# lucidrains/progen

Measured on NVIDIA B200. Metric: tokens_per_sec, higher is better.
Workload: dtype bf16

## Files before the change

### include/progen_b200.h

```cpp
#ifndef PROGEN_B200_H
#define PROGEN_B200_H
#include <stdint.h>

#ifdef __cplusplus
extern "C" {
#endif

#define PROGEN_F32 0
#define PROGEN_BF16 1

#define PROGEN_BACKEND_SIMT 0
#define PROGEN_BACKEND_TCGEN05 1

#define PROGEN_EPI_STORE 0
#define PROGEN_EPI_ROTARY 1
#define PROGEN_EPI_RESIDUAL 2
#define PROGEN_EPI_GLU 3
#define PROGEN_EPI_GELU 4
#define PROGEN_EPI_GLU_BWD 5
#define PROGEN_EPI_GELU_BWD 6
#define PROGEN_EPI_ACCUM 7

const char* progen_version(void);
const char* progen_last_error(void);
int progen_device_check(void);
long long progen_launch_count(void);

typedef struct progen_gemm_t {
  int32_t M, N, K;
  int32_t a_mn_major, b_mn_major;
  int32_t batch;
  int32_t batch_reduce;
  int32_t causal;
  int32_t split_k;
  int32_t in_dtype, out_dtype, epi_kind, backend;
  int32_t seq_len, dim_head;
  int32_t atomic, tril, tril_rows;
  int64_t lda, ldb;
  int64_t a_batch_rows, b_batch_rows, d_batch_rows;
  int64_t ldo, ldo2, ldaux;
  const void* A;
  const void* B;
  void* out;
  void* out2;
  const float* bias;
  const void* aux;
  const float* rot_sin;
  const float* rot_cos;
} progen_gemm_t;

int progen_gemm(const progen_gemm_t* desc, void* stream);

int progen_embed_fwd(const int* tokens, const float* table, float* x, long long T, int d, int V, void* stream);
int progen_embed_bwd(const int* tokens, const float* dx, float* dtable, long long T, int d, int V, void* stream);

int progen_ln_shift_fwd(const void* x, long long ldx, int x_dtype, const float* scale, void* y, long long ldy, int y_dtype,
                        float* mean, float* rstd, long long T, int d, int seq_len, int shift, void* stream);
int progen_ln_shift_bwd(const void* dy, long long lddy, int act_dtype, const void* x, long long ldx, int x_dtype,
                        const float* scale, const float* mean, const float* rstd, float* dres, void* dout, long long ldo,
                        float* dscale, float* dres_colsum, long long T, int d, int seq_len, int shift, int residual,
                        void* stream);

int progen_colsum(const void* in, long long ld, int dtype, float* out, long long T, int N, void* stream);

int progen_ce_fwd_bwd(const void* logits, int dtype, const int* labels, float* weights, float* loss, void* dlogits,
                      int dlogits_dtype, int B, int n, int V, float inv_batch, void* stream);

int progen_rotary_bwd(void* dqkv, long long ld, int dtype, const float* sin_t, const float* cos_t, long long T, int ncols,
                      int seq_len, int dim_head, void* stream);

int progen_local_attn_fwd_simt(const void* qkv, void* out, float* lse, int dtype, int B, int seq_len, int window, int heads,
                               int dim_head, void* stream);
int progen_local_attn_bwd_simt(const void* qkv, const void* out, const void* dout, const float* lse, void* dqkv,
                               float* delta, int dtype, int B, int seq_len, int window, int heads, int dim_head,
                               void* stream);

int progen_local_attn_fwd(const void* qkv, void* out, float* lse, int B, int seq_len, int window, int heads, int dim_head,
                          void* stream);
int progen_local_attn_bwd(const void* qkv, const void* out, const void* dout, const float* lse, void* dqkv, float* delta,
                          const float* rot_sin, const float* rot_cos, int B, int seq_len, int window, int heads, int dim_head,
                          void* stream);

int progen_local_attn_fwd_tc(const void* qkv, void* out, float* lse, int B, int seq_len, int window, int heads, int dim_head,
                             void* stream);

int progen_local_attn_bwd_tc(const void* qkv, const void* out, const void* dout, const float* lse, void* dqkv, float* delta,
                             const float* rot_sin, const float* rot_cos, int B, int seq_len, int window, int heads, int dim_head,
                             void* stream);
int progen_local_attn_bwd_tc_ex(const void* qkv, const void* out, const void* dout, const float* lse, void* dqkv, float* delta,
                                const float* rot_sin, const float* rot_cos, const float* rot_sin_t, const float* rot_cos_t, int B,
                                int seq_len, int window, int heads, int dim_head, int mode, void* stream);

int progen_sgu_gate_fwd(const void* xs, long long ldx, const void* gp, long long ldg, const float* bias, void* out,
                        long long ldo, int dtype, long long T, int C, int seq_len, void* stream);
int progen_sgu_gate_bwd(const void* ds, long long ldds, const void* xs, long long ldx, const void* gp, long long ldg,
                        const float* bias, void* dxs, long long lddx, void* dgp, long long lddg, float* dbias, int dtype,
                        long long T, int C, int seq_len, void* stream);
int progen_gelu_bwd(void* da, const void* u, int dtype, long long numel, void* stream);
int progen_cast_f32(const float* in, void* out, int out_dtype, long long numel, void* stream);
int progen_tril_cast(const float* w, void* out, int out_dtype, int n, void* stream);

int progen_optim_workspace_floats(void);
int progen_grad_sqnorm(const float* g, long long n, float* workspace, float* out_sqnorm, void* stream);
int progen_adamw_step(float* p, void* p_lp, const float* g, float* m, float* v, float* acc, long long n, long long n_decay,
                      const float* gnorm_sq, float lr, float b1, float b2, float eps, float wd, float max_norm,
                      long long step, int emit, void* stream);
int progen_adamw_step_dev(float* p, void* p_lp, const float* g, float* m, float* v, float* acc, long long n, long long n_decay,
                          const float* gnorm_sq, float lr, float b1, float b2, float eps, float wd, float max_norm,
                          int apply_every, void* state, void* stream);

typedef struct progen_decode_layer_t {
  int32_t kind;
  int32_t _pad;
  const float* ln1_scale;
  const void* wqkv_t;
  const void* wo_t;
  const float* bo;
  const float* ln2_scale;
  const void* win_t;
  const float* bin;
  const void* wout_t;
  const float* bout;
  const float* sgu_ln_scale;
  const float* sgu_w;
  const float* sgu_b;
  const void* sgu_proj_t;
  const float* sgu_proj_b;
  float* kcache;
  float* vcache;
  float* shift1;
  float* shift2;
  float* gn_hist;
} progen_decode_layer_t;

typedef struct progen_decode_t {
  int32_t n, d, heads, dim_head, inner, window, hid, V, depth, wdtype, shift_tokens, top_k;
  const float* embed;
  const float* lnf_scale;
  const void* whead_t;
  const float* bhead;
  const float* rot_sin;
  const float* rot_cos;
  const progen_decode_layer_t* layers;
  int32_t* seq;
  int32_t* pos;
  const float* noise;
  float* logits_all;
  float *x, *y, *q, *att, *u, *gn, *sg, *pj, *logits;
} progen_decode_t;

int progen_decode_step(const progen_decode_t* model, int do_sample, void* stream);

typedef struct progen_decode_run_t {
  int32_t n, d, heads, dim_head, inner, window, hid, V, depth, wdtype, shift_tokens, top_k;
  int32_t B, pos0, nsteps, _pad;
  const float* embed;
  const float* lnf_scale;
  const void* whead_t;
  const float* bhead;
  const float* rot_sin;
  const float* rot_cos;
  const progen_decode_layer_t* layers;
  int32_t* seq;
  const int32_t* start;
  const float* noise;
  float* logits_all;
  float* x;
  float* q;
  float* att;
  float* att_part;
  int32_t* att_count;
  float* u;
  float* sg;
  float* pj;
  float* logits;
  uint32_t* grid_bar;
  long long* prof;
} progen_decode_run_t;

int progen_decode_run(const progen_decode_run_t* run, void* stream);

#ifdef __cplusplus
}
#endif
#endif
```

### progen_b200/csrc/api.cu

```cuda
#include <stdarg.h>
#include "gemm.h"
#include "../../include/progen_b200.h"

static thread_local char g_err[1024] = "";
unsigned long long g_progen_launches = 0;

void progen_set_error(const char* fmt, ...) {
  va_list ap;
  va_start(ap, fmt);
  vsnprintf(g_err, sizeof(g_err), fmt, ap);
  va_end(ap);
}

extern "C" {

const char* progen_version(void) { return "progen_b200 0.1.0 (sm_100a; tcgen05/TMA GEMM, CUDA " CUDA_VERSION_STR ")"; }

const char* progen_last_error(void) { return g_err; }

long long progen_launch_count(void) { return (long long)__atomic_load_n(&g_progen_launches, __ATOMIC_RELAXED); }

int progen_device_check(void) {
  int dev = 0;
  PG_CUDA(cudaGetDevice(&dev));
  cudaDeviceProp prop;
  PG_CUDA(cudaGetDeviceProperties(&prop, dev));
  if (prop.major != 10) {
    progen_set_error("device %d (%s) is sm_%d%d; libprogen_b200 is built for sm_100a only", dev, prop.name, prop.major,
                     prop.minor);
    return PROGEN_ERR_DEVICE;
  }
  return PROGEN_OK;
}

int progen_gemm(const progen_gemm_t* d, void* stream) {
  PG_CHECK_ARG(d != nullptr);
  GemmArgs g;
  g.M = d->M; g.N = d->N; g.K = d->K;
  g.A = d->A; g.lda = d->lda; g.a_mn_major = d->a_mn_major;
  g.B = d->B; g.ldb = d->ldb; g.b_mn_major = d->b_mn_major;
  g.batch = d->batch < 1 ? 1 : d->batch;
  g.a_batch_rows = d->a_batch_rows; g.b_batch_rows = d->b_batch_rows; g.d_batch_rows = d->d_batch_rows;
  g.batch_reduce = d->batch_reduce; g.causal = d->causal; g.split_k = d->split_k < 1 ? 1 : d->split_k;
  g.in_dtype = d->in_dtype; g.out_dtype = d->out_dtype; g.epi_kind = d->epi_kind;
  g.epi.out = d->out; g.epi.ldo = d->ldo; g.epi.out2 = d->out2; g.epi.ldo2 = d->ldo2;
  g.epi.bias = d->bias; g.epi.aux = d->aux; g.epi.ldaux = d->ldaux;
  g.epi.rot_sin = d->rot_sin; g.epi.rot_cos = d->rot_cos;
  g.epi.seq_len = d->seq_len > 0 ? d->seq_len : 1; g.epi.dim_head = d->dim_head > 0 ? d->dim_head : 2;
  g.epi.atomic = d->atomic; g.epi.tril = d->tril; g.epi.tril_rows = d->tril_rows > 0 ? d->tril_rows : 1;
  PG_CHECK_ARG(g.epi_kind >= 0 && g.epi_kind < EPI_NUM_KINDS);
  PG_CHECK_ARG(g.epi.out != nullptr);
  if (g.epi_kind == EPI_GLU || g.epi_kind == EPI_GELU) PG_CHECK_ARG(g.epi.out2 != nullptr && g.epi.bias != nullptr);
  if (g.epi_kind == EPI_GLU_BWD || g.epi_kind == EPI_GELU_BWD) PG_CHECK_ARG(g.epi.aux != nullptr);
  if (g.epi_kind == EPI_ROTARY) PG_CHECK_ARG(g.epi.rot_sin && g.epi.rot_cos && d->seq_len > 0 && d->dim_head > 0 && d->dim_head % 2 == 0);
  if (d->backend == PROGEN_BACKEND_TCGEN05) return gemm_tc_launch(g, (cudaStream_t)stream);
  if (d->backend == PROGEN_BACKEND_SIMT) return gemm_simt_launch(g, (cudaStream_t)stream);
  progen_set_error("progen_gemm: unknown backend %d", d->backend);
  return PROGEN_ERR_ARG;
}

}
```

### progen_b200/csrc/elementwise.cu

```cuda
#include "common.cuh"
#include "../../include/progen_b200.h"

int ln_shift_bwd_stream_launch(const void* dy, long long lddy, int act_dtype, const void* x, long long ldx, int x_dtype,
                               const float* scale, const float* mean, const float* rstd, float* dres, void* dout,
                               long long ldo, float* dscale, float* dres_colsum, long long T, int d, int seq_len, int shift,
                               int residual, cudaStream_t stream);

namespace {

constexpr int ROWS_PER_BLOCK = 8;
constexpr float LN_EPS = 1e-5f;

template <typename T> __device__ __forceinline__ void load4(const T* p, float (&v)[4]);
template <> __device__ __forceinline__ void load4<float>(const float* p, float (&v)[4]) {
  const float4 t = *reinterpret_cast<const float4*>(p);
  v[0] = t.x; v[1] = t.y; v[2] = t.z; v[3] = t.w;
}
template <> __device__ __forceinline__ void load4<bf16>(const bf16* p, float (&v)[4]) {
  const uint2 t = *reinterpret_cast<const uint2*>(p);
  const float2 a = __bfloat1622float2(*reinterpret_cast<const __nv_bfloat162*>(&t.x));
  const float2 b = __bfloat1622float2(*reinterpret_cast<const __nv_bfloat162*>(&t.y));
  v[0] = a.x; v[1] = a.y; v[2] = b.x; v[3] = b.y;
}
__device__ __forceinline__ void store4(float* p, const float (&v)[4]) {
  *reinterpret_cast<float4*>(p) = make_float4(v[0], v[1], v[2], v[3]);
}
__device__ __forceinline__ void store4(bf16* p, const float (&v)[4]) {
  uint2 t;
  t.x = pack_bf16x2(v[0], v[1]); t.y = pack_bf16x2(v[2], v[3]);
  *reinterpret_cast<uint2*>(p) = t;
}

__global__ void embed_fwd_kernel(const int* __restrict__ tok, const float* __restrict__ table, float* __restrict__ x,
                                 long long T, int d, int V) {
  const long long total = T * (d / 4);
  for (long long i = blockIdx.x * (long long)blockDim.x + threadIdx.x; i < total; i += (long long)gridDim.x * blockDim.x) {
    const long long t = i / (d / 4);
    const int c = (int)(i % (d / 4)) * 4;
    int id = tok[t];
    id = id < 0 ? 0 : (id >= V ? V - 1 : id);
    *reinterpret_cast<float4*>(x + t * d + c) = *reinterpret_cast<const float4*>(table + (long long)id * d + c);
  }
}

__global__ void embed_bwd_kernel(const int* __restrict__ tok, const float* __restrict__ dx, float* __restrict__ dtable,
                                 long long T, int d, int V, long long rows_per_block) {
  extern __shared__ float bins[];
  const int c0 = blockIdx.x * 32;
  const int lane = threadIdx.x & 31, warp = threadIdx.x >> 5, nwarp = blockDim.x >> 5;
  for (int i = threadIdx.x; i < V * 32; i += blockDim.x) bins[i] = 0.f;
  __syncthreads();
  const long long r0 = blockIdx.y * rows_per_block;
  const long long r1 = min(T, r0 + rows_per_block);
  if (c0 + lane < d) {
    for (long long t = r0 + warp; t < r1; t += nwarp) {
      int id = tok[t];
      id = id < 0 ? 0 : (id >= V ? V - 1 : id);
      atomicAdd(&bins[id * 32 + lane], dx[t * d + c0 + lane]);
    }
  }
  __syncthreads();
  for (int i = threadIdx.x; i < V * 32; i += blockDim.x) {
    const float v = bins[i];
    const int c = c0 + (i & 31);
    if (v != 0.f && c < d) atomicAdd(dtable + (long long)(i >> 5) * d + c, v);
  }
}

template <typename TI, typename TO>
__global__ void ln_shift_fwd_kernel(const TI* __restrict__ x, long long ldx, const float* __restrict__ scale,
                                    TO* __restrict__ y, long long ldy, float* __restrict__ mean_out,
                                    float* __restrict__ rstd_out, long long T, int d, int seq_len, int shift) {
  const int lane = threadIdx.x & 31, warp = threadIdx.x >> 5;
  const int half = d >> 1;
  for (long long t = blockIdx.x * (long long)ROWS_PER_BLOCK + warp; t < T; t += (long long)gridDim.x * ROWS_PER_BLOCK) {
    const TI* xr = x + t * ldx;
    float s = 0.f;
    for (int c = lane * 4; c < d; c += 128) {
      float v[4];
      load4<TI>(xr + c, v);
      s += v[0] + v[1] + v[2] + v[3];
    }
    const float mean = warp_sum(s) / d;
    float q = 0.f;
    for (int c = lane * 4; c < d; c += 128) {
      float v[4];
      load4<TI>(xr + c, v);
#pragma unroll
      for (int i = 0; i < 4; ++i) { const float u = v[i] - mean; q += u * u; }
    }
    const float rstd = rsqrtf(warp_sum(q) / d + LN_EPS);
    if (lane == 0) { mean_out[t] = mean; rstd_out[t] = rstd; }
    const int pos = (int)(t % seq_len);
    for (int c = lane * 4; c < d; c += 128) {
      float v[4], sc[4], o[4];
      load4<TI>(xr + c, v);
      load4<float>(scale + c, sc);
#pragma unroll
      for (int i = 0; i < 4; ++i) o[i] = (v[i] - mean) * rstd * sc[i];
      if (!shift || c >= half) {
        store4(y + t * ldy + c, o);
      } else {
        if (pos + 1 < seq_len) store4(y + (t + 1) * ldy + c, o);
        if (pos == 0) { const float z[4] = {0.f, 0.f, 0.f, 0.f}; store4(y + t * ldy + c, z); }
      }
    }
  }
}

template <typename TI, typename TO, int NCH, bool RESIDUAL>
__global__ void ln_shift_bwd_kernel(const TO* __restrict__ dy, long long lddy, const TI* __restrict__ x, long long ldx,
                                    const float* __restrict__ scale, const float* __restrict__ mean_in,
                                    const float* __restrict__ rstd_in, float* __restrict__ dres, TO* __restrict__ dout,
                                    long long ldo, float* __restrict__ dscale, float* __restrict__ dres_colsum,
                                    long long T, int d, int seq_len, int shift) {
  const int lane = threadIdx.x & 31, warp = threadIdx.x >> 5;
  const int half = d >> 1;
  float ds_acc[NCH][4];
  float cs_acc[RESIDUAL ? NCH : 1][4];
#pragma unroll
  for (int i = 0; i < NCH; ++i)
#pragma unroll
    for (int j = 0; j < 4; ++j) {
      ds_acc[i][j] = 0.f;
      if (RESIDUAL) cs_acc[RESIDUAL ? i : 0][j] = 0.f;
    }

  for (long long t = blockIdx.x * (long long)ROWS_PER_BLOCK + warp; t < T; t += (long long)gridDim.x * ROWS_PER_BLOCK) {
    const TI* xr = x + t * ldx;
    const float mean = mean_in[t], rstd = rstd_in[t];
    const int pos = (int)(t % seq_len);
    const bool has_next = pos + 1 < seq_len;
    float s1 = 0.f, s2 = 0.f;
    if constexpr (NCH <= 4) {
      float xh[NCH][4], gs[NCH][4], rr[NCH][4];
#pragma unroll
      for (int ch = 0; ch < NCH; ++ch) {
        const int c = ch * 128 + lane * 4;
#pragma unroll
        for (int i = 0; i < 4; ++i) { xh[ch][i] = 0.f; gs[ch][i] = 0.f; rr[ch][i] = 0.f; }
        if (c < d) {
          float sc[4];
          load4<TI>(xr + c, xh[ch]);
          load4<float>(scale + c, sc);
          if (!shift || c >= half) load4<TO>(dy + t * lddy + c, gs[ch]);
          else if (has_next) load4<TO>(dy + (t + 1) * lddy + c, gs[ch]);
          if constexpr (RESIDUAL) load4<float>(dres + t * (long long)d + c, rr[ch]);
#pragma unroll
          for (int i = 0; i < 4; ++i) {
            xh[ch][i] = (xh[ch][i] - mean) * rstd;
            ds_acc[ch][i] += gs[ch][i] * xh[ch][i];
            gs[ch][i] *= sc[i];
            s1 += gs[ch][i]; s2 += gs[ch][i] * xh[ch][i];
          }
        }
      }
      s1 = warp_sum(s1) / d;
      s2 = warp_sum(s2) / d;
#pragma unroll
      for (int ch = 0; ch < NCH; ++ch) {
        const int c = ch * 128 + lane * 4;
        if (c < d) {
          float o[4];
#pragma unroll
          for (int i = 0; i < 4; ++i) o[i] = rstd * (gs[ch][i] - s1 - xh[ch][i] * s2);
          if constexpr (RESIDUAL) {
#pragma unroll
            for (int i = 0; i < 4; ++i) { rr[ch][i] += o[i]; cs_acc[ch][i] += rr[ch][i]; }
            store4(dres + t * (long long)d + c, rr[ch]);
            if (dout) store4(dout + t * ldo + c, rr[ch]);
          } else {
            store4(dout + t * ldo + c, o);
          }
        }
      }
      continue;
    }
#pragma unroll
    for (int ch = 0; ch < NCH; ++ch) {
      const int c = ch * 128 + lane * 4;
      if (c < d) {
        float xv[4], sc[4], g[4] = {0.f, 0.f, 0.f, 0.f};
        load4<TI>(xr + c, xv);
        load4<float>(scale + c, sc);
        if (!shift || c >= half) load4<TO>(dy + t * lddy + c, g);
        else if (has_next) load4<TO>(dy + (t + 1) * lddy + c, g);
#pragma unroll
        for (int i = 0; i < 4; ++i) {
          const float xh = (xv[i] - mean) * rstd;
          ds_acc[ch][i] += g[i] * xh;
          const float gs = g[i] * sc[i];
          s1 += gs; s2 += gs * xh;
        }
      }
    }
    s1 = warp_sum(s1) / d;
    s2 = warp_sum(s2) / d;
#pragma unroll
    for (int ch = 0; ch < NCH; ++ch) {
      const int c = ch * 128 + lane * 4;
      if (c < d) {
        float xv[4], sc[4], g[4] = {0.f, 0.f, 0.f, 0.f}, o[4];
        load4<TI>(xr + c, xv);
        load4<float>(scale + c, sc);
        if (!shift || c >= half) load4<TO>(dy + t * lddy + c, g);
        else if (has_next) load4<TO>(dy + (t + 1) * lddy + c, g);
#pragma unroll
        for (int i = 0; i < 4; ++i) {
          const float xh = (xv[i] - mean) * rstd;
          o[i] = rstd * (g[i] * sc[i] - s1 - xh * s2);
        }
        if constexpr (RESIDUAL) {
          float r[4];
          load4<float>(dres + t * (long long)d + c, r);
#pragma unroll
          for (int i = 0; i < 4; ++i) { r[i] += o[i]; cs_acc[ch][i] += r[i]; }
          store4(dres + t * (long long)d + c, r);
          if (dout) store4(dout + t * ldo + c, r);
        } else {
          store4(dout + t * ldo + c, o);
        }
      }
    }
  }
  __shared__ float red[ROWS_PER_BLOCK][128];
#pragma unroll
  for (int ch = 0; ch < NCH; ++ch) {
    if (ch * 128 >= d) break;
#pragma unroll
    for (int i = 0; i < 4; ++i) red[warp][lane * 4 + i] = ds_acc[ch][i];
    __syncthreads();
    if (threadIdx.x < 128) {
      float s = 0.f;
#pragma unroll
      for (int w = 0; w < ROWS_PER_BLOCK; ++w) s += red[w][threadIdx.x];
      const int c = ch * 128 + threadIdx.x;
      if (c < d) atomicAdd(dscale + c, s);
    }
    __syncthreads();
    if constexpr (RESIDUAL) {
      if (dres_colsum) {
#pragma unroll
        for (int i = 0; i < 4; ++i) red[warp][lane * 4 + i] = cs_acc[ch][i];
        __syncthreads();
        if (threadIdx.x < 128) {
          float s = 0.f;
#pragma unroll
          for (int w = 0; w < ROWS_PER_BLOCK; ++w) s += red[w][threadIdx.x];
          const int c = ch * 128 + threadIdx.x;
          if (c < d) atomicAdd(dres_colsum + c, s);
        }
        __syncthreads();
      }
    }
  }
}

template <typename TI>
__global__ void colsum_kernel(const TI* __restrict__ in, long long ld, float* __restrict__ out, long long T, int N,
                              long long rows_per_block) {
  __shared__ float red[ROWS_PER_BLOCK][128];
  const int lane = threadIdx.x & 31, warp = threadIdx.x >> 5;
  const int c = blockIdx.x * 128 + lane * 4;
  const long long r0 = blockIdx.y * rows_per_block, r1 = min(T, r0 + rows_per_block);
  float acc[4] = {0.f, 0.f, 0.f, 0.f};
  if (c < N) {
    for (long long t = r0 + warp; t < r1; t += ROWS_PER_BLOCK) {
      float v[4];
      load4<TI>(in + t * ld + c, v);
#pragma unroll
      for (int i = 0; i < 4; ++i) acc[i] += v[i];
    }
  }
#pragma unroll
  for (int i = 0; i < 4; ++i) red[warp][lane * 4 + i] = acc[i];
  __syncthreads();
  if (threadIdx.x < 128) {
    float s = 0.f;
#pragma unroll
    for (int w = 0; w < ROWS_PER_BLOCK; ++w) s += red[w][threadIdx.x];
    const int cc = blockIdx.x * 128 + threadIdx.x;
    if (cc < N) atomicAdd(out + cc, s);
  }
}

__global__ void ce_weights_kernel(const int* __restrict__ labels, float* __restrict__ w, int n, float inv_batch) {
  __shared__ int s_first, s_count;
  const int b = blockIdx.x;
  if (threadIdx.x == 0) { s_first = n; s_count = 0; }
  __syncthreads();
  const int* lb = labels + (long long)b * n;
  int first = n, cnt = 0;
  for (int i = threadIdx.x; i < n; i += blockDim.x) {
    if (lb[i] == 0) first = min(first, i); else cnt++;
  }
  atomicMin(&s_first, first);
  atomicAdd(&s_count, cnt);
  __syncthreads();
  const int total = s_count + (s_first < n ? 1 : 0);
  const float wv = inv_batch / (float)total;
  for (int i = threadIdx.x; i < n; i += blockDim.x) w[(long long)b * n + i] = (lb[i] != 0 || i == s_first) ? wv : 0.f;
}

template <typename TL, typename TD>
__global__ void ce_fwd_bwd_kernel(const TL* __restrict__ logits, const int* __restrict__ labels,
                                  const float* __restrict__ w, float* __restrict__ loss, TD* __restrict__ dlogits,
                                  long long T, int V) {
  const int lane = threadIdx.x & 31, warp = threadIdx.x >> 5;
  float block_loss = 0.f;
  for (long long t = blockIdx.x * (long long)ROWS_PER_BLOCK + warp; t < T; t += (long long)gridDim.x * ROWS_PER_BLOCK) {
    const TL* lr = logits + t * V;
    float mx = -INFINITY;
    for (int c = lane * 4; c < V; c += 128) {
      float v[4];
      load4<TL>(lr + c, v);
      mx = fmaxf(mx, fmaxf(fmaxf(v[0], v[1]), fmaxf(v[2], v[3])));
    }
    mx = warp_max(mx);
    float se = 0.f;
    for (int c = lane * 4; c < V; c += 128) {
      float v[4];
      load4<TL>(lr + c, v);
#pragma unroll
      for (int i = 0; i < 4; ++i) se += expf(v[i] - mx);
    }
    se = warp_sum(se);
    const int lab = min(max(labels[t], 0), V - 1);
    const float wt = w[t];
    const float lse = mx + logf(se);
    if (lane == 0) block_loss += wt * (lse - to_f32(lr[lab]));
    if (dlogits) {
      const float inv = 1.f / se;
      for (int c = lane * 4; c < V; c += 128) {
        float v[4], o[4];
        load4<TL>(lr + c, v);
#pragma unroll
        for (int i = 0; i < 4; ++i) o[i] = wt * (expf(v[i] - mx) * inv - ((c + i) == lab ? 1.f : 0.f));
        store4(dlogits + t * V + c, o);
      }
    }
  }
  __shared__ float red[ROWS_PER_BLOCK];
  if (lane == 0) red[warp] = block_loss;
  __syncthreads();
  if (threadIdx.x == 0) {
    float s = 0.f;
    for (int i = 0; i < ROWS_PER_BLOCK; ++i) s += red[i];
    atomicAdd(loss, s);
  }
}

template <typename TO>
__global__ void rotary_bwd_kernel(TO* __restrict__ dqkv, long long ld, const float* __restrict__ sin_t,
                                  const float* __restrict__ cos_t, long long T, int ncols, int seq_len, int dim_head) {
  const long long total = T * (ncols / 4);
  const int half = dim_head >> 1;
  for (long long i = blockIdx.x * (long long)blockDim.x + threadIdx.x; i < total; i += (long long)gridDim.x * blockDim.x) {
    const long long t = i / (ncols / 4);
    const int c = (int)(i % (ncols / 4)) * 4;
    const int pos = (int)(t % seq_len);
    float v[4], o[4];
    load4<TO>(dqkv + t * ld + c, v);
#pragma unroll
    for (int p = 0; p < 4; p += 2) {
      const int j = ((c + p) % dim_head) >> 1;
      const float s = __ldg(sin_t + (long long)pos * half + j), cs = __ldg(cos_t + (long long)pos * half + j);
      o[p] = v[p] * cs + v[p + 1] * s;
      o[p + 1] = v[p + 1] * cs - v[p] * s;
    }
    store4(dqkv + t * ld + c, o);
  }
}

template <typename TO>
__global__ void sgu_gate_fwd_kernel(const TO* __restrict__ xs, long long ldx, const TO* __restrict__ gp, long long ldg,
                                    const float* __restrict__ bias, TO* __restrict__ out, long long ldo, long long T, int C,
                                    int seq_len) {
  const long long total = T * (C / 4);
  for (long long i = blockIdx.x * (long long)blockDim.x + threadIdx.x; i < total; i += (long long)gridDim.x * blockDim.x) {
    const long long t = i / (C / 4);
    const int c = (int)(i % (C / 4)) * 4;
    const float b = __ldg(bias + (t % seq_len));
    float x[4], g[4], o[4];
    load4<TO>(xs + t * ldx + c, x);
    load4<TO>(gp + t * ldg + c, g);
#pragma unroll
    for (int j = 0; j < 4; ++j) o[j] = x[j] * (g[j] + b);
    store4(out + t * ldo + c, o);
  }
}

template <typename TO>
__global__ void sgu_gate_bwd_kernel(const TO* __restrict__ ds, long long ldds, const TO* __restrict__ xs, long long ldx,
                                    const TO* __restrict__ gp, long long ldg, const float* __restrict__ bias,
                                    TO* __restrict__ dxs, long long lddx, TO* __restrict__ dgp, long long lddg,
                                    float* __restrict__ dbias, long long T, int C, int seq_len) {
  const int lane = threadIdx.x & 31, warp = threadIdx.x >> 5;
  for (long long t = blockIdx.x * (long long)ROWS_PER_BLOCK + warp; t < T; t += (long long)gridDim.x * ROWS_PER_BLOCK) {
    const int m = (int)(t % seq_len);
    const float b = __ldg(bias + m);
    float acc = 0.f;
    for (int c = lane * 4; c < C; c += 128) {
      float d[4], x[4], g[4], o1[4], o2[4];
      load4<TO>(ds + t * ldds + c, d);
      load4<TO>(xs + t * ldx + c, x);
      load4<TO>(gp + t * ldg + c, g);
#pragma unroll
      for (int j = 0; j < 4; ++j) {
        o1[j] = d[j] * (g[j] + b);
        o2[j] = d[j] * x[j];
        acc += o2[j];
      }
      store4(dxs + t * lddx + c, o1);
      store4(dgp + t * lddg + c, o2);
    }
    acc = warp_sum(acc);
    if (lane == 0) atomicAdd(dbias + m, acc);
  }
}

template <typename TO>
__global__ void gelu_bwd_kernel(TO* __restrict__ da, const TO* __restrict__ u, long long total4) {
  for (long long i = blockIdx.x * (long long)blockDim.x + threadIdx.x; i < total4; i += (long long)gridDim.x * blockDim.x) {
    float d[4], x[4];
    load4<TO>(da + i * 4, d);
    load4<TO>(u + i * 4, x);
#pragma unroll
    for (int j = 0; j < 4; ++j) d[j] *= gelu_tanh_grad(x[j]);
    store4(da + i * 4, d);
  }
}

template <typename TO>
__global__ void cast_kernel(const float* __restrict__ in, TO* __restrict__ out, long long total4) {
  for (long long i = blockIdx.x * (long long)blockDim.x + threadIdx.x; i < total4; i += (long long)gridDim.x * blockDim.x) {
    float v[4];
    load4<float>(in + i * 4, v);
    store4(out + i * 4, v);
  }
}

template <typename TO>
__global__ void tril_cast_kernel(const float* __restrict__ w, TO* __restrict__ out, int n) {
  const long long total = (long long)n * (n / 4);
  for (long long i = blockIdx.x * (long long)blockDim.x + threadIdx.x; i < total; i += (long long)gridDim.x * blockDim.x) {
    const int r = (int)(i / (n / 4));
    const int c = (int)(i % (n / 4)) * 4;
    float v[4];
    load4<float>(w + (long long)r * n + c, v);
#pragma unroll
    for (int j = 0; j < 4; ++j) v[j] = (c + j <= r) ? v[j] : 0.f;
    store4(out + (long long)r * n + c, v);
  }
}

inline int ew_grid(long long work_items, int threads) {
  long long b = (work_items + threads - 1) / threads;
  const long long cap = (long long)pg_num_sms() * 8;
  return (int)(b < 1 ? 1 : (b > cap ? cap : b));
}
inline int row_grid(long long T) {
  long long b = (T + ROWS_PER_BLOCK - 1) / ROWS_PER_BLOCK;
  const long long cap = (long long)pg_num_sms() * 4;
  return (int)(b < 1 ? 1 : (b > cap ? cap : b));
}

}

extern "C" {

int progen_embed_fwd(const int* tokens, const float* table, float* x, long long T, int d, int V, void* stream) {
  PG_CHECK_ARG(T > 0 && d % 4 == 0 && V > 0);
  embed_fwd_kernel<<<ew_grid(T * (d / 4), 256), 256, 0, (cudaStream_t)stream>>>(tokens, table, x, T, d, V);
  PG_LAUNCH_CHECK();
  return PROGEN_OK;
}

int progen_embed_bwd(const int* tokens, const float* dx, float* dtable, long long T, int d, int V, void* stream) {
  PG_CHECK_ARG(T > 0 && d > 0 && V > 0 && V * 32 * 4 <= 48 * 1024);
  const int row_blocks = (int)((T + 4095) / 4096);
  const long long rpb = (T + row_blocks - 1) / row_blocks;
  dim3 grid((d + 31) / 32, row_blocks);
  embed_bwd_kernel<<<grid, 256, V * 32 * sizeof(float), (cudaStream_t)stream>>>(tokens, dx, dtable, T, d, V, rpb);
  PG_LAUNCH_CHECK();
  return PROGEN_OK;
}

int progen_ln_shift_fwd(const void* x, long long ldx, int x_dtype, const float* scale, void* y, long long ldy, int y_dtype,
                        float* mean, float* rstd, long long T, int d, int seq_len, int shift, void* stream) {
  PG_CHECK_ARG(T > 0 && d % 8 == 0 && seq_len > 0 && T % seq_len == 0);
  PG_CHECK_ARG(ldx % 4 == 0 && ldy % 4 == 0);
  cudaStream_t s = (cudaStream_t)stream;
  const int grid = row_grid(T);
#define LN_FWD(TI, TO) ln_shift_fwd_kernel<TI, TO><<<grid, 256, 0, s>>>((const TI*)x, ldx, scale, (TO*)y, ldy, mean, rstd, T, d, seq_len, shift)
  if (x_dtype == PG_F32 && y_dtype == PG_F32) LN_FWD(float, float);
  else if (x_dtype == PG_F32 && y_dtype == PG_BF16) LN_FWD(float, bf16);
  else if (x_dtype == PG_BF16 && y_dtype == PG_BF16) LN_FWD(bf16, bf16);
  else { progen_set_error("ln_shift_fwd: unsupported dtypes %d -> %d", x_dtype, y_dtype); return PROGEN_ERR_UNSUPPORTED; }
#undef LN_FWD
  PG_LAUNCH_CHECK();
  return PROGEN_OK;
}

int progen_ln_shift_bwd(const void* dy, long long lddy, int act_dtype, const void* x, long long ldx, int x_dtype,
                        const float* scale, const float* mean, const float* rstd, float* dres, void* dout, long long ldo,
                        float* dscale, float* dres_colsum, long long T, int d, int seq_len, int shift, int residual,
                        void* stream) {
  PG_CHECK_ARG(T > 0 && d % 8 == 0 && d <= 4096 && seq_len > 0 && T % seq_len == 0);
  PG_CHECK_ARG(residual ? (dres != nullptr && x_dtype == PG_F32) : (dout != nullptr));
  cudaStream_t s = (cudaStream_t)stream;
  const int rc_stream = ln_shift_bwd_stream_launch(dy, lddy, act_dtype, x, ldx, x_dtype, scale, mean, rstd, dres, dout, ldo,
                                                   dscale, dres_colsum, T, d, seq_len, shift, residual, s);
  if (rc_stream <= 0) return rc_stream;
  long long b = (T + ROWS_PER_BLOCK - 1) / ROWS_PER_BLOCK;
  const int per_sm = d <= 1024 ? 6 : 3;
  const int grid = (int)(b > pg_num_sms() * per_sm ? pg_num_sms() * per_sm : b);
  const int nch = (d + 127) / 128;
#define LN_BWD_N(TI, TO, NCH, RES) ln_shift_bwd_kernel<TI, TO, NCH, RES><<<grid, 256, 0, s>>>((const TO*)dy, lddy, (const TI*)x, ldx, scale, mean, rstd, dres, (TO*)dout, ldo, dscale, dres_colsum, T, d, seq_len, shift)
#define LN_BWD(TI, TO, RES) do { if (nch <= 4) LN_BWD_N(TI, TO, 4, RES); else if (nch <= 8) LN_BWD_N(TI, TO, 8, RES); \
    else if (nch <= 16) LN_BWD_N(TI, TO, 16, RES); else LN_BWD_N(TI, TO, 32, RES); } while (0)
  if (residual) {
    if (act_dtype == PG_F32) LN_BWD(float, float, true);
    else LN_BWD(float, bf16, true);
  } else {
    if (act_dtype == PG_F32 && x_dtype == PG_F32) LN_BWD(float, float, false);
    else if (act_dtype == PG_BF16 && x_dtype == PG_BF16) LN_BWD(bf16, bf16, false);
    else if (act_dtype == PG_BF16 && x_dtype == PG_F32) LN_BWD(float, bf16, false);
    else { progen_set_error("ln_shift_bwd: unsupported dtypes"); return PROGEN_ERR_UNSUPPORTED; }
  }
#undef LN_BWD
#undef LN_BWD_N
  PG_LAUNCH_CHECK();
  return PROGEN_OK;
}

int progen_colsum(const void* in, long long ld, int dtype, float* out, long long T, int N, void* stream) {
  PG_CHECK_ARG(T > 0 && N % 4 == 0 && ld % 4 == 0);
  int row_blocks = (int)((T + 1023) / 1024);
  if (row_blocks > 64) row_blocks = 64;
  const long long rpb = (T + row_blocks - 1) / row_blocks;
  dim3 grid((N + 127) / 128, row_blocks);
  if (dtype == PG_F32) colsum_kernel<float><<<grid, 256, 0, (cudaStream_t)stream>>>((const float*)in, ld, out, T, N, rpb);
  else colsum_kernel<bf16><<<grid, 256, 0, (cudaStream_t)stream>>>((const bf16*)in, ld, out, T, N, rpb);
  PG_LAUNCH_CHECK();
  return PROGEN_OK;
}

int progen_ce_fwd_bwd(const void* logits, int dtype, const int* labels, float* weights, float* loss, void* dlogits,
                      int dlogits_dtype, int B, int n, int V, float inv_batch, void* stream) {
  PG_CHECK_ARG(B > 0 && n > 0 && V % 4 == 0);
  cudaStream_t s = (cudaStream_t)stream;
  const long long T = (long long)B * n;
  ce_weights_kernel<<<B, 256, 0, s>>>(labels, weights, n, inv_batch);
  PG_LAUNCH_CHECK();
  const int grid = row_grid(T);
#define CE_CASE(TL, TD) ce_fwd_bwd_kernel<TL, TD><<<grid, 256, 0, s>>>((const TL*)logits, labels, weights, loss, (TD*)dlogits, T, V)
  if (dtype == PG_F32 && dlogits_dtype == PG_F32) CE_CASE(float, float);
  else if (dtype == PG_F32 && dlogits_dtype == PG_BF16) CE_CASE(float, bf16);
  else if (dtype == PG_BF16 && dlogits_dtype == PG_BF16) CE_CASE(bf16, bf16);
  else { progen_set_error("ce_fwd_bwd: unsupported dtypes %d / %d", dtype, dlogits_dtype); return PROGEN_ERR_UNSUPPORTED; }
#undef CE_CASE
  PG_LAUNCH_CHECK();
  return PROGEN_OK;
}

int progen_rotary_bwd(void* dqkv, long long ld, int dtype, const float* sin_t, const float* cos_t, long long T, int ncols,
                      int seq_len, int dim_head, void* stream) {
  PG_CHECK_ARG(T > 0 && ncols % 4 == 0 && dim_head % 2 == 0 && ld % 4 == 0);
  cudaStream_t s = (cudaStream_t)stream;
  const int grid = ew_grid(T * (ncols / 4), 256);
  if (dtype == PG_F32) rotary_bwd_kernel<float><<<grid, 256, 0, s>>>((float*)dqkv, ld, sin_t, cos_t, T, ncols, seq_len, dim_head);
  else rotary_bwd_kernel<bf16><<<grid, 256, 0, s>>>((bf16*)dqkv, ld, sin_t, cos_t, T, ncols, seq_len, dim_head);
  PG_LAUNCH_CHECK();
  return PROGEN_OK;
}

int progen_sgu_gate_fwd(const void* xs, long long ldx, const void* gp, long long ldg, const float* bias, void* out,
                        long long ldo, int dtype, long long T, int C, int seq_len, void* stream) {
  PG_CHECK_ARG(T > 0 && C % 4 == 0 && ldx % 4 == 0 && ldg % 4 == 0 && ldo % 4 == 0);
  cudaStream_t s = (cudaStream_t)stream;
  const int grid = ew_grid(T * (C / 4), 256);
  if (dtype == PG_F32) sgu_gate_fwd_kernel<float><<<grid, 256, 0, s>>>((const float*)xs, ldx, (const float*)gp, ldg, bias, (float*)out, ldo, T, C, seq_len);
  else sgu_gate_fwd_kernel<bf16><<<grid, 256, 0, s>>>((const bf16*)xs, ldx, (const bf16*)gp, ldg, bias, (bf16*)out, ldo, T, C, seq_len);
  PG_LAUNCH_CHECK();
  return PROGEN_OK;
}

int progen_sgu_gate_bwd(const void* ds, long long ldds, const void* xs, long long ldx, const void* gp, long long ldg,
                        const float* bias, void* dxs, long long lddx, void* dgp, long long lddg, float* dbias, int dtype,
                        long long T, int C, int seq_len, void* stream) {
  PG_CHECK_ARG(T > 0 && C % 4 == 0);
  cudaStream_t s = (cudaStream_t)stream;
  if (dtype == PG_F32) sgu_gate_bwd_kernel<float><<<row_grid(T), 256, 0, s>>>((const float*)ds, ldds, (const float*)xs, ldx, (const float*)gp, ldg, bias, (float*)dxs, lddx, (float*)dgp, lddg, dbias, T, C, seq_len);
  else sgu_gate_bwd_kernel<bf16><<<row_grid(T), 256, 0, s>>>((const bf16*)ds, ldds, (const bf16*)xs, ldx, (const bf16*)gp, ldg, bias, (bf16*)dxs, lddx, (bf16*)dgp, lddg, dbias, T, C, seq_len);
  PG_LAUNCH_CHECK();
  return PROGEN_OK;
}

int progen_gelu_bwd(void* da, const void* u, int dtype, long long numel, void* stream) {
  PG_CHECK_ARG(numel > 0 && numel % 4 == 0);
  cudaStream_t s = (cudaStream_t)stream;
  const int grid = ew_grid(numel / 4, 256);
  if (dtype == PG_F32) gelu_bwd_kernel<float><<<grid, 256, 0, s>>>((float*)da, (const float*)u, numel / 4);
  else gelu_bwd_kernel<bf16><<<grid, 256, 0, s>>>((bf16*)da, (const bf16*)u, numel / 4);
  PG_LAUNCH_CHECK();
  return PROGEN_OK;
}

int progen_cast_f32(const float* in, void* out, int out_dtype, long long numel, void* stream) {
  PG_CHECK_ARG(numel > 0 && numel % 4 == 0);
  cudaStream_t s = (cudaStream_t)stream;
  const int grid = ew_grid(numel / 4, 256);
  if (out_dtype == PG_F32) cast_kernel<float><<<grid, 256, 0, s>>>(in, (float*)out, numel / 4);
  else cast_kernel<bf16><<<grid, 256, 0, s>>>(in, (bf16*)out, numel / 4);
  PG_LAUNCH_CHECK();
  return PROGEN_OK;
}

int progen_tril_cast(const float* w, void* out, int out_dtype, int n, void* stream) {
  PG_CHECK_ARG(n > 0 && n % 4 == 0);
  cudaStream_t s = (cudaStream_t)stream;
  const int grid = ew_grid((long long)n * (n / 4), 256);
  if (out_dtype == PG_F32) tril_cast_kernel<float><<<grid, 256, 0, s>>>(w, (float*)out, n);
  else tril_cast_kernel<bf16><<<grid, 256, 0, s>>>(w, (bf16*)out, n);
  PG_LAUNCH_CHECK();
  return PROGEN_OK;
}

}
```

### progen_b200/csrc/epilogues.cuh

```cuda
#pragma once
#include "common.cuh"

enum EpiKind : int {
  EPI_STORE = 0,
  EPI_ROTARY = 1,
  EPI_RESIDUAL = 2,
  EPI_GLU = 3,
  EPI_GELU = 4,
  EPI_GLU_BWD = 5,
  EPI_GELU_BWD = 6,
  EPI_ACCUM = 7,
  EPI_NUM_KINDS = 8
};

struct EpiArgs {
  void* out; long long ldo;
  void* out2; long long ldo2;
  const float* bias;
  const void* aux; long long ldaux;
  const float* rot_sin;
  const float* rot_cos;
  int seq_len; int dim_head;
  int atomic;
  int tril;
  int tril_rows;
};

struct DirectIO {
  template <int N, typename T> __device__ __forceinline__ void store(T* p, long long, const float (&v)[N], bool valid) const {
    if (valid) store_vec<N>(p, v);
  }
  template <int N, typename T> __device__ __forceinline__ void load(const T* p, long long, float (&v)[N], bool valid) const {
    if (valid) load_vec<N>(p, v);
    else {
#pragma unroll
      for (int i = 0; i < N; ++i) v[i] = 0.f;
    }
  }
};

constexpr int STAGE_WARP_BYTES = 32 * 64;

template <int PPR> __device__ __forceinline__ int stage_off(int r, int q) {
  return r * (PPR * 16) + ((q ^ ((r * PPR / 8) & (PPR - 1))) << 4);
}

struct WarpStagedIO {
  uint8_t* buf;
  int lane;
  unsigned valid_mask;

  template <typename T> static __device__ __forceinline__ uint4 pack16(const float* v) {
    uint4 t;
    if constexpr (sizeof(T) == 2) {
      t.x = pack_bf16x2(v[0], v[1]); t.y = pack_bf16x2(v[2], v[3]); t.z = pack_bf16x2(v[4], v[5]); t.w = pack_bf16x2(v[6], v[7]);
    } else {
      t.x = __float_as_uint(v[0]); t.y = __float_as_uint(v[1]); t.z = __float_as_uint(v[2]); t.w = __float_as_uint(v[3]);
    }
    return t;
  }
  template <typename T> static __device__ __forceinline__ void unpack16(const uint4 t, float* v) {
    if constexpr (sizeof(T) == 2) {
      const __nv_bfloat162* h = reinterpret_cast<const __nv_bfloat162*>(&t);
#pragma unroll
      for (int j = 0; j < 4; ++j) { const float2 f = __bfloat1622float2(h[j]); v[2 * j] = f.x; v[2 * j + 1] = f.y; }
    } else {
      v[0] = __uint_as_float(t.x); v[1] = __uint_as_float(t.y); v[2] = __uint_as_float(t.z); v[3] = __uint_as_float(t.w);
    }
  }

  template <int N, typename T> __device__ __forceinline__ void store(T* p, long long ld, const float (&v)[N], bool) const {
    constexpr int BYTES = N * (int)sizeof(T);
    constexpr int SW = BYTES < 64 ? BYTES : 64;
    constexpr int PPR = SW / 16;
    constexpr int EPP = 16 / (int)sizeof(T);
    uint8_t* base = reinterpret_cast<uint8_t*>(p - (long long)lane * ld);
#pragma unroll
    for (int s = 0; s < BYTES / SW; ++s) {
#pragma unroll
      for (int q = 0; q < PPR; ++q)
        *reinterpret_cast<uint4*>(buf + stage_off<PPR>(lane, q)) = pack16<T>(&v[s * (SW / (int)sizeof(T)) + q * EPP]);
      __syncwarp();
#pragma unroll
      for (int it = 0; it < PPR; ++it) {
        const int idx = it * 32 + lane;
        const int r = idx / PPR, q = idx % PPR;
        if ((valid_mask >> r) & 1u) {
          const uint4 t = *reinterpret_cast<const uint4*>(buf + stage_off<PPR>(r, q));
          *reinterpret_cast<uint4*>(base + (long long)r * ld * (int)sizeof(T) + s * SW + q * 16) = t;
        }
      }
      __syncwarp();
    }
  }
  template <int N, typename T>
  __device__ __forceinline__ void load_issue(const T* p, long long ld, uint4 (&t)[N * (int)sizeof(T) / 16], unsigned mask) const {
    constexpr int BYTES = N * (int)sizeof(T);
    constexpr int SW = BYTES < 64 ? BYTES : 64;
    constexpr int PPR = SW / 16;
    constexpr int PASSES = BYTES / SW;
    const uint8_t* base = reinterpret_cast<const uint8_t*>(p - (long long)lane * ld);
#pragma unroll
    for (int s = 0; s < PASSES; ++s) {
#pragma unroll
      for (int it = 0; it < PPR; ++it) {
        const int idx = it * 32 + lane;
        const int r = idx / PPR, q = idx % PPR;
        t[s * PPR + it] = make_uint4(0u, 0u, 0u, 0u);
        if ((mask >> r) & 1u)
          t[s * PPR + it] = *reinterpret_cast<const uint4*>(base + (long long)r * ld * (int)sizeof(T) + s * SW + q * 16);
      }
    }
  }
  template <int N, typename T> __device__ __forceinline__ void load(const T* p, long long ld, float (&v)[N], bool) const {
    uint4 t[N * (int)sizeof(T) / 16];
    load_issue<N, T>(p, ld, t, valid_mask);
    load_finish<N, T>(t, v);
  }
  template <int N, typename T>
  __device__ __forceinline__ void load_finish(const uint4 (&t)[N * (int)sizeof(T) / 16], float (&v)[N]) const {
    constexpr int BYTES = N * (int)sizeof(T);
    constexpr int SW = BYTES < 64 ? BYTES : 64;
    constexpr int PPR = SW / 16;
    constexpr int EPP = 16 / (int)sizeof(T);
    constexpr int PASSES = BYTES / SW;
#pragma unroll
    for (int s = 0; s < PASSES; ++s) {
#pragma unroll
      for (int it = 0; it < PPR; ++it) {
        const int idx = it * 32 + lane;
        const int r = idx / PPR, q = idx % PPR;
        *reinterpret_cast<uint4*>(buf + stage_off<PPR>(r, q)) = t[s * PPR + it];
      }
      __syncwarp();
#pragma unroll
      for (int q = 0; q < PPR; ++q)
        unpack16<T>(*reinterpret_cast<const uint4*>(buf + stage_off<PPR>(lane, q)), &v[s * (SW / (int)sizeof(T)) + q * EPP]);
      __syncwarp();
    }
  }
};

template <int NV> __device__ __forceinline__ void add_bias(const float* __restrict__ bias, int col, float (&v)[NV]) {
#pragma unroll
  for (int i = 0; i < NV; i += 4) {
    const float4 b = __ldg(reinterpret_cast<const float4*>(bias + col + i));
    v[i] += b.x; v[i + 1] += b.y; v[i + 2] += b.z; v[i + 3] += b.w;
  }
}

template <int KIND, typename TO, int NV, typename IO>
__device__ __forceinline__ void epi_apply(const EpiArgs& e, const IO& io, long long row, int col, float (&v)[NV], bool valid) {
  constexpr bool FAST = sizeof(TO) == 2;
  if constexpr (KIND == EPI_STORE) {
    if (e.bias) add_bias<NV>(e.bias, col, v);
    io.template store<NV>(reinterpret_cast<TO*>(e.out) + row * e.ldo + col, e.ldo, v, valid);
  } else if constexpr (KIND == EPI_ROTARY) {
    const int pos = (int)(row % e.seq_len);
    const int half = e.dim_head >> 1;
    const float* sp = e.rot_sin + (long long)pos * half;
    const float* cp = e.rot_cos + (long long)pos * half;
    float o[NV];
    if (e.dim_head % NV == 0) {
      const int j0 = (col % e.dim_head) >> 1;
      float s[NV / 2], c[NV / 2];
      if constexpr (NV >= 32) {
        io.template load<NV / 2>(sp + j0, half, s, true);
        io.template load<NV / 2>(cp + j0, half, c, true);
      } else {
        load_vec<NV / 2>(sp + j0, s);
        load_vec<NV / 2>(cp + j0, c);
      }
#pragma unroll
      for (int i = 0; i < NV; i += 2) {
        o[i] = v[i] * c[i >> 1] - v[i + 1] * s[i >> 1];
        o[i + 1] = v[i + 1] * c[i >> 1] + v[i] * s[i >> 1];
      }
    } else {
#pragma unroll
      for (int i = 0; i < NV; i += 2) {
        const int j = ((col + i) % e.dim_head) >> 1;
        const float s = __ldg(sp + j), c = __ldg(cp + j);
        o[i] = v[i] * c - v[i + 1] * s;
        o[i + 1] = v[i + 1] * c + v[i] * s;
      }
    }
    io.template store<NV>(reinterpret_cast<TO*>(e.out) + row * e.ldo + col, e.ldo, o, valid);
  } else if constexpr (KIND == EPI_RESIDUAL) {
    float* p = reinterpret_cast<float*>(e.out) + row * e.ldo + col;
    float r[NV];
    if (e.aux) io.template load<NV>(reinterpret_cast<const float*>(e.aux) + row * e.ldaux + col, e.ldaux, r, valid);
    else io.template load<NV>(const_cast<const float*>(p), e.ldo, r, valid);
    if (e.bias) add_bias<NV>(e.bias, col, v);
#pragma unroll
    for (int i = 0; i < NV; ++i) r[i] += v[i];
    io.template store<NV>(p, e.ldo, r, valid);
  } else if constexpr (KIND == EPI_GLU) {
    add_bias<NV>(e.bias, col, v);
    io.template store<NV>(reinterpret_cast<TO*>(e.out2) + row * e.ldo2 + col, e.ldo2, v, valid);
    TO* po = reinterpret_cast<TO*>(e.out) + row * e.ldo + (col >> 1);
    if constexpr (NV >= 16) {
      float o[NV / 2];
#pragma unroll
      for (int i = 0; i < NV / 2; ++i) o[i] = v[2 * i] * gelu_fwd<FAST>(v[2 * i + 1]);
      io.template store<NV / 2>(po, e.ldo, o, valid);
    } else {
      if (valid) {
#pragma unroll
        for (int i = 0; i < NV / 2; ++i) po[i] = from_f32<TO>(v[2 * i] * gelu_fwd<FAST>(v[2 * i + 1]));
      }
    }
  } else if constexpr (KIND == EPI_GELU) {
    add_bias<NV>(e.bias, col, v);
    io.template store<NV>(reinterpret_cast<TO*>(e.out2) + row * e.ldo2 + col, e.ldo2, v, valid);
    float o[NV];
#pragma unroll
    for (int i = 0; i < NV; ++i) o[i] = gelu_fwd<FAST>(v[i]);
    io.template store<NV>(reinterpret_cast<TO*>(e.out) + row * e.ldo + col, e.ldo, o, valid);
  } else if constexpr (KIND == EPI_GLU_BWD) {
    float u[2 * NV];
    io.template load<2 * NV>(reinterpret_cast<const TO*>(e.aux) + row * e.ldaux + 2 * col, e.ldaux, u, valid);
#pragma unroll
    for (int i = 0; i < NV; ++i) {
      const float dh = v[i], val = u[2 * i], gate = u[2 * i + 1];
      float gf, gd;
      gelu_fwd_bwd<FAST>(gate, gf, gd);
      u[2 * i] = dh * gf;
      u[2 * i + 1] = dh * val * gd;
    }
    io.template store<2 * NV>(reinterpret_cast<TO*>(e.out) + row * e.ldo + 2 * col, e.ldo, u, valid);
  } else if constexpr (KIND == EPI_GELU_BWD) {
    float u[NV];
    io.template load<NV>(reinterpret_cast<const TO*>(e.aux) + row * e.ldaux + col, e.ldaux, u, valid);
#pragma unroll
    for (int i = 0; i < NV; ++i) v[i] *= gelu_bwd<FAST>(u[i]);
    io.template store<NV>(reinterpret_cast<TO*>(e.out) + row * e.ldo + col, e.ldo, v, valid);
  } else if constexpr (KIND == EPI_ACCUM) {
    if (!valid) return;
    float* p = reinterpret_cast<float*>(e.out) + row * e.ldo + col;
    const int lim = e.tril ? (int)(row % e.tril_rows) : 0x7fffffff;
    if (e.atomic) {
#pragma unroll
      for (int i = 0; i < NV; i += 4) {
        if (col + i + 3 <= lim) {
          asm volatile("red.global.add.v4.f32 [%0], {%1, %2, %3, %4};" ::"l"(p + i), "f"(v[i]), "f"(v[i + 1]),
                       "f"(v[i + 2]), "f"(v[i + 3]) : "memory");
        } else {
#pragma unroll
          for (int j = 0; j < 4; ++j)
            if (col + i + j <= lim) atomicAdd(p + i + j, v[i + j]);
        }
      }
    } else {
      float r[NV];
      load_vec<NV>(p, r);
#pragma unroll
      for (int i = 0; i < NV; ++i) r[i] += (col + i <= lim) ? v[i] : 0.f;
      store_vec<NV>(p, r);
    }
  }
}

template <int KIND> constexpr bool epi_has_aux = KIND == EPI_RESIDUAL || KIND == EPI_GLU_BWD || KIND == EPI_GELU_BWD;
```

### progen_b200/csrc/gemm_tc2.cu

```cuda
#include "tc_ptx.cuh"
#include "gemm.h"

namespace {

using namespace tc;
using namespace tc2;

constexpr int BM = 128;
constexpr int BN = 256;
constexpr int BK = 64;
constexpr int EW = 8;
constexpr int NGROUP = 2;
constexpr int CPG = BN / NGROUP / 32;
constexpr int THREADS = 128 + 32 * EW;
constexpr int A_BYTES = BM * BK * 2;
constexpr int B_BYTES = (BN / 2) * BK * 2;
constexpr int STAGE_BYTES = A_BYTES + B_BYTES;
constexpr int BAR_BYTES = 256;
constexpr int TMEM_COLS = 2 * BN;
constexpr int SMEM_LIMIT = 227 * 1024;

template <int KIND, typename TO> struct Epi2 {
  static constexpr bool AUX = epi_has_aux<KIND>;
  static constexpr int ROWB0 = (KIND == EPI_RESIDUAL || KIND == EPI_ACCUM) ? 32 * 4 : KIND == EPI_GLU_BWD ? 64 * (int)sizeof(TO) : 32 * (int)sizeof(TO);
  static constexpr int ROWB1 = KIND == EPI_GLU ? 16 * (int)sizeof(TO) : KIND == EPI_GELU ? 32 * (int)sizeof(TO) : 0;
  static constexpr int NB = AUX ? 3 : 2;
  static constexpr int SLOT_BYTES = BM * (ROWB0 + ROWB1);
  static constexpr int SLOTS_TOTAL = NGROUP * NB * SLOT_BYTES;
  static constexpr int ROT_BYTES = KIND == EPI_ROTARY ? EW * STAGE_WARP_BYTES : 0;
  static constexpr int FIXED = 1024 + SLOTS_TOTAL + BAR_BYTES + ROT_BYTES;
  static constexpr int STAGES_FIT = (SMEM_LIMIT - FIXED) / STAGE_BYTES;
  static constexpr int STAGES = STAGES_FIT > 6 ? 6 : STAGES_FIT;
  static constexpr int SMEM_TOTAL = STAGES * STAGE_BYTES + FIXED;
  static_assert(ROWB0 <= 128 && ROWB0 >= 32 && STAGES >= 3, "epilogue slot shape");
};

struct Gemm2Dev {
  int M, N, K;
  int split_k;
  EpiArgs epi;
};

template <int CL>
__device__ __forceinline__ bool decode_tile2(const Gemm2Dev& g, int t, int& m0, int& n0, int& kb0, int& kb1) {
  const int m_tiles = (g.M + 2 * BM - 1) / (2 * BM);
  const int n_tiles = g.N / (BN * CL);
  const int tiles = m_tiles * n_tiles;
  if (t >= tiles * g.split_k) return false;
  const int tile = t % tiles, sp = t / tiles;
  m0 = (tile / n_tiles) * (2 * BM);
  n0 = (tile % n_tiles) * (BN * CL);
  const long long kb_total = g.K / BK;
  kb0 = (int)(kb_total * sp / g.split_k);
  kb1 = (int)(kb_total * (sp + 1) / g.split_k);
  return true;
}

template <int ROWB> __device__ __forceinline__ uint32_t box_off(int r, int q) { return (uint32_t)stage_off<ROWB / 16>(r, q); }

template <int ROWB, typename T, int N> __device__ __forceinline__ void box_read(const uint8_t* box, int r, float (&v)[N]) {
  constexpr int EPP = 16 / (int)sizeof(T);
  static_assert(N * (int)sizeof(T) == ROWB, "row width");
#pragma unroll
  for (int q = 0; q < ROWB / 16; ++q)
    WarpStagedIO::unpack16<T>(*reinterpret_cast<const uint4*>(box + box_off<ROWB>(r, q)), &v[q * EPP]);
}
template <int ROWB, typename T, int N> __device__ __forceinline__ void box_write(uint8_t* box, int r, const float (&v)[N]) {
  constexpr int EPP = 16 / (int)sizeof(T);
  static_assert(N * (int)sizeof(T) == ROWB, "row width");
#pragma unroll
  for (int q = 0; q < ROWB / 16; ++q)
    *reinterpret_cast<uint4*>(box + box_off<ROWB>(r, q)) = WarpStagedIO::pack16<T>(&v[q * EPP]);
}

template <bool A_MN, bool B_MN, int KIND, typename TO, int CL>
__global__ void __launch_bounds__(THREADS, 1)
gemm_tc2_kernel(const __grid_constant__ CUtensorMap tma_a, const __grid_constant__ CUtensorMap tma_b,
                const __grid_constant__ CUtensorMap tma_aux, const __grid_constant__ CUtensorMap tma_out,
                const __grid_constant__ CUtensorMap tma_out2, const Gemm2Dev g) {
  using E = Epi2<KIND, TO>;
  constexpr int STAGES = E::STAGES;
  extern __shared__ uint8_t smem_raw[];
  const uint32_t smem_base = (smem_u32(smem_raw) + 1023u) & ~1023u;
  const uint32_t slots_base = smem_base + STAGES * STAGE_BYTES;
  const uint32_t bar_base = slots_base + E::SLOTS_TOTAL;
  auto full_bar = [&](int s) { return bar_base + 8u * s; };
  auto empty_bar = [&](int s) { return bar_base + 8u * (6 + s); };
  auto tfull_bar = [&](int s) { return bar_base + 8u * (12 + s); };
  auto tempty_bar = [&](int s) { return bar_base + 8u * (14 + s); };
  auto sready_bar = [&](int grp, int b) { return bar_base + 8u * (16 + grp * 3 + b); };
  const uint32_t tmem_slot = bar_base + 8u * 22;
  uint8_t* gen = smem_raw + (smem_base - smem_u32(smem_raw));

  const int warp = threadIdx.x >> 5, lane = threadIdx.x & 31;
  const uint32_t crank = cluster_ctarank();
  const uint32_t rank = crank & 1u, pidx = crank >> 1, lead_crank = crank & ~1u;
  const bool leader = rank == 0;
  const int pair = blockIdx.x / (2 * CL), npairs = gridDim.x / (2 * CL);
  const int ncol = (int)pidx * BN;
  constexpr uint16_t ALL_CTAS = (uint16_t)((1u << (2 * CL)) - 1u);

  if (warp == 0 && lane == 0) {
    prefetch_tensormap(&tma_a); prefetch_tensormap(&tma_b); prefetch_tensormap(&tma_out);
    if constexpr (E::AUX) prefetch_tensormap(&tma_aux);
    if constexpr (E::ROWB1 > 0) prefetch_tensormap(&tma_out2);
  }
  if (warp == 1 && lane == 0) {
    for (int s = 0; s < STAGES; ++s) { mbar_init(full_bar(s), 1); mbar_init(empty_bar(s), CL); }
    for (int s = 0; s < 2; ++s) { mbar_init(tfull_bar(s), 1); mbar_init(tempty_bar(s), 2 * EW); }
    for (int grp = 0; grp < NGROUP; ++grp)
      for (int b = 0; b < E::NB; ++b) mbar_init(sready_bar(grp, b), 1);
    fence_barrier_init();
  }
  if (warp == 2) tmem_alloc_pair<TMEM_COLS>(tmem_slot);
  tcgen05_fence_before();
  cluster_sync();
  tcgen05_fence_after();
  const uint32_t tmem_base = *reinterpret_cast<volatile uint32_t*>(gen + (tmem_slot - smem_base));

  if (warp == 0) {
    {
      int stage = 0;
      uint32_t phase = 0;
      int m0, n0, kb0, kb1;
      for (int t = pair; decode_tile2<CL>(g, t, m0, n0, kb0, kb1); t += npairs) {
        n0 += ncol;
        for (int kb = kb0; kb < kb1; ++kb) {
          mbar_wait(empty_bar(stage), phase ^ 1);
          const uint32_t sa = smem_base + stage * STAGE_BYTES, sb = sa + A_BYTES;
          const uint32_t lead_full = mapa(full_bar(stage), lead_crank);
          const int k0 = kb * BK;
          if (elect_one()) {
          if (leader) mbar_expect_tx(full_bar(stage), 2 * STAGE_BYTES);
          if constexpr (CL == 1) {
            if constexpr (!A_MN) {
              tma_load_2d_pair(sa, &tma_a, lead_full, k0, m0 + (int)rank * BM);
            } else {
#pragma unroll
              for (int i = 0; i < BM / 64; ++i)
                tma_load_2d_pair(sa + i * 8192, &tma_a, lead_full, m0 + (int)rank * BM + 64 * i, k0);
            }
          } else if (pidx == 0) {
            const uint16_t mask = (uint16_t)((1u << rank) | (1u << (rank + 2)));
            if constexpr (!A_MN) {
              tma_load_2d_pair_mc(sa, &tma_a, full_bar(stage), mask, k0, m0 + (int)rank * BM);
            } else {
#pragma unroll
              for (int i = 0; i < BM / 64; ++i)
                tma_load_2d_pair_mc(sa + i * 8192, &tma_a, full_bar(stage), mask, m0 + (int)rank * BM + 64 * i, k0);
            }
          }
          if constexpr (!B_MN) {
            tma_load_2d_pair(sb, &tma_b, lead_full, k0, n0 + (int)rank * (BN / 2));
          } else {
#pragma unroll
            for (int i = 0; i < BN / 2 / 64; ++i)
              tma_load_2d_pair(sb + i * 8192, &tma_b, lead_full, n0 + (int)rank * (BN / 2) + 64 * i, k0);
          }
          }
          __syncwarp();
          if (++stage == STAGES) { stage = 0; phase ^= 1; }
        }
      }
    }
  } else if (warp == 1) {
    if (leader) {
      constexpr uint32_t idesc = make_idesc(2 * BM, BN, A_MN, B_MN);
      int stage = 0, acc = 0;
      uint32_t phase = 0, acc_phase = 0;
      int m0, n0, kb0, kb1;
      for (int t = pair; decode_tile2<CL>(g, t, m0, n0, kb0, kb1); t += npairs) {
        mbar_wait(tempty_bar(acc), acc_phase ^ 1);
        tcgen05_fence_after();
        const uint32_t d_tmem = tmem_base + acc * BN;
        for (int kb = kb0; kb < kb1; ++kb) {
          mbar_wait(full_bar(stage), phase);
          tcgen05_fence_after();
          const uint32_t sa = smem_base + stage * STAGE_BYTES;
          const uint64_t adesc = make_smem_desc<A_MN>(sa);
          const uint64_t bdesc = make_smem_desc<B_MN>(sa + A_BYTES);
          if (elect_one()) {
#pragma unroll
            for (int k = 0; k < BK / 16; ++k)
              umma_bf16_pair(d_tmem, adesc + (uint64_t)(k * (A_MN ? (2048 >> 4) : 2)),
                             bdesc + (uint64_t)(k * (B_MN ? (2048 >> 4) : 2)), idesc, (kb > kb0 || k > 0) ? 1u : 0u);
            tcgen05_commit_pair(empty_bar(stage), ALL_CTAS);
          }
          __syncwarp();
          if (++stage == STAGES) { stage = 0; phase ^= 1; }
        }
        if (elect_one()) tcgen05_commit_pair(tfull_bar(acc), (uint16_t)(3u << (2 * pidx)));
        __syncwarp();
        if (++acc == 2) { acc = 0; acc_phase ^= 1; }
      }
    }
  } else if (warp >= 4) {
    const int q = warp & 3;
    const int grp = (warp - 4) >> 2;
    const int r_in_tile = q * 32 + lane;
    const bool elected = q == 0 && lane == 0;
    const int m_tiles = (g.M + 2 * BM - 1) / (2 * BM), n_tiles = g.N / (BN * CL);
    const int total_tiles = m_tiles * n_tiles * g.split_k;
    const int my_tiles = total_tiles > pair ? (total_tiles - pair + npairs - 1) / npairs : 0;
    const int nchunks = my_tiles * CPG;
    auto chunk_coords = [&](int i, int& row0, int& col) {
      int m0, n0, kb0, kb1;
      decode_tile2<CL>(g, pair + (i / CPG) * npairs, m0, n0, kb0, kb1);
      row0 = m0 + (int)rank * BM;
      col = n0 + ncol + (grp * CPG + (i % CPG)) * 32;
    };
    auto slot_addr = [&](int b) { return slots_base + (uint32_t)((grp * E::NB + b) * E::SLOT_BYTES); };
    auto prepare = [&](int i) {
      const int b = i % E::NB;
      if constexpr (E::AUX) {
        int row0, col;
        chunk_coords(i, row0, col);
        mbar_expect_tx(sready_bar(grp, b), BM * E::ROWB0);
        tma_load_2d(slot_addr(b), &tma_aux, sready_bar(grp, b), KIND == EPI_GLU_BWD ? 2 * col : col, row0);
      } else {
        mbar_arrive(sready_bar(grp, b));
      }
    };
    if (elected)
      for (int i = 0; i < E::NB - 1 && i < nchunks; ++i) prepare(i);

    WarpStagedIO rio;
    rio.buf = gen + (bar_base - smem_base) + BAR_BYTES + (warp - 4) * STAGE_WARP_BYTES;
    rio.lane = lane;
    rio.valid_mask = 0xffffffffu;
    float rs[KIND == EPI_ROTARY ? 32 : 1], rc[KIND == EPI_ROTARY ? 32 : 1];

    int acc = 0;
    uint32_t acc_phase = 0;
    uint32_t taddr = 0;
    uint32_t vr[32];
    constexpr bool PF = KIND != EPI_ROTARY;
    long long row = 0;
#pragma unroll 1
    for (int i = 0; i < nchunks; ++i) {
      int row0, col;
      chunk_coords(i, row0, col);
      const int ci = i % CPG;
      if (ci == 0) {
        row = row0 + r_in_tile;
        if constexpr (KIND == EPI_ROTARY) {
          const long long pos = row % g.epi.seq_len;
          rio.template load<32>(g.epi.rot_sin + pos * 32, 32, rs, true);
          rio.template load<32>(g.epi.rot_cos + pos * 32, 32, rc, true);
        }
        mbar_wait(tfull_bar(acc), acc_phase);
        tcgen05_fence_after();
        taddr = tmem_base + acc * BN + ((uint32_t)(q * 32) << 16) + grp * (CPG * 32);
        tmem_ld32_issue(taddr, vr);
      }
      else if (!PF) tmem_ld32_issue(taddr + ci * 32, vr);
      const int b = i % E::NB;
      tmem_ld32_wait(vr);
      float v[32];
#pragma unroll
      for (int j = 0; j < 32; ++j) v[j] = __uint_as_float(vr[j]);
      if (ci == CPG - 1) {
        tcgen05_fence_before();
        __syncwarp();
        if (lane == 0) mbar_arrive_cluster(mapa(tempty_bar(acc), lead_crank));
        if (++acc == 2) { acc = 0; acc_phase ^= 1; }
      }
      mbar_wait(sready_bar(grp, b), (uint32_t)(i / E::NB) & 1u);
      uint8_t* box0 = gen + (slot_addr(b) - smem_base);
      uint8_t* box1 = box0 + BM * E::ROWB0;
      constexpr bool FAST = sizeof(TO) == 2;
      if constexpr (KIND == EPI_STORE) {
        if (g.epi.bias) add_bias<32>(g.epi.bias, col, v);
        box_write<E::ROWB0, TO, 32>(box0, r_in_tile, v);
      } else if constexpr (KIND == EPI_ROTARY) {
        float o[32];
        if ((col & 32) == 0) {
#pragma unroll
          for (int j = 0; j < 32; j += 2) {
            o[j] = v[j] * rc[j >> 1] - v[j + 1] * rs[j >> 1];
            o[j + 1] = v[j + 1] * rc[j >> 1] + v[j] * rs[j >> 1];
          }
        } else {
#pragma unroll
          for (int j = 0; j < 32; j += 2) {
            o[j] = v[j] * rc[16 + (j >> 1)] - v[j + 1] * rs[16 + (j >> 1)];
            o[j + 1] = v[j + 1] * rc[16 + (j >> 1)] + v[j] * rs[16 + (j >> 1)];
          }
        }
        box_write<E::ROWB0, TO, 32>(box0, r_in_tile, o);
      } else if constexpr (KIND == EPI_RESIDUAL) {
        float r[32];
        box_read<E::ROWB0, float, 32>(box0, r_in_tile, r);
        if (g.epi.bias) add_bias<32>(g.epi.bias, col, v);
#pragma unroll
        for (int j = 0; j < 32; ++j) r[j] += v[j];
        box_write<E::ROWB0, float, 32>(box0, r_in_tile, r);
      } else if constexpr (KIND == EPI_GLU) {
        add_bias<32>(g.epi.bias, col, v);
        box_write<E::ROWB0, TO, 32>(box0, r_in_tile, v);
        float o[16];
#pragma unroll
        for (int j = 0; j < 16; ++j) o[j] = v[2 * j] * gelu_fwd<FAST>(v[2 * j + 1]);
        box_write<E::ROWB1, TO, 16>(box1, r_in_tile, o);
      } else if constexpr (KIND == EPI_GELU) {
        add_bias<32>(g.epi.bias, col, v);
        box_write<E::ROWB0, TO, 32>(box0, r_in_tile, v);
        float o[32];
#pragma unroll
        for (int j = 0; j < 32; ++j) o[j] = gelu_fwd<FAST>(v[j]);
        box_write<E::ROWB1, TO, 32>(box1, r_in_tile, o);
      } else if constexpr (KIND == EPI_GLU_BWD) {
        float u[64];
        box_read<E::ROWB0, TO, 64>(box0, r_in_tile, u);
#pragma unroll
        for (int j = 0; j < 32; ++j) {
          const float dh = v[j], val = u[2 * j], gate = u[2 * j + 1];
          float gf, gd;
          gelu_fwd_bwd<FAST>(gate, gf, gd);
          u[2 * j] = dh * gf;
          u[2 * j + 1] = dh * val * gd;
        }
        box_write<E::ROWB0, TO, 64>(box0, r_in_tile, u);
      } else if constexpr (KIND == EPI_ACCUM) {
        box_write<E::ROWB0, float, 32>(box0, r_in_tile, v);
      } else if constexpr (KIND == EPI_GELU_BWD) {
        float u[32];
        box_read<E::ROWB0, TO, 32>(box0, r_in_tile, u);
#pragma unroll
        for (int j = 0; j < 32; ++j) v[j] *= gelu_bwd<FAST>(u[j]);
        box_write<E::ROWB0, TO, 32>(box0, r_in_tile, v);
      }
      if (PF && ci + 1 < CPG) tmem_ld32_issue(taddr + (ci + 1) * 32, vr);
      fence_proxy_async();
      if (grp == 0) asm volatile("bar.sync 1, 128;" ::: "memory");
      else asm volatile("bar.sync 2, 128;" ::: "memory");
      if (elected) {
        if constexpr (KIND == EPI_GLU) {
          tma_store_2d(&tma_out2, slot_addr(b), col, row0);
          tma_store_2d(&tma_out, slot_addr(b) + BM * E::ROWB0, col >> 1, row0);
        } else if constexpr (KIND == EPI_GELU) {
          tma_store_2d(&tma_out2, slot_addr(b), col, row0);
          tma_store_2d(&tma_out, slot_addr(b) + BM * E::ROWB0, col, row0);
        } else if constexpr (KIND == EPI_ACCUM) {
          tma_reduce_add_2d(&tma_out, slot_addr(b), col, row0);
        } else {
          tma_store_2d(&tma_out, slot_addr(b), KIND == EPI_GLU_BWD ? 2 * col : col, row0);
        }
        bulk_commit_group();
        if (i + E::NB - 1 < nchunks) {
          bulk_wait_group_read<1>();
          prepare(i + E::NB - 1);
        }
      }
    }
    if (elected) bulk_wait_group<0>();
  }

  tcgen05_fence_before();
  cluster_sync();
  if (warp == 2) { tcgen05_fence_after(); tmem_dealloc_pair<TMEM_COLS>(tmem_base); }
}

template <bool A_MN, bool B_MN, int KIND, typename TO, int CL>
int max_clusters() {
  using E = Epi2<KIND, TO>;
  static int cached = -1;
  if (cached >= 0) return cached;
  auto kern = gemm_tc2_kernel<A_MN, B_MN, KIND, TO, CL>;
  if (cudaFuncSetAttribute(kern, cudaFuncAttributeMaxDynamicSharedMemorySize, E::SMEM_TOTAL) != cudaSuccess) return cached = 0;
  cudaLaunchConfig_t cfg{};
  cfg.gridDim = dim3(2 * CL * (pg_num_sms() / (2 * CL)));
  cfg.blockDim = dim3(THREADS);
  cfg.dynamicSmemBytes = E::SMEM_TOTAL;
  cudaLaunchAttribute attr[1];
  attr[0].id = cudaLaunchAttributeClusterDimension;
  attr[0].val.clusterDim.x = 2 * CL; attr[0].val.clusterDim.y = 1; attr[0].val.clusterDim.z = 1;
  cfg.attrs = attr;
  cfg.numAttrs = 1;
  int n = 0;
  if (cudaOccupancyMaxActiveClusters(&n, kern, &cfg) != cudaSuccess) { cudaGetLastError(); n = 0; }
  const int cap = pg_num_sms() / (2 * CL);
  if (getenv("PROGEN_DEBUG")) fprintf(stderr, "[progen] gemm_tc2 kind %d: %d resident clusters of %d CTAs (cap %d)\n", KIND, n, 2 * CL, cap);
  return cached = (n < cap ? n : cap);
}

template <bool A_MN, bool B_MN, int KIND, typename TO, int CL>
int launch2(const CUtensorMap& ta, const CUtensorMap& tb, const CUtensorMap& taux, const CUtensorMap& tout,
            const CUtensorMap& tout2, const Gemm2Dev& gd, int items, cudaStream_t stream) {
  using E = Epi2<KIND, TO>;
  auto kern = gemm_tc2_kernel<A_MN, B_MN, KIND, TO, CL>;
  int clusters = max_clusters<A_MN, B_MN, KIND, TO, CL>();
  if (clusters <= 0) { progen_set_error("gemm_tc2: no resident cluster of %d CTAs", 2 * CL); return PROGEN_ERR_CUDA; }
  if (items < clusters) clusters = items;
  cudaLaunchConfig_t cfg{};
  cfg.gridDim = dim3(2 * CL * clusters);
  cfg.blockDim = dim3(THREADS);
  cfg.dynamicSmemBytes = E::SMEM_TOTAL;
  cfg.stream = stream;
  cudaLaunchAttribute attr[1];
  attr[0].id = cudaLaunchAttributeClusterDimension;
  attr[0].val.clusterDim.x = 2 * CL; attr[0].val.clusterDim.y = 1; attr[0].val.clusterDim.z = 1;
  cfg.attrs = attr;
  cfg.numAttrs = 1;
  PG_CUDA(cudaLaunchKernelEx(&cfg, kern, ta, tb, taux, tout, tout2, gd));
  PG_LAUNCH_CHECK();
  return PROGEN_OK;
}

template <bool A_MN, bool B_MN, int KIND, typename TO>
int launch2_auto(const CUtensorMap& ta, const CUtensorMap& tb, const CUtensorMap& taux, const CUtensorMap& tout,
                 const CUtensorMap& tout2, Gemm2Dev gd, const GemmArgs& a, cudaStream_t stream) {
  static int quad = [] { const char* e = getenv("PROGEN_GEMM_4CTA"); return e ? atoi(e) : 0; }();
  const int m_tiles = (a.M + 2 * BM - 1) / (2 * BM);
  const bool use4 = quad && a.N % (2 * BN) == 0 && max_clusters<A_MN, B_MN, KIND, TO, 2>() > 0;
  const int cl = use4 ? 2 : 1;
  const int tiles = m_tiles * (a.N / (BN * cl));
  const int streams = use4 ? max_clusters<A_MN, B_MN, KIND, TO, 2>() : max_clusters<A_MN, B_MN, KIND, TO, 1>();
  int split = 1;
  if (a.epi_kind == EPI_ACCUM && a.epi.atomic && streams > 0) {
    const int kb_total = a.K / BK;
    double best = 0.0;
    for (int s = 1; s <= 48 && kb_total / s >= 16; ++s) {
      const int items = tiles * s, waves = (items + streams - 1) / streams;
      const double eff = (double)items / (waves * streams);
      if (eff > best + 0.02) { best = eff; split = s; }
    }
  }
  gd.split_k = split;
  if (use4) return launch2<A_MN, B_MN, KIND, TO, 2>(ta, tb, taux, tout, tout2, gd, tiles * split, stream);
  return launch2<A_MN, B_MN, KIND, TO, 1>(ta, tb, taux, tout, tout2, gd, tiles * split, stream);
}

}

bool gemm_tc2_eligible(const GemmArgs& a) {
  static int enabled = [] { const char* e = getenv("PROGEN_GEMM_2CTA"); return e ? atoi(e) : 1; }();
  if (!enabled) return false;
  if (a.in_dtype != PG_BF16 || a.batch != 1 || a.causal || a.batch_reduce) return false;
  if (a.N % BN != 0 || a.K % BK != 0 || a.M < 2 * BM) return false;
  const bool am = a.a_mn_major != 0, bm = a.b_mn_major != 0, obf = a.out_dtype == PG_BF16;
  if (a.epi_kind == EPI_ACCUM) {
    if (!am || !bm || a.epi.tril || a.M % 8 != 0) return false;
    if (a.split_k > 1 && !a.epi.atomic) return false;
    return a.epi.out && ((uintptr_t)a.epi.out & 15) == 0 && (a.epi.ldo * 4) % 16 == 0;
  }
  if (am || a.split_k != 1) return false;
  const int osz = obf ? 2 : 4;
  auto tma_ok = [](const void* p, long long ld, int esz) { return p && ((uintptr_t)p & 15) == 0 && (ld * esz) % 16 == 0; };
  switch (a.epi_kind) {
    case EPI_STORE: return tma_ok(a.epi.out, a.epi.ldo, osz);
    case EPI_ROTARY: return bm && obf && a.epi.dim_head == 64 && a.epi.seq_len % 128 == 0 && tma_ok(a.epi.out, a.epi.ldo, 2);
    case EPI_GLU: case EPI_GELU:
      return bm && obf && a.epi.bias && tma_ok(a.epi.out, a.epi.ldo, 2) && tma_ok(a.epi.out2, a.epi.ldo2, 2);
    case EPI_RESIDUAL:
      return bm && tma_ok(a.epi.out, a.epi.ldo, 4) && (!a.epi.aux || tma_ok(a.epi.aux, a.epi.ldaux, 4));
    case EPI_GLU_BWD: case EPI_GELU_BWD:
      return !bm && obf && tma_ok(a.epi.out, a.epi.ldo, 2) && tma_ok(a.epi.aux, a.epi.ldaux, 2);
    default: return false;
  }
}

int gemm_tc2_launch(const GemmArgs& a, cudaStream_t stream) {
  PG_CHECK_ARG(gemm_tc2_eligible(a));
  PG_CHECK_ARG(a.lda % 8 == 0 && a.ldb % 8 == 0);
  CUtensorMap ta, tb, taux, tout, tout2;
  int rc;
  if (!a.a_mn_major) rc = pg_tensor_map_2d_bf16(a.A, a.K, a.M, a.lda, BK, BM, &ta);
  else               rc = pg_tensor_map_2d_bf16(a.A, a.M, a.K, a.lda, 64, BK, &ta);
  if (rc) return rc;
  if (!a.b_mn_major) rc = pg_tensor_map_2d_bf16(a.B, a.K, a.N, a.ldb, BK, BN / 2, &tb);
  else               rc = pg_tensor_map_2d_bf16(a.B, a.N, a.K, a.ldb, 64, BK, &tb);
  if (rc) return rc;
  const bool bm = a.b_mn_major != 0, obf = a.out_dtype == PG_BF16;
  const uint32_t osz = obf ? 2 : 4;
  const EpiArgs& e = a.epi;
  auto emap = [&](const void* p, uint32_t esz, uint64_t width, long long ld, uint32_t box_cols, CUtensorMap* m) {
    return pg_tensor_map_2d(p, esz, width, (uint64_t)a.M, (uint64_t)ld, box_cols, BM, box_cols * esz, m);
  };
  taux = ta; tout2 = ta;
  switch (a.epi_kind) {
    case EPI_STORE: case EPI_ROTARY: rc = emap(e.out, osz, a.N, e.ldo, 32, &tout); break;
    case EPI_ACCUM: rc = emap(e.out, 4, a.N, e.ldo, 32, &tout); break;
    case EPI_RESIDUAL:
      rc = emap(e.out, 4, a.N, e.ldo, 32, &tout);
      if (!rc) rc = e.aux ? emap(e.aux, 4, a.N, e.ldaux, 32, &taux) : emap(e.out, 4, a.N, e.ldo, 32, &taux);
      break;
    case EPI_GLU:
      rc = emap(e.out2, 2, a.N, e.ldo2, 32, &tout2);
      if (!rc) rc = emap(e.out, 2, a.N / 2, e.ldo, 16, &tout);
      break;
    case EPI_GELU:
      rc = emap(e.out2, 2, a.N, e.ldo2, 32, &tout2);
      if (!rc) rc = emap(e.out, 2, a.N, e.ldo, 32, &tout);
      break;
    case EPI_GLU_BWD:
      rc = emap(e.out, 2, 2ull * a.N, e.ldo, 64, &tout);
      if (!rc) rc = emap(e.aux, 2, 2ull * a.N, e.ldaux, 64, &taux);
      break;
    case EPI_GELU_BWD:
      rc = emap(e.out, 2, a.N, e.ldo, 32, &tout);
      if (!rc) rc = emap(e.aux, 2, a.N, e.ldaux, 32, &taux);
      break;
    default: break;
  }
  if (rc) return rc;
  Gemm2Dev gd{a.M, a.N, a.K, 1, a.epi};
#define TC2_CASE(BMJ, KIND, TO) return launch2_auto<false, BMJ, KIND, TO>(ta, tb, taux, tout, tout2, gd, a, stream)
  switch (a.epi_kind) {
    case EPI_ACCUM: return launch2_auto<true, true, EPI_ACCUM, float>(ta, tb, taux, tout, tout2, gd, a, stream);
    case EPI_STORE:
      if (bm) { if (obf) TC2_CASE(true, EPI_STORE, bf16); else TC2_CASE(true, EPI_STORE, float); }
      else { if (obf) TC2_CASE(false, EPI_STORE, bf16); else TC2_CASE(false, EPI_STORE, float); }
    case EPI_ROTARY: if (bm && obf) TC2_CASE(true, EPI_ROTARY, bf16); break;
    case EPI_RESIDUAL: if (bm) TC2_CASE(true, EPI_RESIDUAL, float); break;
    case EPI_GLU: if (bm && obf) TC2_CASE(true, EPI_GLU, bf16); break;
    case EPI_GELU: if (bm && obf) TC2_CASE(true, EPI_GELU, bf16); break;
    case EPI_GLU_BWD: if (!bm && obf) TC2_CASE(false, EPI_GLU_BWD, bf16); break;
    case EPI_GELU_BWD: if (!bm && obf) TC2_CASE(false, EPI_GELU_BWD, bf16); break;
    default: break;
  }
#undef TC2_CASE
  progen_set_error("gemm_tc2: unsupported combination epi=%d b_mn=%d out=%d", a.epi_kind, (int)bm, a.out_dtype);
  return PROGEN_ERR_UNSUPPORTED;
}
```

### progen_b200/csrc/ln_stream.cu

```cuda
#include "tc_ptx.cuh"
#include "../../include/progen_b200.h"

namespace {

using namespace tc;

constexpr int RB = 8;
constexpr int CG = 2;
constexpr int CW = RB * CG;
constexpr int THREADS = 32 * (CW + 1);
constexpr int MAX_STAGES = 6;
constexpr int SMEM_BUDGET = 212 * 1024;

struct LnStreamArgs {
  const void* dy; long long lddy;
  const void* x; long long ldx;
  const float* scale; const float* mean; const float* rstd;
  float* dres;
  void* dout; long long ldo;
  float* dscale; float* dres_colsum;
  long long T; int d, seq_len, shift;
  int stages;
  int off_dy, off_r, off_out, off_stat, stage_bytes;
};

__device__ __forceinline__ void bulk_load(uint32_t dst, const void* src, uint32_t bytes, uint32_t bar) {
  asm volatile("cp.async.bulk.shared::cluster.global.mbarrier::complete_tx::bytes [%0], [%1], %2, [%3];"
               ::"r"(dst), "l"(src), "r"(bytes), "r"(bar) : "memory");
}
__device__ __forceinline__ void bulk_store(void* dst, uint32_t src, uint32_t bytes) {
  asm volatile("cp.async.bulk.global.shared::cta.bulk_group [%0], [%1], %2;" ::"l"(dst), "r"(src), "r"(bytes) : "memory");
}
__device__ __forceinline__ void bulk_commit() { asm volatile("cp.async.bulk.commit_group;" ::: "memory"); }
__device__ __forceinline__ void bulk_wait_read() { asm volatile("cp.async.bulk.wait_group.read 0;" ::: "memory"); }
__device__ __forceinline__ void bulk_wait_all() { asm volatile("cp.async.bulk.wait_group 0;" ::: "memory"); }
__device__ __forceinline__ void named_bar_sync(int id, int count) {
  asm volatile("bar.sync %0, %1;" ::"r"(id), "r"(count) : "memory");
}

template <typename T> __device__ __forceinline__ void ld4(const uint8_t* p, float (&v)[4]) {
  if constexpr (sizeof(T) == 4) {
    const float4 t = *reinterpret_cast<const float4*>(p);
    v[0] = t.x; v[1] = t.y; v[2] = t.z; v[3] = t.w;
  } else {
    const uint2 t = *reinterpret_cast<const uint2*>(p);
    const float2 a = __bfloat1622float2(*reinterpret_cast<const __nv_bfloat162*>(&t.x));
    const float2 b = __bfloat1622float2(*reinterpret_cast<const __nv_bfloat162*>(&t.y));
    v[0] = a.x; v[1] = a.y; v[2] = b.x; v[3] = b.y;
  }
}
template <typename T> __device__ __forceinline__ void st4(uint8_t* p, const float (&v)[4]) {
  if constexpr (sizeof(T) == 4) {
    *reinterpret_cast<float4*>(p) = make_float4(v[0], v[1], v[2], v[3]);
  } else {
    uint2 t;
    t.x = pack_bf16x2(v[0], v[1]); t.y = pack_bf16x2(v[2], v[3]);
    *reinterpret_cast<uint2*>(p) = t;
  }
}

template <typename TI, typename TO, int NCH, bool RESIDUAL, int RBT>
__global__ void __launch_bounds__(32 * (RBT * CG + 1), 1) ln_shift_bwd_stream_kernel(const LnStreamArgs a) {
  constexpr int CWT = RBT * CG;
  extern __shared__ __align__(128) uint8_t smem[];
  __shared__ __align__(8) uint64_t bars[2 * MAX_STAGES];
  __shared__ float red[CWT][128];
  const int warp = threadIdx.x >> 5, lane = threadIdx.x & 31;
  const int d = a.d, half = d >> 1;
  const uint32_t smem0 = smem_u32(smem);
  auto full_bar = [&](int s) { return smem_u32(&bars[s]); };
  auto done_bar = [&](int s) { return smem_u32(&bars[MAX_STAGES + s]); };
  const long long nchunks = a.T / RBT;
  const long long n_my = nchunks > blockIdx.x ? (nchunks - blockIdx.x + gridDim.x - 1) / gridDim.x : 0;
  const bool has_out = a.dout != nullptr;

  if (threadIdx.x == 0) {
    for (int s = 0; s < a.stages; ++s) { mbar_init(full_bar(s), 1); mbar_init(done_bar(s), RBT); }
    fence_barrier_init();
  }
  __syncthreads();

  if (warp == CWT) {
    const uint32_t xrow = d * (uint32_t)sizeof(TI), yrow = d * (uint32_t)sizeof(TO), rrow = d * 4u;
    const int dy_rows = a.shift ? RBT + 1 : RBT;
    const bool x_contig = a.ldx == d, dy_contig = a.lddy == d;
    uint32_t tx = RBT * xrow + 2 * RBT * 4u + (RESIDUAL ? RBT * rrow : 0u);
    for (long long it = 0; it < n_my + a.stages; ++it) {
      const int stage = (int)(it % a.stages);
      const uint32_t sbase = smem0 + stage * a.stage_bytes;
      if (it >= a.stages) {
        const long long t0 = (blockIdx.x + (it - a.stages) * gridDim.x) * RBT;
        mbar_wait(done_bar(stage), (uint32_t)((it / a.stages) - 1) & 1u);
        if (lane <= RBT) {
          bool issued = false;
          if (lane == RBT) {
            if constexpr (RESIDUAL) { bulk_store(a.dres + t0 * (long long)d, sbase + a.off_r, RBT * rrow); issued = true; }
          }
          if (issued) { bulk_commit(); bulk_wait_read(); }
        }
        __syncwarp();
      }
      if (it < n_my) {
        const long long t0 = (blockIdx.x + it * gridDim.x) * RBT;
        const int ny = (t0 + dy_rows <= a.T) ? dy_rows : RBT;
        if (lane == 0) mbar_expect_tx(full_bar(stage), tx + ny * yrow);
        __syncwarp();
        const uint32_t fb = full_bar(stage);
        if (lane < RBT) {
          const TI* xs = reinterpret_cast<const TI*>(a.x) + (t0 + lane) * a.ldx;
          if (!x_contig) bulk_load(sbase + lane * xrow, xs, xrow, fb);
          else if (lane == 0) bulk_load(sbase, xs, RBT * xrow, fb);
        } else if (lane < RBT + 9) {
          const int r = lane - RBT;
          const TO* ys = reinterpret_cast<const TO*>(a.dy) + (t0 + r) * a.lddy;
          if (!dy_contig) { if (r < ny) bulk_load(sbase + a.off_dy + r * yrow, ys, yrow, fb); }
          else if (r == 0) bulk_load(sbase + a.off_dy, ys, ny * yrow, fb);
        } else if (lane == RBT + 9) {
          bulk_load(sbase + a.off_stat, a.mean + t0, RBT * 4u, fb);
        } else if (lane == RBT + 10) {
          bulk_load(sbase + a.off_stat + RBT * 4u, a.rstd + t0, RBT * 4u, fb);
        } else if (lane == RBT + 11) {
          if constexpr (RESIDUAL) bulk_load(sbase + a.off_r, a.dres + t0 * (long long)d, RBT * rrow, fb);
        }
      }
    }
    if (lane <= RBT) bulk_wait_all();
    return;
  }

  constexpr bool SCREG = NCH <= 4;
  float ds_acc[NCH][4], cs_acc[RESIDUAL ? NCH : 1][4], sc[SCREG ? NCH : 1][4];
#pragma unroll
  for (int ch = 0; ch < NCH; ++ch) {
    const int c = ch * 128 + lane * 4;
#pragma unroll
    for (int i = 0; i < 4; ++i) {
      ds_acc[ch][i] = 0.f;
      if (RESIDUAL) cs_acc[RESIDUAL ? ch : 0][i] = 0.f;
      if constexpr (SCREG) sc[ch][i] = c < d ? a.scale[c + i] : 0.f;
    }
  }
  auto scale4 = [&](int ch, int c, float (&s4)[4]) {
    if constexpr (SCREG) {
#pragma unroll
      for (int i = 0; i < 4; ++i) s4[i] = sc[ch][i];
    } else {
      const float4 t = __ldg(reinterpret_cast<const float4*>(a.scale + c));
      s4[0] = t.x; s4[1] = t.y; s4[2] = t.z; s4[3] = t.w;
    }
  };
  const int group = warp / RBT, row = warp % RBT;
  constexpr bool KEEP = NCH <= 4;
  for (long long it = group; it < n_my; it += CG) {
    const int stage = (int)(it % a.stages);
    uint8_t* sb = smem + stage * a.stage_bytes;
    const long long t = (blockIdx.x + it * gridDim.x) * RBT + row;
    const bool has_next = (int)(t % a.seq_len) + 1 < a.seq_len;
    mbar_wait(full_bar(stage), (uint32_t)(it / a.stages) & 1u);
    const float mean = reinterpret_cast<const float*>(sb + a.off_stat)[row];
    const float rstd = reinterpret_cast<const float*>(sb + a.off_stat)[RBT + row];
    const uint8_t* xr = sb + (size_t)row * d * sizeof(TI);
    const uint8_t* yr = sb + a.off_dy + (size_t)row * d * sizeof(TO);
    const uint8_t* yn = yr + (size_t)d * sizeof(TO);
    float s1 = 0.f, s2 = 0.f;
    float kx[KEEP ? NCH : 1][4], kg[KEEP ? NCH : 1][4];
#pragma unroll
    for (int ch = 0; ch < NCH; ++ch) {
      const int c = ch * 128 + lane * 4;
      if (c < d) {
        float xv[4], g[4] = {0.f, 0.f, 0.f, 0.f};
        ld4<TI>(xr + c * sizeof(TI), xv);
        if (!a.shift || c >= half) ld4<TO>(yr + c * sizeof(TO), g);
        else if (has_next) ld4<TO>(yn + c * sizeof(TO), g);
        float s4[4];
        scale4(ch, c, s4);
#pragma unroll
        for (int i = 0; i < 4; ++i) {
          const float xh = (xv[i] - mean) * rstd;
          ds_acc[ch][i] += g[i] * xh;
          const float gs = g[i] * s4[i];
          s1 += gs; s2 += gs * xh;
          if constexpr (KEEP) { kx[ch][i] = xh; kg[ch][i] = gs; }
        }
      }
    }
    s1 = warp_sum(s1) / d;
    s2 = warp_sum(s2) / d;
    uint8_t* rr = sb + a.off_r + (size_t)row * d * 4;
    TO* orow = reinterpret_cast<TO*>(a.dout) + t * a.ldo;
#pragma unroll
    for (int ch = 0; ch < NCH; ++ch) {
      const int c = ch * 128 + lane * 4;
      if (c < d) {
        float o[4];
        if constexpr (KEEP) {
#pragma unroll
          for (int i = 0; i < 4; ++i) o[i] = rstd * (kg[ch][i] - s1 - kx[ch][i] * s2);
        } else {
          float xv[4], g[4] = {0.f, 0.f, 0.f, 0.f};
          ld4<TI>(xr + c * sizeof(TI), xv);
          if (!a.shift || c >= half) ld4<TO>(yr + c * sizeof(TO), g);
          else if (has_next) ld4<TO>(yn + c * sizeof(TO), g);
          float s4[4];
          scale4(ch, c, s4);
#pragma unroll
          for (int i = 0; i < 4; ++i) {
            const float xh = (xv[i] - mean) * rstd;
            o[i] = rstd * (g[i] * s4[i] - s1 - xh * s2);
          }
        }
        if constexpr (RESIDUAL) {
          float r[4];
          ld4<float>(rr + c * 4, r);
#pragma unroll
          for (int i = 0; i < 4; ++i) { r[i] += o[i]; cs_acc[ch][i] += r[i]; }
          st4<float>(rr + c * 4, r);
          if (has_out) st4<TO>(reinterpret_cast<uint8_t*>(orow + c), r);
        } else {
          st4<TO>(reinterpret_cast<uint8_t*>(orow + c), o);
        }
      }
    }
    fence_proxy_async();
    __syncwarp();
    if (lane == 0) mbar_arrive(done_bar(stage));
  }

#pragma unroll
  for (int ch = 0; ch < NCH; ++ch) {
    if (ch * 128 >= d) break;
#pragma unroll
    for (int pass = 0; pass < (RESIDUAL ? 2 : 1); ++pass) {
      float* dst = pass == 0 ? a.dscale : a.dres_colsum;
      if (dst == nullptr) continue;
#pragma unroll
      for (int i = 0; i < 4; ++i) red[warp][lane * 4 + i] = pass == 0 ? ds_acc[ch][i] : cs_acc[RESIDUAL ? ch : 0][i];
      named_bar_sync(1, 32 * CWT);
      if (threadIdx.x < 128) {
        float s = 0.f;
#pragma unroll
        for (int w = 0; w < CWT; ++w) s += red[w][threadIdx.x];
        const int c = ch * 128 + threadIdx.x;
        if (c < d) atomicAdd(dst + c, s);
      }
      named_bar_sync(1, 32 * CWT);
    }
  }
}

template <typename TI, typename TO, bool RESIDUAL>
int launch_stream(const LnStreamArgs& a, int smem_bytes, int rbt, cudaStream_t s) {
  const long long nchunks = a.T / rbt;
  const int grid = (int)(nchunks < pg_num_sms() ? nchunks : pg_num_sms());
  static bool attr_set = false;
  if (!attr_set) {
    PG_CUDA(cudaFuncSetAttribute(ln_shift_bwd_stream_kernel<TI, TO, 4, RESIDUAL, 8>, cudaFuncAttributeMaxDynamicSharedMemorySize, SMEM_BUDGET));
    PG_CUDA(cudaFuncSetAttribute(ln_shift_bwd_stream_kernel<TI, TO, 8, RESIDUAL, 8>, cudaFuncAttributeMaxDynamicSharedMemorySize, SMEM_BUDGET));
    PG_CUDA(cudaFuncSetAttribute(ln_shift_bwd_stream_kernel<TI, TO, 12, RESIDUAL, 4>, cudaFuncAttributeMaxDynamicSharedMemorySize, SMEM_BUDGET));
    PG_CUDA(cudaFuncSetAttribute(ln_shift_bwd_stream_kernel<TI, TO, 16, RESIDUAL, 4>, cudaFuncAttributeMaxDynamicSharedMemorySize, SMEM_BUDGET));
    attr_set = true;
  }
  if (a.d <= 512) ln_shift_bwd_stream_kernel<TI, TO, 4, RESIDUAL, 8><<<grid, 32 * (8 * CG + 1), smem_bytes, s>>>(a);
  else if (a.d <= 1024) ln_shift_bwd_stream_kernel<TI, TO, 8, RESIDUAL, 8><<<grid, 32 * (8 * CG + 1), smem_bytes, s>>>(a);
  else if (a.d <= 1536) ln_shift_bwd_stream_kernel<TI, TO, 12, RESIDUAL, 4><<<grid, 32 * (4 * CG + 1), smem_bytes, s>>>(a);
  else ln_shift_bwd_stream_kernel<TI, TO, 16, RESIDUAL, 4><<<grid, 32 * (4 * CG + 1), smem_bytes, s>>>(a);
  PG_LAUNCH_CHECK();
  return PROGEN_OK;
}

}

int ln_shift_bwd_stream_launch(const void* dy, long long lddy, int act_dtype, const void* x, long long ldx, int x_dtype,
                               const float* scale, const float* mean, const float* rstd, float* dres, void* dout,
                               long long ldo, float* dscale, float* dres_colsum, long long T, int d, int seq_len, int shift,
                               int residual, cudaStream_t stream) {
  static int enabled = [] { const char* e = getenv("PROGEN_LN_STREAM"); return e ? atoi(e) : 1; }();
  if (!enabled) return 1;
  const int so = act_dtype == PG_BF16 ? 2 : 4, si = x_dtype == PG_BF16 ? 2 : 4;
  const int rbt = d > 1024 ? 4 : RB;
  if (T % RB != 0 || T % seq_len != 0 || d % 128 != 0 || d > 2048 || T < 8 * RB) return 1;
  if ((lddy * so) % 16 || (ldx * si) % 16 || (ldo * so) % 16) return 1;
  if (((uintptr_t)dy | (uintptr_t)x | (uintptr_t)dout | (uintptr_t)dres | (uintptr_t)mean | (uintptr_t)rstd) % 16) return 1;
  LnStreamArgs a{};
  a.dy = dy; a.lddy = lddy; a.x = x; a.ldx = ldx; a.scale = scale; a.mean = mean; a.rstd = rstd; a.dres = dres;
  a.dout = dout; a.ldo = ldo; a.dscale = dscale; a.dres_colsum = residual ? dres_colsum : nullptr;
  a.T = T; a.d = d; a.seq_len = seq_len; a.shift = shift;
  auto up = [](int v) { return (v + 127) & ~127; };
  int off = up(rbt * d * si);
  a.off_dy = off; off += up((rbt + 1) * d * so);
  a.off_r = off; if (residual) off += up(rbt * d * 4);
  a.off_out = off;
  a.off_stat = off; off += 128;
  a.stage_bytes = off;
  a.stages = SMEM_BUDGET / a.stage_bytes;
  if (a.stages > MAX_STAGES) a.stages = MAX_STAGES;
  if (a.stages < 2) return 1;
  const int smem_bytes = a.stages * a.stage_bytes;
#define LNS(TI, TO, RES) return launch_stream<TI, TO, RES>(a, smem_bytes, rbt, stream)
  if (residual) {
    if (x_dtype != PG_F32) return 1;
    if (act_dtype == PG_F32) LNS(float, float, true);
    LNS(float, bf16, true);
  }
  if (act_dtype == PG_F32 && x_dtype == PG_F32) LNS(float, float, false);
  if (act_dtype == PG_BF16 && x_dtype == PG_BF16) LNS(bf16, bf16, false);
  if (act_dtype == PG_BF16 && x_dtype == PG_F32) LNS(float, bf16, false);
#undef LNS
  return 1;
}
```

### progen_b200/csrc/tc_ptx.cuh

```cuda
#pragma once
#include <cuda.h>
#include "common.cuh"

namespace tc {

__device__ __forceinline__ uint32_t smem_u32(const void* p) { return (uint32_t)__cvta_generic_to_shared(p); }

__device__ __forceinline__ void mbar_init(uint32_t bar, uint32_t count) {
  asm volatile("mbarrier.init.shared::cta.b64 [%0], %1;" ::"r"(bar), "r"(count) : "memory");
}
__device__ __forceinline__ void mbar_expect_tx(uint32_t bar, uint32_t bytes) {
  asm volatile("mbarrier.arrive.expect_tx.shared::cta.b64 _, [%0], %1;" ::"r"(bar), "r"(bytes) : "memory");
}
__device__ __forceinline__ void mbar_arrive(uint32_t bar) {
  asm volatile("mbarrier.arrive.shared::cta.b64 _, [%0];" ::"r"(bar) : "memory");
}
__device__ __forceinline__ void mbar_wait(uint32_t bar, uint32_t parity) {
  uint32_t ok = 0, spins = 0;
  do {
    asm volatile(
        "{\n\t.reg .pred p;\n\t"
        "mbarrier.try_wait.parity.shared::cta.b64 p, [%1], %2;\n\t"
        "selp.u32 %0, 1, 0, p;\n\t}"
        : "=r"(ok) : "r"(bar), "r"(parity) : "memory");
    if (!ok && ++spins > (1u << 26)) __trap();
  } while (!ok);
}
__device__ __forceinline__ void fence_barrier_init() { asm volatile("fence.mbarrier_init.release.cluster;" ::: "memory"); }
__device__ __forceinline__ void fence_proxy_async() { asm volatile("fence.proxy.async.shared::cta;" ::: "memory"); }

__device__ __forceinline__ void tma_load_2d(uint32_t dst, const CUtensorMap* map, uint32_t bar, int c0, int c1) {
  asm volatile(
      "cp.async.bulk.tensor.2d.shared::cluster.global.mbarrier::complete_tx::bytes [%0], [%1, {%3, %4}], [%2];"
      ::"r"(dst), "l"(map), "r"(bar), "r"(c0), "r"(c1) : "memory");
}
__device__ __forceinline__ void prefetch_tensormap(const CUtensorMap* map) {
  asm volatile("prefetch.tensormap [%0];" ::"l"(map) : "memory");
}

template <int COLS> __device__ __forceinline__ void tmem_alloc(uint32_t slot_smem_addr) {
  asm volatile("tcgen05.alloc.cta_group::1.sync.aligned.shared::cta.b32 [%0], %1;" ::"r"(slot_smem_addr), "n"(COLS) : "memory");
  asm volatile("tcgen05.relinquish_alloc_permit.cta_group::1.sync.aligned;" ::: "memory");
}
template <int COLS> __device__ __forceinline__ void tmem_dealloc(uint32_t taddr) {
  asm volatile("tcgen05.dealloc.cta_group::1.sync.aligned.b32 %0, %1;" ::"r"(taddr), "n"(COLS) : "memory");
}
__device__ __forceinline__ void tcgen05_commit(uint32_t bar) {
  asm volatile("tcgen05.commit.cta_group::1.mbarrier::arrive::one.shared::cluster.b64 [%0];" ::"r"(bar) : "memory");
}
__device__ __forceinline__ void tcgen05_fence_before() { asm volatile("tcgen05.fence::before_thread_sync;" ::: "memory"); }
__device__ __forceinline__ void tcgen05_fence_after() { asm volatile("tcgen05.fence::after_thread_sync;" ::: "memory"); }

__device__ __forceinline__ void umma_bf16(uint32_t d_tmem, uint64_t adesc, uint64_t bdesc, uint32_t idesc, uint32_t accum) {
  asm volatile(
      "{\n\t.reg .pred p;\n\t"
      "setp.ne.b32 p, %4, 0;\n\t"
      "tcgen05.mma.cta_group::1.kind::f16 [%0], %1, %2, %3, p;\n\t}"
      ::"r"(d_tmem), "l"(adesc), "l"(bdesc), "r"(idesc), "r"(accum) : "memory");
}

__device__ __forceinline__ void tmem_ld32(uint32_t taddr, float (&v)[32]) {
  uint32_t r[32];
  asm volatile(
      "tcgen05.ld.sync.aligned.32x32b.x32.b32 "
      "{%0, %1, %2, %3, %4, %5, %6, %7, %8, %9, %10, %11, %12, %13, %14, %15, "
      "%16, %17, %18, %19, %20, %21, %22, %23, %24, %25, %26, %27, %28, %29, %30, %31}, [%32];"
      : "=r"(r[0]), "=r"(r[1]), "=r"(r[2]), "=r"(r[3]), "=r"(r[4]), "=r"(r[5]), "=r"(r[6]), "=r"(r[7]),
        "=r"(r[8]), "=r"(r[9]), "=r"(r[10]), "=r"(r[11]), "=r"(r[12]), "=r"(r[13]), "=r"(r[14]), "=r"(r[15]),
        "=r"(r[16]), "=r"(r[17]), "=r"(r[18]), "=r"(r[19]), "=r"(r[20]), "=r"(r[21]), "=r"(r[22]), "=r"(r[23]),
        "=r"(r[24]), "=r"(r[25]), "=r"(r[26]), "=r"(r[27]), "=r"(r[28]), "=r"(r[29]), "=r"(r[30]), "=r"(r[31])
      : "r"(taddr));
  asm volatile("tcgen05.wait::ld.sync.aligned;" ::: "memory");
#pragma unroll
  for (int i = 0; i < 32; ++i) v[i] = __uint_as_float(r[i]);
}

__device__ __forceinline__ void tmem_ld32_issue(uint32_t taddr, uint32_t (&r)[32]) {
  asm volatile(
      "tcgen05.ld.sync.aligned.32x32b.x32.b32 {%0, %1, %2, %3, %4, %5, %6, %7, %8, %9, %10, %11, %12, %13, %14, %15, %16, %17, %18, %19, %20, %21, %22, %23, %24, %25, %26, %27, %28, %29, %30, %31}, [%32];"
      : "=r"(r[0]), "=r"(r[1]), "=r"(r[2]), "=r"(r[3]), "=r"(r[4]), "=r"(r[5]), "=r"(r[6]), "=r"(r[7]), "=r"(r[8]), "=r"(r[9]), "=r"(r[10]), "=r"(r[11]), "=r"(r[12]), "=r"(r[13]), "=r"(r[14]), "=r"(r[15]), "=r"(r[16]), "=r"(r[17]), "=r"(r[18]), "=r"(r[19]), "=r"(r[20]), "=r"(r[21]), "=r"(r[22]), "=r"(r[23]), "=r"(r[24]), "=r"(r[25]), "=r"(r[26]), "=r"(r[27]), "=r"(r[28]), "=r"(r[29]), "=r"(r[30]), "=r"(r[31])
      : "r"(taddr));
}
__device__ __forceinline__ void tmem_ld32_wait(uint32_t (&r)[32]) {
  asm volatile("tcgen05.wait::ld.sync.aligned;" : "+r"(r[0]), "+r"(r[1]), "+r"(r[2]), "+r"(r[3]), "+r"(r[4]), "+r"(r[5]), "+r"(r[6]), "+r"(r[7]), "+r"(r[8]), "+r"(r[9]), "+r"(r[10]), "+r"(r[11]), "+r"(r[12]), "+r"(r[13]), "+r"(r[14]), "+r"(r[15]), "+r"(r[16]), "+r"(r[17]), "+r"(r[18]), "+r"(r[19]), "+r"(r[20]), "+r"(r[21]), "+r"(r[22]), "+r"(r[23]), "+r"(r[24]), "+r"(r[25]), "+r"(r[26]), "+r"(r[27]), "+r"(r[28]), "+r"(r[29]), "+r"(r[30]), "+r"(r[31]) :: "memory");
}

__device__ __forceinline__ void tmem_ld64(uint32_t taddr, float (&v)[64]) {
  uint32_t r[64];
  asm volatile(
      "tcgen05.ld.sync.aligned.32x32b.x64.b32 {%0, %1, %2, %3, %4, %5, %6, %7, %8, %9, %10, %11, %12, %13, %14, %15, %16, %17, %18, %19, %20, %21, %22, %23, %24, %25, %26, %27, %28, %29, %30, %31, %32, %33, %34, %35, %36, %37, %38, %39, %40, %41, %42, %43, %44, %45, %46, %47, %48, %49, %50, %51, %52, %53, %54, %55, %56, %57, %58, %59, %60, %61, %62, %63}, [%64];"
      : "=r"(r[0]), "=r"(r[1]), "=r"(r[2]), "=r"(r[3]), "=r"(r[4]), "=r"(r[5]), "=r"(r[6]), "=r"(r[7]), "=r"(r[8]), "=r"(r[9]), "=r"(r[10]), "=r"(r[11]), "=r"(r[12]), "=r"(r[13]), "=r"(r[14]), "=r"(r[15]), "=r"(r[16]), "=r"(r[17]), "=r"(r[18]), "=r"(r[19]), "=r"(r[20]), "=r"(r[21]), "=r"(r[22]), "=r"(r[23]), "=r"(r[24]), "=r"(r[25]), "=r"(r[26]), "=r"(r[27]), "=r"(r[28]), "=r"(r[29]), "=r"(r[30]), "=r"(r[31]), "=r"(r[32]), "=r"(r[33]), "=r"(r[34]), "=r"(r[35]), "=r"(r[36]), "=r"(r[37]), "=r"(r[38]), "=r"(r[39]), "=r"(r[40]), "=r"(r[41]), "=r"(r[42]), "=r"(r[43]), "=r"(r[44]), "=r"(r[45]), "=r"(r[46]), "=r"(r[47]), "=r"(r[48]), "=r"(r[49]), "=r"(r[50]), "=r"(r[51]), "=r"(r[52]), "=r"(r[53]), "=r"(r[54]), "=r"(r[55]), "=r"(r[56]), "=r"(r[57]), "=r"(r[58]), "=r"(r[59]), "=r"(r[60]), "=r"(r[61]), "=r"(r[62]), "=r"(r[63])
      : "r"(taddr));
  asm volatile("tcgen05.wait::ld.sync.aligned;" ::: "memory");
#pragma unroll
  for (int i = 0; i < 64; ++i) v[i] = __uint_as_float(r[i]);
}

__device__ __forceinline__ void tmem_ld32x2(uint32_t taddr_a, uint32_t taddr_b, float (&a)[32], float (&b)[32]) {
  uint32_t ra[32], rb[32];
  asm volatile(
      "tcgen05.ld.sync.aligned.32x32b.x32.b32 {%0, %1, %2, %3, %4, %5, %6, %7, %8, %9, %10, %11, %12, %13, %14, %15, %16, %17, %18, %19, %20, %21, %22, %23, %24, %25, %26, %27, %28, %29, %30, %31}, [%64];\n\t"
      "tcgen05.ld.sync.aligned.32x32b.x32.b32 {%32, %33, %34, %35, %36, %37, %38, %39, %40, %41, %42, %43, %44, %45, %46, %47, %48, %49, %50, %51, %52, %53, %54, %55, %56, %57, %58, %59, %60, %61, %62, %63}, [%65];\n\t"
      "tcgen05.wait::ld.sync.aligned;"
      : "=r"(ra[0]), "=r"(ra[1]), "=r"(ra[2]), "=r"(ra[3]), "=r"(ra[4]), "=r"(ra[5]), "=r"(ra[6]), "=r"(ra[7]), "=r"(ra[8]), "=r"(ra[9]), "=r"(ra[10]), "=r"(ra[11]), "=r"(ra[12]), "=r"(ra[13]), "=r"(ra[14]), "=r"(ra[15]), "=r"(ra[16]), "=r"(ra[17]), "=r"(ra[18]), "=r"(ra[19]), "=r"(ra[20]), "=r"(ra[21]), "=r"(ra[22]), "=r"(ra[23]), "=r"(ra[24]), "=r"(ra[25]), "=r"(ra[26]), "=r"(ra[27]), "=r"(ra[28]), "=r"(ra[29]), "=r"(ra[30]), "=r"(ra[31]), "=r"(rb[0]), "=r"(rb[1]), "=r"(rb[2]), "=r"(rb[3]), "=r"(rb[4]), "=r"(rb[5]), "=r"(rb[6]), "=r"(rb[7]), "=r"(rb[8]), "=r"(rb[9]), "=r"(rb[10]), "=r"(rb[11]), "=r"(rb[12]), "=r"(rb[13]), "=r"(rb[14]), "=r"(rb[15]), "=r"(rb[16]), "=r"(rb[17]), "=r"(rb[18]), "=r"(rb[19]), "=r"(rb[20]), "=r"(rb[21]), "=r"(rb[22]), "=r"(rb[23]), "=r"(rb[24]), "=r"(rb[25]), "=r"(rb[26]), "=r"(rb[27]), "=r"(rb[28]), "=r"(rb[29]), "=r"(rb[30]), "=r"(rb[31])
      : "r"(taddr_a), "r"(taddr_b) : "memory");
#pragma unroll
  for (int i = 0; i < 32; ++i) { a[i] = __uint_as_float(ra[i]); b[i] = __uint_as_float(rb[i]); }
}

template <bool MN_MAJOR>
__device__ __forceinline__ uint64_t make_smem_desc(uint32_t smem_addr, uint32_t lbo_bytes = 8192) {
  uint64_t d = 0;
  d |= (uint64_t)((smem_addr & 0x3FFFF) >> 4);
  d |= (uint64_t)(MN_MAJOR ? (lbo_bytes >> 4) : 1) << 16;
  d |= (uint64_t)(1024 >> 4) << 32;
  d |= (uint64_t)1 << 46;
  d |= (uint64_t)2 << 61;
  return d;
}
__device__ __forceinline__ constexpr uint32_t make_idesc(int M, int N, bool a_mn, bool b_mn) {
  return (1u << 4) | (1u << 7) | (1u << 10) | ((a_mn ? 1u : 0u) << 15) | ((b_mn ? 1u : 0u) << 16) |
         ((uint32_t)(N >> 3) << 17) | ((uint32_t)(M >> 4) << 24);
}

__device__ __forceinline__ void tma_store_2d(const CUtensorMap* map, uint32_t src, int c0, int c1) {
  asm volatile("cp.async.bulk.tensor.2d.global.shared::cta.bulk_group [%0, {%2, %3}], [%1];"
               ::"l"(map), "r"(src), "r"(c0), "r"(c1) : "memory");
}
__device__ __forceinline__ void tma_reduce_add_2d(const CUtensorMap* map, uint32_t src, int c0, int c1) {
  asm volatile("cp.reduce.async.bulk.tensor.2d.global.shared::cta.add.tile.bulk_group [%0, {%2, %3}], [%1];"
               ::"l"(map), "r"(src), "r"(c0), "r"(c1) : "memory");
}
__device__ __forceinline__ void bulk_commit_group() { asm volatile("cp.async.bulk.commit_group;" ::: "memory"); }
template <int N> __device__ __forceinline__ void bulk_wait_group_read() {
  asm volatile("cp.async.bulk.wait_group.read %0;" ::"n"(N) : "memory");
}
template <int N> __device__ __forceinline__ void bulk_wait_group() {
  asm volatile("cp.async.bulk.wait_group %0;" ::"n"(N) : "memory");
}

__device__ __forceinline__ void umma_bf16_ts(uint32_t d_tmem, uint32_t a_tmem, uint64_t bdesc, uint32_t idesc, uint32_t accum) {
  asm volatile(
      "{\n\t.reg .pred p;\n\t"
      "setp.ne.b32 p, %4, 0;\n\t"
      "tcgen05.mma.cta_group::1.kind::f16 [%0], [%1], %2, %3, p;\n\t}"
      ::"r"(d_tmem), "r"(a_tmem), "l"(bdesc), "r"(idesc), "r"(accum) : "memory");
}
__device__ __forceinline__ void tmem_cp_128x256b(uint32_t taddr, uint64_t sdesc) {
  asm volatile("tcgen05.cp.cta_group::1.128x256b [%0], %1;" ::"r"(taddr), "l"(sdesc) : "memory");
}
template <int N> __device__ __forceinline__ void tmem_st(uint32_t taddr, const uint32_t (&r)[N]);
template <> __device__ __forceinline__ void tmem_st<8>(uint32_t taddr, const uint32_t (&r)[8]) {
  asm volatile("tcgen05.st.sync.aligned.32x32b.x8.b32 [%0], {%1, %2, %3, %4, %5, %6, %7, %8};"
               ::"r"(taddr), "r"(r[0]), "r"(r[1]), "r"(r[2]), "r"(r[3]), "r"(r[4]), "r"(r[5]), "r"(r[6]), "r"(r[7]) : "memory");
}
template <> __device__ __forceinline__ void tmem_st<16>(uint32_t taddr, const uint32_t (&r)[16]) {
  asm volatile("tcgen05.st.sync.aligned.32x32b.x16.b32 [%0], {%1, %2, %3, %4, %5, %6, %7, %8, %9, %10, %11, %12, %13, %14, %15, %16};"
               ::"r"(taddr), "r"(r[0]), "r"(r[1]), "r"(r[2]), "r"(r[3]), "r"(r[4]), "r"(r[5]), "r"(r[6]), "r"(r[7]), "r"(r[8]), "r"(r[9]), "r"(r[10]), "r"(r[11]), "r"(r[12]), "r"(r[13]), "r"(r[14]), "r"(r[15]) : "memory");
}
template <> __device__ __forceinline__ void tmem_st<32>(uint32_t taddr, const uint32_t (&r)[32]) {
  asm volatile("tcgen05.st.sync.aligned.32x32b.x32.b32 [%0], {%1, %2, %3, %4, %5, %6, %7, %8, %9, %10, %11, %12, %13, %14, %15, %16, %17, %18, %19, %20, %21, %22, %23, %24, %25, %26, %27, %28, %29, %30, %31, %32};"
               ::"r"(taddr), "r"(r[0]), "r"(r[1]), "r"(r[2]), "r"(r[3]), "r"(r[4]), "r"(r[5]), "r"(r[6]), "r"(r[7]), "r"(r[8]), "r"(r[9]), "r"(r[10]), "r"(r[11]), "r"(r[12]), "r"(r[13]), "r"(r[14]), "r"(r[15]), "r"(r[16]), "r"(r[17]), "r"(r[18]), "r"(r[19]), "r"(r[20]), "r"(r[21]), "r"(r[22]), "r"(r[23]), "r"(r[24]), "r"(r[25]), "r"(r[26]), "r"(r[27]), "r"(r[28]), "r"(r[29]), "r"(r[30]), "r"(r[31]) : "memory");
}
__device__ __forceinline__ void tmem_st_wait() { asm volatile("tcgen05.wait::st.sync.aligned;" ::: "memory"); }
__device__ __forceinline__ void tmem_ld_wait() { asm volatile("tcgen05.wait::ld.sync.aligned;" ::: "memory"); }

__device__ __forceinline__ float2 ffma2(float2 a, float2 b, float2 c) {
  float2 d;
  asm("fma.rn.f32x2 %0, %1, %2, %3;" : "=l"(reinterpret_cast<uint64_t&>(d))
      : "l"(reinterpret_cast<uint64_t&>(a)), "l"(reinterpret_cast<uint64_t&>(b)), "l"(reinterpret_cast<uint64_t&>(c)));
  return d;
}
__device__ __forceinline__ float2 fadd2(float2 a, float2 b) {
  float2 d;
  asm("add.rn.f32x2 %0, %1, %2;" : "=l"(reinterpret_cast<uint64_t&>(d))
      : "l"(reinterpret_cast<uint64_t&>(a)), "l"(reinterpret_cast<uint64_t&>(b)));
  return d;
}
__device__ __forceinline__ float2 fmul2(float2 a, float2 b) {
  float2 d;
  asm("mul.rn.f32x2 %0, %1, %2;" : "=l"(reinterpret_cast<uint64_t&>(d))
      : "l"(reinterpret_cast<uint64_t&>(a)), "l"(reinterpret_cast<uint64_t&>(b)));
  return d;
}
__device__ __forceinline__ float fmax3(float a, float b, float c) {
  float d;
  asm("max.f32 %0, %1, %2, %3;" : "=f"(d) : "f"(a), "f"(b), "f"(c));
  return d;
}
__device__ __forceinline__ float ex2f(float x) {
  float y;
  asm("ex2.approx.ftz.f32 %0, %1;" : "=f"(y) : "f"(x));
  return y;
}
__device__ __forceinline__ float ex2_poly(float x) {
  x = fmaxf(x, -126.f);
  float r;
  asm("add.rm.ftz.f32 %0, %1, %2;" : "=f"(r) : "f"(x), "f"(12582912.f));
  const float f = x - (r - 12582912.f);
  float p = fmaf(0.07711908966302872f, f, 0.22756439447402954f);
  p = fmaf(p, f, 0.6951461434364319f);
  p = fmaf(p, f, 1.0f);
  return __uint_as_float(__float_as_uint(p) + (__float_as_uint(r) << 23));
}
__device__ __forceinline__ bool elect_one() {
  uint32_t pred = 0;
  asm volatile("{\n\t.reg .pred P1;\n\telect.sync _|P1, 0xffffffff;\n\tselp.u32 %0, 1, 0, P1;\n\t}" : "=r"(pred));
  return pred != 0;
}
template <int REGS> __device__ __forceinline__ void setmaxnreg_inc() { asm volatile("setmaxnreg.inc.sync.aligned.u32 %0;" ::"n"(REGS)); }
template <int REGS> __device__ __forceinline__ void setmaxnreg_dec() { asm volatile("setmaxnreg.dec.sync.aligned.u32 %0;" ::"n"(REGS)); }

}

int pg_tensor_map_2d_bf16(const void* ptr, uint64_t inner, uint64_t outer, uint64_t row_stride_elems, uint32_t box_inner,
                          uint32_t box_outer, CUtensorMap* out);
int pg_tensor_map_2d(const void* ptr, uint32_t elem_bytes, uint64_t inner, uint64_t outer, uint64_t row_stride_elems,
                     uint32_t box_inner, uint32_t box_outer, uint32_t swizzle_bytes, CUtensorMap* out);

namespace tc2 {

__device__ __forceinline__ uint32_t cluster_ctarank() {
  uint32_t r;
  asm volatile("mov.u32 %0, %%cluster_ctarank;" : "=r"(r));
  return r;
}
__device__ __forceinline__ void cluster_sync() {
  asm volatile("barrier.cluster.arrive.release.aligned;" ::: "memory");
  asm volatile("barrier.cluster.wait.acquire.aligned;" ::: "memory");
}
__device__ __forceinline__ uint32_t mapa(uint32_t smem_addr, uint32_t rank) {
  uint32_t r;
  asm volatile("mapa.shared::cluster.u32 %0, %1, %2;" : "=r"(r) : "r"(smem_addr), "r"(rank));
  return r;
}
__device__ __forceinline__ void mbar_arrive_cluster(uint32_t cluster_addr) {
  asm volatile("mbarrier.arrive.relaxed.cluster.shared::cluster.b64 _, [%0];" ::"r"(cluster_addr) : "memory");
}
__device__ __forceinline__ void tma_load_2d_pair(uint32_t dst, const CUtensorMap* map, uint32_t bar_cluster_addr, int c0, int c1) {
  asm volatile(
      "cp.async.bulk.tensor.2d.cta_group::2.shared::cluster.global.mbarrier::complete_tx::bytes [%0], [%1, {%3, %4}], [%2];"
      ::"r"(dst), "l"(map), "r"(bar_cluster_addr), "r"(c0), "r"(c1) : "memory");
}
__device__ __forceinline__ void tma_load_2d_pair_mc(uint32_t dst, const CUtensorMap* map, uint32_t bar_own_addr, uint16_t cta_mask,
                                                    int c0, int c1) {
  asm volatile(
      "cp.async.bulk.tensor.2d.cta_group::2.shared::cluster.global.mbarrier::complete_tx::bytes.multicast::cluster"
      " [%0], [%1, {%4, %5}], [%2], %3;"
      ::"r"(dst), "l"(map), "r"(bar_own_addr & 0xFEFFFFFFu), "h"(cta_mask), "r"(c0), "r"(c1) : "memory");
}
template <int COLS> __device__ __forceinline__ void tmem_alloc_pair(uint32_t slot_smem_addr) {
  asm volatile("tcgen05.alloc.cta_group::2.sync.aligned.shared::cta.b32 [%0], %1;" ::"r"(slot_smem_addr), "n"(COLS) : "memory");
  asm volatile("tcgen05.relinquish_alloc_permit.cta_group::2.sync.aligned;" ::: "memory");
}
template <int COLS> __device__ __forceinline__ void tmem_dealloc_pair(uint32_t taddr) {
  asm volatile("tcgen05.dealloc.cta_group::2.sync.aligned.b32 %0, %1;" ::"r"(taddr), "n"(COLS) : "memory");
}
__device__ __forceinline__ void tcgen05_commit_pair(uint32_t bar, uint16_t cta_mask = 3) {
  asm volatile("tcgen05.commit.cta_group::2.mbarrier::arrive::one.shared::cluster.multicast::cluster.b64 [%0], %1;"
               ::"r"(bar), "h"(cta_mask) : "memory");
}
__device__ __forceinline__ void umma_bf16_pair(uint32_t d_tmem, uint64_t adesc, uint64_t bdesc, uint32_t idesc, uint32_t accum) {
  asm volatile(
      "{\n\t.reg .pred p;\n\t"
      "setp.ne.b32 p, %4, 0;\n\t"
      "tcgen05.mma.cta_group::2.kind::f16 [%0], %1, %2, %3, p;\n\t}"
      ::"r"(d_tmem), "l"(adesc), "l"(bdesc), "r"(idesc), "r"(accum) : "memory");
}

}
```

### progen_b200/engine.py

```python
import math
import numpy as np
import torch

from . import lib as L

P = 'pro_gen_base/~/'
ALIGN = 64


def layer_kinds(depth, global_mlp_depth, ff_glu):
    out = []
    for i in range(depth):
        use_gmlp = (depth - i) <= global_mlp_depth
        out.append('sgu' if use_gmlp else ('glu' if ff_glu else 'gelu'))
    return out


class ParamSpec:
    __slots__ = ('module', 'name', 'shape', 'decay', 'interleave', 'offset', 'size')

    def __init__(self, module, name, shape, interleave=False):
        self.module, self.name, self.shape = module, name, tuple(shape)
        self.decay = len(shape) > 1
        self.interleave = interleave
        self.size = int(np.prod(shape))
        self.offset = -1


def build_param_specs(cfg):
    d, V, n = cfg['dim'], cfg['num_tokens'], cfg['seq_len']
    inner = cfg['heads'] * cfg['dim_head']
    hid = d * cfg['ff_mult']
    specs = [ParamSpec(P + 'embed', 'embeddings', (V, d))]
    for i, kind in enumerate(layer_kinds(cfg['depth'], cfg['global_mlp_depth'], cfg['ff_glu'])):
        a = P + f'attn{i}/~/'
        specs += [ParamSpec(a + 'layer_norm', 'scale', (d,)),
                  ParamSpec(a + 'linear', 'w', (d, 3 * inner)),
                  ParamSpec(a + 'linear_1', 'w', (inner, d)), ParamSpec(a + 'linear_1', 'b', (d,))]
        f = P + f'ff{i}/~/'
        h_in = hid * 2 if kind == 'glu' else hid
        h_out = hid // 2 if kind == 'sgu' else hid
        glu = kind == 'glu'
        specs += [ParamSpec(f + 'layer_norm', 'scale', (d,)),
                  ParamSpec(f + 'linear', 'w', (d, h_in), interleave=glu), ParamSpec(f + 'linear', 'b', (h_in,), interleave=glu)]
        if kind == 'sgu':
            half = hid // 2
            specs += [ParamSpec(f + 'sgu/~/layer_norm', 'scale', (half,)),
                      ParamSpec(f + 'sgu', 'spatial_weights', (n, n)), ParamSpec(f + 'sgu', 'spatial_biases', (n, 1)),
                      ParamSpec(f + 'sgu/~/linear', 'w', (half, half)), ParamSpec(f + 'sgu/~/linear', 'b', (half,))]
        specs += [ParamSpec(f + 'linear_1', 'w', (h_out, d)), ParamSpec(f + 'linear_1', 'b', (d,))]
    specs += [ParamSpec(P + 'layer_norm', 'scale', (d,)),
              ParamSpec(P + 'linear', 'w', (d, V)), ParamSpec(P + 'linear', 'b', (V,))]
    off = 0
    for s in [s for s in specs if s.decay] + [s for s in specs if not s.decay]:
        s.offset = off
        off += (s.size + ALIGN - 1) // ALIGN * ALIGN
    n_decay = sum((s.size + ALIGN - 1) // ALIGN * ALIGN for s in specs if s.decay)
    return specs, off, n_decay


def _interleave(a):
    H = a.shape[-1] // 2
    return np.stack((a[..., :H], a[..., H:]), axis=-1).reshape(a.shape)


def _deinterleave(a):
    return np.concatenate((a[..., 0::2], a[..., 1::2]), axis=-1)


class Engine:
    def __init__(self, cfg, mixed_precision=False, device=None):
        L.require_device()
        self.cfg = cfg
        self.dev = torch.device('cuda', torch.cuda.current_device()) if device is None else torch.device(device)
        self.mp = bool(mixed_precision)
        self.act = torch.bfloat16 if self.mp else torch.float32
        self.act_dt = L.BF16 if self.mp else L.F32
        self.backend = L.BACKEND_TC if self.mp else L.BACKEND_SIMT
        self.kinds = layer_kinds(cfg['depth'], cfg['global_mlp_depth'], cfg['ff_glu'])
        self.attn_tc = self.mp
        import os
        self.attn_fwd_kind = os.environ.get('PROGEN_ATTN_FWD', 'tcgen05')
        self.attn_bwd_kind = os.environ.get('PROGEN_ATTN_BWD', 'tcgen05')
        if cfg['window_size'] % 128 != 0:
            self.attn_fwd_kind = self.attn_bwd_kind = 'mma'
        d, n, w = cfg['dim'], cfg['seq_len'], cfg['window_size']
        self.d, self.n, self.w, self.V = d, n, w, cfg['num_tokens']
        self.h, self.dh = cfg['heads'], cfg['dim_head']
        self.I = self.h * self.dh
        self.hid = d * cfg['ff_mult']
        if n % w != 0:
            raise L.ProgenError('sequence length must be divisible by the window size')
        if self.dh not in (16, 32, 64, 128):
            raise L.ProgenError('dim_head must be one of 16/32/64/128')
        if d % 8 or self.I % 8 or self.V % 8:
            raise L.ProgenError('dim, heads*dim_head and num_tokens must be multiples of 8')
        if self.V > 384:
            raise L.ProgenError('num_tokens > 384 is not supported (embed_bwd keeps num_tokens x 32 fp32 bins in 48 KB of shared memory)')
        if self.mp and self.dh != 64:
            raise L.ProgenError(f'mixed_precision needs dim_head == 64 (got {self.dh}); use mixed_precision=False for other head sizes')
        if self.mp and w % 64:
            raise L.ProgenError(f'mixed_precision needs window_size % 64 == 0 (got {w}); use mixed_precision=False')
        if self.mp:
            bad = [k for k, v in dict(dim=d, inner=self.I, seq_len=n, num_tokens=self.V).items() if v % 64]
            if bad:
                raise L.ProgenError(f'mixed_precision (tcgen05 path) needs {bad} to be multiples of 64')
        self.specs, self.n_params_padded, self.n_decay = build_param_specs(cfg)
        self.by_key = {(s.module, s.name): s for s in self.specs}
        self.num_params = sum(s.size for s in self.specs)
        f32 = dict(device=self.dev, dtype=torch.float32)
        self.params = torch.zeros(self.n_params_padded, **f32)
        self.grads = torch.zeros(self.n_params_padded, **f32)
        self.params_lp = torch.zeros(self.n_params_padded, device=self.dev, dtype=torch.bfloat16) if self.mp else None
        self.wm = {}
        for i, kind in enumerate(self.kinds):
            if kind == 'sgu':
                self.wm[i] = torch.zeros(n, n, device=self.dev, dtype=self.act)
        inv_freq = 1.0 / (10000 ** (np.arange(0, self.dh, 2, dtype=np.float64) / self.dh))
        ang = np.arange(n, dtype=np.float64)[:, None] * inv_freq[None, :]
        self.rot_sin = torch.tensor(np.sin(ang), **f32).contiguous()
        self.rot_cos = torch.tensor(np.cos(ang), **f32).contiguous()
        self.rot_sin_t = self.rot_sin.t().contiguous()
        self.rot_cos_t = self.rot_cos.t().contiguous()
        self.B = 0
        self.loss = torch.zeros(1, device=self.dev)
        self.loaded_token = None
        self.on_layer_grads = None
        self.lib = L.load()

    def layer_grad_range(self, i):
        pre = (P + f'attn{i}/~/', P + f'ff{i}/~/')
        segs = [s for s in self.specs if s.decay and s.module.startswith(pre)]
        return min(s.offset for s in segs), max(s.offset + (s.size + ALIGN - 1) // ALIGN * ALIGN for s in segs)

    def seg(self, buf, module, name):
        s = self.by_key[(module, name)]
        return buf[s.offset:s.offset + s.size]

    def load_params(self, params):
        host = np.zeros(self.n_params_padded, np.float32)
        for s in self.specs:
            a = params[s.module][s.name]
            a = a.detach().cpu().numpy() if isinstance(a, torch.Tensor) else np.asarray(a)
            a = a.astype(np.float32)
            if a.shape != s.shape:
                raise L.ProgenError(f'{s.module}/{s.name}: expected shape {s.shape}, got {a.shape}')
            if s.interleave:
                a = _interleave(a)
            host[s.offset:s.offset + s.size] = a.ravel()
        self.params.copy_(torch.from_numpy(host))
        self.refresh_compute_copies()

    def export_tree(self, buf):
        host = buf.detach().float().cpu().numpy()
        out = {}
        for s in self.specs:
            a = host[s.offset:s.offset + s.size].reshape(s.shape).copy()
            if s.interleave:
                a = _deinterleave(a)
            out.setdefault(s.module, {})[s.name] = a
        return out

    def export_params(self):
        return self.export_tree(self.params)

    def export_grads(self):
        return self.export_tree(self.grads)

    def refresh_compute_copies(self):
        st = L.stream()
        if self.mp:
            L.check(self.lib.progen_cast_f32(self.params.data_ptr(), self.params_lp.data_ptr(), L.BF16, self.n_params_padded, st),
                    'cast params')
        self.refresh_masked_copies()

    def refresh_masked_copies(self):
        st = L.stream()
        for i, wm in self.wm.items():
            src = self.seg(self.params, P + f'ff{i}/~/sgu', 'spatial_weights')
            L.check(self.lib.progen_tril_cast(src.data_ptr(), wm.data_ptr(), self.act_dt, self.n, st), 'tril_cast')

    def W(self, module, name):
        return self.seg(self.params_lp if self.mp else self.params, module, name)

    def Pf(self, module, name):
        return self.seg(self.params, module, name)

    def G(self, module, name):
        return self.seg(self.grads, module, name)

    def ensure_batch(self, B):
        if B == self.B:
            return
        self.B = B
        self.alloc_epoch = getattr(self, 'alloc_epoch', 0) + 1
        T = B * self.n
        self.T = T
        d, I, hid = self.d, self.I, self.hid
        dev, act = self.dev, self.act
        A = lambda *shape: torch.empty(*shape, device=dev, dtype=act)
        F = lambda *shape: torch.empty(*shape, device=dev, dtype=torch.float32)
        nl = len(self.kinds)
        self.tok = torch.empty(T, device=dev, dtype=torch.int32)
        self.labels = torch.empty(T, device=dev, dtype=torch.int32)
        self.X = [F(T, d) for _ in range(2 * nl + 1)]
        self.lay = []
        for kind in self.kinds:
            s = dict(mean1=F(T), rstd1=F(T), y1=A(T, d), qkv=A(T, 3 * I), att=A(T, I), lse=F(T, self.h),
                     mean2=F(T), rstd2=F(T), y2=A(T, d))
            if kind == 'glu':
                s.update(u=A(T, 2 * hid), hact=A(T, hid))
            else:
                s.update(u=A(T, hid), hact=A(T, hid))
            if kind == 'sgu':
                half = hid // 2
                s.update(mean3=F(T), rstd3=F(T), gn=A(T, half), gp=A(T, half), sg=A(T, half), pj=A(T, half))
            self.lay.append(s)
        self.meanf, self.rstdf, self.yf = F(T), F(T), A(T, d)
        self.logits = F(T, self.V)
        self.dlogits = A(T, self.V)
        self.ce_w = F(T)
        self.dres = F(T, d)
        self.dres_lp = A(T, d) if self.mp else self.dres
        self.dy = A(T, d)
        self.dqkv = A(T, 3 * I)
        self.datt = A(T, I)
        self.delta = F(T, self.h)
        self.du = A(T, 2 * hid)
        self.dh_ = A(T, hid)
        half = hid // 2
        if 'sgu' in self.kinds:
            self.dpj, self.dsg, self.dgp, self.dgn = A(T, half), A(T, half), A(T, half), A(T, half)

    def _mm(self, **kw):
        L.gemm(backend=self.backend, in_dtype=self.act_dt, **kw)

    def fwd_gemm(self, x, K, w, N, out, epi=L.EPI_STORE, out_dtype=None, **kw):
        self._mm(M=self.T, N=N, K=K, A=x, lda=K, B=w, ldb=N, b_mn=True, out=out, ldo=kw.pop('ldo', N), epi=epi,
                 out_dtype=self.act_dt if out_dtype is None else out_dtype, **kw)

    def dgrad_gemm(self, dy, N_out, w, K_in, out, epi=L.EPI_STORE, **kw):
        self._mm(M=self.T, N=K_in, K=N_out, A=dy, lda=N_out, B=w, ldb=N_out, out=out, ldo=kw.pop('ldo', K_in), epi=epi,
                 out_dtype=self.act_dt, **kw)

    def wgrad_gemm(self, x, K_in, dy, N_out, dw):
        split = 1
        if self.backend == L.BACKEND_TC:
            bn = 256 if (N_out % 256 == 0) else 128
            tiles = ((K_in + 127) // 128) * ((N_out + bn - 1) // bn)
            split = max(1, min(self.T // 64, 148 // tiles))
        self._mm(M=K_in, N=N_out, K=self.T, A=x, lda=K_in, a_mn=True, B=dy, ldb=N_out, b_mn=True, out=dw, ldo=N_out,
                 epi=L.EPI_ACCUM, out_dtype=L.F32, split_k=split, atomic=split > 1)

    def colsum(self, t, N, out, ld=None):
        L.check(self.lib.progen_colsum(t.data_ptr(), N if ld is None else ld, L.dt(t), out.data_ptr(), self.T, N, L.stream()), 'colsum')

    def ln_fwd(self, x, ldx, scale, y, ldy, mean, rstd, dcols, shift):
        L.check(self.lib.progen_ln_shift_fwd(x.data_ptr(), ldx, L.dt(x), scale.data_ptr(), y.data_ptr(), ldy, L.dt(y),
                                             mean.data_ptr(), rstd.data_ptr(), self.T, dcols, self.n, int(shift), L.stream()), 'ln_fwd')

    def forward(self, ids):
        B = ids.shape[0]
        self.ensure_batch(B)
        self.tok.copy_(torch.as_tensor(ids).reshape(-1).to(device=self.dev, dtype=torch.int32), non_blocking=True)
        self._forward_device()
        return self.logits

    def _forward_device(self):
        lib, st = self.lib, L.stream()
        cfg, d, I, hid, T, n = self.cfg, self.d, self.I, self.hid, self.T, self.n
        shift = cfg['shift_tokens']
        L.check(lib.progen_embed_fwd(self.tok.data_ptr(), self.Pf(P + 'embed', 'embeddings').data_ptr(), self.X[0].data_ptr(),
                                     T, d, self.V, st), 'embed_fwd')
        for i, kind in enumerate(self.kinds):
            s = self.lay[i]
            a, f = P + f'attn{i}/~/', P + f'ff{i}/~/'
            x0, x1, x2 = self.X[2 * i], self.X[2 * i + 1], self.X[2 * i + 2]
            self.ln_fwd(x0, d, self.Pf(a + 'layer_norm', 'scale'), s['y1'], d, s['mean1'], s['rstd1'], d, shift)
            self.fwd_gemm(s['y1'], d, self.W(a + 'linear', 'w'), 3 * I, s['qkv'], epi=L.EPI_ROTARY, rot_sin=self.rot_sin,
                          rot_cos=self.rot_cos, seq_len=n, dim_head=self.dh)
            self.attn_fwd(s['qkv'], s['att'], s['lse'])
            self.fwd_gemm(s['att'], I, self.W(a + 'linear_1', 'w'), d, x1, epi=L.EPI_RESIDUAL, bias=self.Pf(a + 'linear_1', 'b'),
                          aux=x0, ldaux=d)
            self.ln_fwd(x1, d, self.Pf(f + 'layer_norm', 'scale'), s['y2'], d, s['mean2'], s['rstd2'], d, shift)
            if kind == 'glu':
                self.fwd_gemm(s['y2'], d, self.W(f + 'linear', 'w'), 2 * hid, s['hact'], epi=L.EPI_GLU, ldo=hid, out2=s['u'],
                              ldo2=2 * hid, bias=self.Pf(f + 'linear', 'b'))
                last, last_k = s['hact'], hid
            else:
                self.fwd_gemm(s['y2'], d, self.W(f + 'linear', 'w'), hid, s['hact'], epi=L.EPI_GELU, out2=s['u'], ldo2=hid,
                              bias=self.Pf(f + 'linear', 'b'))
                last, last_k = s['hact'], hid
            if kind == 'sgu':
                half = hid // 2
                g = f + 'sgu'
                gate = s['hact'][:, half:]
                self.ln_fwd(gate, hid, self.Pf(g + '/~/layer_norm', 'scale'), s['gn'], half, s['mean3'], s['rstd3'], half, False)
                self._mm(M=n, N=half, K=n, A=self.wm[i], lda=n, B=s['gn'], ldb=half, b_mn=True, out=s['gp'], ldo=half,
                         out_dtype=self.act_dt, batch=self.B, b_batch_rows=n, d_batch_rows=n, causal=1)
                L.check(lib.progen_sgu_gate_fwd(s['hact'].data_ptr(), hid, s['gp'].data_ptr(), half,
                                                self.Pf(g, 'spatial_biases').data_ptr(), s['sg'].data_ptr(), half, self.act_dt,
                                                T, half, n, st), 'sgu_gate_fwd')
                self.fwd_gemm(s['sg'], half, self.W(g + '/~/linear', 'w'), half, s['pj'], bias=self.Pf(g + '/~/linear', 'b'))
                last, last_k = s['pj'], half
            self.fwd_gemm(last, last_k, self.W(f + 'linear_1', 'w'), d, x2, epi=L.EPI_RESIDUAL, bias=self.Pf(f + 'linear_1', 'b'),
                          aux=x1, ldaux=d)
        xl = self.X[-1]
        self.ln_fwd(xl, d, self.Pf(P + 'layer_norm', 'scale'), self.yf, d, self.meanf, self.rstdf, d, False)
        self.fwd_gemm(self.yf, d, self.W(P + 'linear', 'w'), self.V, self.logits, bias=self.Pf(P + 'linear', 'b'), out_dtype=L.F32)

    def attn_fwd(self, qkv, out, lse):
        if self.attn_tc:
            if self.attn_fwd_kind == 'tcgen05':
                L.check(self.lib.progen_local_attn_fwd_tc(qkv.data_ptr(), out.data_ptr(), lse.data_ptr(), self.B, self.n, self.w,
                                                          self.h, self.dh, L.stream()), 'local_attn_fwd_tc')
                return
            L.check(self.lib.progen_local_attn_fwd(qkv.data_ptr(), out.data_ptr(), lse.data_ptr(), self.B, self.n, self.w, self.h,
                                                   self.dh, L.stream()), 'local_attn_fwd')
            return
        L.check(self.lib.progen_local_attn_fwd_simt(qkv.data_ptr(), out.data_ptr(), lse.data_ptr(), self.act_dt, self.B, self.n,
                                                    self.w, self.h, self.dh, L.stream()), 'local_attn_fwd')

    def attn_bwd(self, qkv, out, dout, lse, dqkv):
        if self.attn_tc:
            if self.attn_bwd_kind == 'tcgen05':
                L.check(self.lib.progen_local_attn_bwd_tc_ex(qkv.data_ptr(), out.data_ptr(), dout.data_ptr(), lse.data_ptr(),
                                                             dqkv.data_ptr(), self.delta.data_ptr(), self.rot_sin.data_ptr(),
                                                             self.rot_cos.data_ptr(), self.rot_sin_t.data_ptr(),
                                                             self.rot_cos_t.data_ptr(), self.B, self.n, self.w, self.h, self.dh, -1,
                                                             L.stream()), 'local_attn_bwd')
                return
            L.check(self.lib.progen_local_attn_bwd(qkv.data_ptr(), out.data_ptr(), dout.data_ptr(), lse.data_ptr(), dqkv.data_ptr(),
                                                   self.delta.data_ptr(), self.rot_sin.data_ptr(), self.rot_cos.data_ptr(), self.B,
                                                   self.n, self.w, self.h, self.dh, L.stream()), 'local_attn_bwd')
            return
        L.check(self.lib.progen_local_attn_bwd_simt(qkv.data_ptr(), out.data_ptr(), dout.data_ptr(), lse.data_ptr(), dqkv.data_ptr(),
                                                    self.delta.data_ptr(), self.act_dt, self.B, self.n, self.w, self.h, self.dh,
                                                    L.stream()), 'local_attn_bwd')

    def loss_and_grad(self, data, global_batch=None, zero_grads=True):
        B = self.load_batch(data)
        self.step_device(global_batch or B, zero_grads)
        return self.loss

    def load_batch(self, data):
        data = torch.as_tensor(np.asarray(data).astype(np.int32) if not isinstance(data, torch.Tensor) else data)
        B = data.shape[0]
        self.ensure_batch(B)
        dd = data.to(device=self.dev, dtype=torch.int32, non_blocking=True)
        self.tok.copy_(dd[:, :-1].reshape(-1))
        self.labels.copy_(dd[:, 1:].reshape(-1))
        return B

    def step_device(self, global_batch, zero_grads=True):
        self._forward_device()
        lib, st = self.lib, L.stream()
        self.loss.zero_()
        if zero_grads:
            self.grads.zero_()
        L.check(lib.progen_ce_fwd_bwd(self.logits.data_ptr(), L.F32, self.labels.data_ptr(), self.ce_w.data_ptr(),
                                      self.loss.data_ptr(), self.dlogits.data_ptr(), self.act_dt, self.B, self.n, self.V,
                                      1.0 / global_batch, st), 'ce_fwd_bwd')
        self._backward_device()

    def ln_bwd_res(self, dy, x, scale, mean, rstd, dscale, shift, next_bias_grad=None):
        L.check(self.lib.progen_ln_shift_bwd(dy.data_ptr(), self.d, self.act_dt, x.data_ptr(), self.d, L.F32, scale.data_ptr(),
                                             mean.data_ptr(), rstd.data_ptr(), self.dres.data_ptr(),
                                             self.dres_lp.data_ptr() if self.mp else 0, self.d, dscale.data_ptr(),
                                             L.ptr(next_bias_grad), self.T, self.d, self.n, int(shift), 1, L.stream()), 'ln_bwd')

    def _backward_device(self):
        lib, st = self.lib, L.stream()
        cfg, d, I, hid, T, n = self.cfg, self.d, self.I, self.hid, self.T, self.n
        shift = cfg['shift_tokens']
        hw, hl = P + 'linear', P + 'layer_norm'
        self.colsum(self.dlogits, self.V, self.G(hw, 'b'))
        self.wgrad_gemm(self.yf, d, self.dlogits, self.V, self.G(hw, 'w'))
        self.dgrad_gemm(self.dlogits, self.V, self.W(hw, 'w'), d, self.dy)
        self.dres.zero_()
        nl = len(self.kinds)
        self.ln_bwd_res(self.dy, self.X[-1], self.Pf(hl, 'scale'), self.meanf, self.rstdf, self.G(hl, 'scale'), False,
                        next_bias_grad=self.G(P + f'ff{nl - 1}/~/linear_1', 'b'))
        for i in reversed(range(len(self.kinds))):
            kind, s = self.kinds[i], self.lay[i]
            a, f = P + f'attn{i}/~/', P + f'ff{i}/~/'
            x0, x1 = self.X[2 * i], self.X[2 * i + 1]
            dres_lp = self.dres_lp
            if kind == 'sgu':
                half = hid // 2
                g = f + 'sgu'
                self.wgrad_gemm(s['pj'], half, dres_lp, d, self.G(f + 'linear_1', 'w'))
                self.dgrad_gemm(dres_lp, d, self.W(f + 'linear_1', 'w'), half, self.dpj)
                self.colsum(self.dpj, half, self.G(g + '/~/linear', 'b'))
                self.wgrad_gemm(s['sg'], half, self.dpj, half, self.G(g + '/~/linear', 'w'))
                self.dgrad_gemm(self.dpj, half, self.W(g + '/~/linear', 'w'), half, self.dsg)
                da = self.dh_
                L.check(lib.progen_sgu_gate_bwd(self.dsg.data_ptr(), half, s['hact'].data_ptr(), hid, s['gp'].data_ptr(), half,
                                                self.Pf(g, 'spatial_biases').data_ptr(), da.data_ptr(), hid, self.dgp.data_ptr(),
                                                half, self.G(g, 'spatial_biases').data_ptr(), self.act_dt, T, half, n, st),
                        'sgu_gate_bwd')
                self._mm(M=n, N=n, K=half, A=self.dgp, lda=half, B=s['gn'], ldb=half, out=self.G(g, 'spatial_weights'), ldo=n,
                         epi=L.EPI_ACCUM, out_dtype=L.F32, batch=self.B, a_batch_rows=n, b_batch_rows=n, batch_reduce=True,
                         atomic=True, tril=True, tril_rows=n)
                self._mm(M=n, N=half, K=n, A=self.wm[i], lda=n, a_mn=True, B=self.dgp, ldb=half, b_mn=True, out=self.dgn,
                         ldo=half, out_dtype=self.act_dt, batch=self.B, b_batch_rows=n, d_batch_rows=n, causal=2)
                gate = s['hact'][:, half:]
                L.check(lib.progen_ln_shift_bwd(self.dgn.data_ptr(), half, self.act_dt, gate.data_ptr(), hid, self.act_dt,
                                                self.Pf(g + '/~/layer_norm', 'scale').data_ptr(), s['mean3'].data_ptr(),
                                                s['rstd3'].data_ptr(), 0, da[:, half:].data_ptr(), hid,
                                                self.G(g + '/~/layer_norm', 'scale').data_ptr(), 0, T, half, n, 0, 0, st), 'ln_bwd_sgu')
                L.check(lib.progen_gelu_bwd(da.data_ptr(), s['u'].data_ptr(), self.act_dt, T * hid, st), 'gelu_bwd')
                du, n_in = da, hid
            elif kind == 'glu':
                self.wgrad_gemm(s['hact'], hid, dres_lp, d, self.G(f + 'linear_1', 'w'))
                self.dgrad_gemm(dres_lp, d, self.W(f + 'linear_1', 'w'), hid, self.du, epi=L.EPI_GLU_BWD, ldo=2 * hid,
                                aux=s['u'], ldaux=2 * hid)
                du, n_in = self.du, 2 * hid
            else:
                self.wgrad_gemm(s['hact'], hid, dres_lp, d, self.G(f + 'linear_1', 'w'))
                self.dgrad_gemm(dres_lp, d, self.W(f + 'linear_1', 'w'), hid, self.dh_, epi=L.EPI_GELU_BWD, aux=s['u'], ldaux=hid)
                du, n_in = self.dh_, hid
            self.colsum(du, n_in, self.G(f + 'linear', 'b'))
            self.wgrad_gemm(s['y2'], d, du, n_in, self.G(f + 'linear', 'w'))
            self.dgrad_gemm(du, n_in, self.W(f + 'linear', 'w'), d, self.dy)
            self.ln_bwd_res(self.dy, x1, self.Pf(f + 'layer_norm', 'scale'), s['mean2'], s['rstd2'], self.G(f + 'layer_norm', 'scale'), shift,
                            next_bias_grad=self.G(a + 'linear_1', 'b'))
            self.wgrad_gemm(s['att'], I, dres_lp, d, self.G(a + 'linear_1', 'w'))
            self.dgrad_gemm(dres_lp, d, self.W(a + 'linear_1', 'w'), I, self.datt)
            self.attn_bwd(s['qkv'], s['att'], self.datt, s['lse'], self.dqkv)
            if not self.attn_tc:
                L.check(lib.progen_rotary_bwd(self.dqkv.data_ptr(), 3 * I, self.act_dt, self.rot_sin.data_ptr(),
                                              self.rot_cos.data_ptr(), T, 3 * I, n, self.dh, st), 'rotary_bwd')
            self.wgrad_gemm(s['y1'], d, self.dqkv, 3 * I, self.G(a + 'linear', 'w'))
            self.dgrad_gemm(self.dqkv, 3 * I, self.W(a + 'linear', 'w'), d, self.dy)
            self.ln_bwd_res(self.dy, x0, self.Pf(a + 'layer_norm', 'scale'), s['mean1'], s['rstd1'], self.G(a + 'layer_norm', 'scale'), shift,
                            next_bias_grad=self.G(P + f'ff{i - 1}/~/linear_1', 'b') if i > 0 else None)
            if self.on_layer_grads is not None:
                self.on_layer_grads(i)
        L.check(lib.progen_embed_bwd(self.tok.data_ptr(), self.dres.data_ptr(), self.G(P + 'embed', 'embeddings').data_ptr(),
                                     T, d, self.V, st), 'embed_bwd')
```

### progen_b200/lib.py

```python
import ctypes as C
import os
import torch

F32, BF16 = 0, 1
BACKEND_SIMT, BACKEND_TC = 0, 1
EPI_STORE, EPI_ROTARY, EPI_RESIDUAL, EPI_GLU, EPI_GELU, EPI_GLU_BWD, EPI_GELU_BWD, EPI_ACCUM = range(8)

_HERE = os.path.dirname(os.path.abspath(__file__))
LIB_PATH = os.path.join(_HERE, 'libprogen_b200.so')


class ProgenError(RuntimeError):
    pass


class GemmDesc(C.Structure):
    _fields_ = [
        ('M', C.c_int32), ('N', C.c_int32), ('K', C.c_int32),
        ('a_mn_major', C.c_int32), ('b_mn_major', C.c_int32),
        ('batch', C.c_int32), ('batch_reduce', C.c_int32), ('causal', C.c_int32), ('split_k', C.c_int32),
        ('in_dtype', C.c_int32), ('out_dtype', C.c_int32), ('epi_kind', C.c_int32), ('backend', C.c_int32),
        ('seq_len', C.c_int32), ('dim_head', C.c_int32),
        ('atomic', C.c_int32), ('tril', C.c_int32), ('tril_rows', C.c_int32),
        ('lda', C.c_int64), ('ldb', C.c_int64),
        ('a_batch_rows', C.c_int64), ('b_batch_rows', C.c_int64), ('d_batch_rows', C.c_int64),
        ('ldo', C.c_int64), ('ldo2', C.c_int64), ('ldaux', C.c_int64),
        ('A', C.c_void_p), ('B', C.c_void_p), ('out', C.c_void_p), ('out2', C.c_void_p),
        ('bias', C.c_void_p), ('aux', C.c_void_p), ('rot_sin', C.c_void_p), ('rot_cos', C.c_void_p),
    ]


_lib = None

_LL, _I, _P, _F = C.c_longlong, C.c_int, C.c_void_p, C.c_float

PROTOTYPES = {
    'progen_version': [],
    'progen_last_error': [],
    'progen_device_check': [],
    'progen_launch_count': [],
    'progen_gemm': [C.POINTER(GemmDesc), _P],
    'progen_embed_fwd': [_P, _P, _P, _LL, _I, _I, _P],
    'progen_embed_bwd': [_P, _P, _P, _LL, _I, _I, _P],
    'progen_ln_shift_fwd': [_P, _LL, _I, _P, _P, _LL, _I, _P, _P, _LL, _I, _I, _I, _P],
    'progen_ln_shift_bwd': [_P, _LL, _I, _P, _LL, _I, _P, _P, _P, _P, _P, _LL, _P, _P, _LL, _I, _I, _I, _I, _P],
    'progen_colsum': [_P, _LL, _I, _P, _LL, _I, _P],
    'progen_ce_fwd_bwd': [_P, _I, _P, _P, _P, _P, _I, _I, _I, _I, _F, _P],
    'progen_rotary_bwd': [_P, _LL, _I, _P, _P, _LL, _I, _I, _I, _P],
    'progen_local_attn_fwd_simt': [_P, _P, _P, _I, _I, _I, _I, _I, _I, _P],
    'progen_local_attn_bwd_simt': [_P, _P, _P, _P, _P, _P, _I, _I, _I, _I, _I, _I, _P],
    'progen_local_attn_fwd': [_P, _P, _P, _I, _I, _I, _I, _I, _P],
    'progen_local_attn_fwd_tc': [_P, _P, _P, _I, _I, _I, _I, _I, _P],
    'progen_local_attn_bwd': [_P, _P, _P, _P, _P, _P, _P, _P, _I, _I, _I, _I, _I, _P],
    'progen_local_attn_bwd_tc': [_P, _P, _P, _P, _P, _P, _P, _P, _I, _I, _I, _I, _I, _P],
    'progen_local_attn_bwd_tc_ex': [_P, _P, _P, _P, _P, _P, _P, _P, _P, _P, _I, _I, _I, _I, _I, _I, _P],
    'progen_sgu_gate_fwd': [_P, _LL, _P, _LL, _P, _P, _LL, _I, _LL, _I, _I, _P],
    'progen_sgu_gate_bwd': [_P, _LL, _P, _LL, _P, _LL, _P, _P, _LL, _P, _LL, _P, _I, _LL, _I, _I, _P],
    'progen_gelu_bwd': [_P, _P, _I, _LL, _P],
    'progen_cast_f32': [_P, _P, _I, _LL, _P],
    'progen_tril_cast': [_P, _P, _I, _I, _P],
    'progen_decode_step': [_P, _I, _P],
    'progen_decode_run': [_P, _P],
    'progen_optim_workspace_floats': [],
    'progen_grad_sqnorm': [_P, _LL, _P, _P, _P],
    'progen_adamw_step': [_P, _P, _P, _P, _P, _P, _LL, _LL, _P, _F, _F, _F, _F, _F, _F, _LL, _I, _P],
    'progen_adamw_step_dev': [_P, _P, _P, _P, _P, _P, _LL, _LL, _P, _F, _F, _F, _F, _F, _F, _I, _P, _P],
}
_RESTYPES = {'progen_version': C.c_char_p, 'progen_last_error': C.c_char_p, 'progen_launch_count': C.c_longlong}


def load():
    global _lib
    if _lib is not None:
        return _lib
    if not os.path.exists(LIB_PATH):
        raise ProgenError(f'{LIB_PATH} not found: run `python -c "import __graft_entry__ as g; g.build()"` '
                          f'(or progen_b200/csrc/build.sh). There is no CPU fallback.')
    lib = C.CDLL(LIB_PATH)
    for name, argtypes in PROTOTYPES.items():
        fn = getattr(lib, name)
        fn.argtypes = argtypes
        fn.restype = _RESTYPES.get(name, C.c_int)
    _lib = lib
    return lib


def version():
    return load().progen_version().decode()


def check(rc, what=''):
    if rc != 0:
        raise ProgenError(f'{what} failed (code {rc}): {load().progen_last_error().decode()}')


def require_device():
    if not torch.cuda.is_available():
        raise ProgenError('no CUDA device: progen_b200 has no CPU fallback (sm_100a only)')
    check(load().progen_device_check(), 'progen_device_check')


def dt(t):
    if t.dtype == torch.float32:
        return F32
    if t.dtype == torch.bfloat16:
        return BF16
    raise ProgenError(f'unsupported dtype {t.dtype}')


def ptr(t):
    return 0 if t is None else t.data_ptr()


def stream():
    return torch.cuda.current_stream().cuda_stream


def gemm(*, M, N, K, A, lda, B, ldb, out, ldo, epi=EPI_STORE, backend, a_mn=False, b_mn=False, in_dtype, out_dtype=F32,
         batch=1, a_batch_rows=0, b_batch_rows=0, d_batch_rows=0, batch_reduce=False, causal=0, split_k=1,
         out2=None, ldo2=0, bias=None, aux=None, ldaux=0, rot_sin=None, rot_cos=None, seq_len=0, dim_head=0,
         atomic=False, tril=False, tril_rows=0):
    d = GemmDesc()
    d.M, d.N, d.K = M, N, K
    d.a_mn_major, d.b_mn_major = int(a_mn), int(b_mn)
    d.batch, d.batch_reduce, d.causal, d.split_k = batch, int(batch_reduce), causal, split_k
    d.in_dtype, d.out_dtype, d.epi_kind, d.backend = in_dtype, out_dtype, epi, backend
    d.seq_len, d.dim_head = seq_len, dim_head
    d.atomic, d.tril, d.tril_rows = int(atomic), int(tril), tril_rows
    d.lda, d.ldb = lda, ldb
    d.a_batch_rows, d.b_batch_rows, d.d_batch_rows = a_batch_rows, b_batch_rows, d_batch_rows
    d.ldo, d.ldo2, d.ldaux = ldo, ldo2, ldaux
    as_ptr = lambda x: x if isinstance(x, int) else ptr(x)
    d.A, d.B, d.out, d.out2 = as_ptr(A), as_ptr(B), as_ptr(out), as_ptr(out2)
    d.bias, d.aux, d.rot_sin, d.rot_cos = as_ptr(bias), as_ptr(aux), as_ptr(rot_sin), as_ptr(rot_cos)
    check(load().progen_gemm(C.byref(d), stream()), 'progen_gemm')
```

Before: 1.862 million.

## Fuse bias-gradient colsum into wgrad GEMM and GELU backward into SGU/LN kernels

Adds an optional colsum output to the tcgen05 wgrad GEMM. Two otherwise idle warps read the B tiles already staged in shared memory and atomically accumulate per-column sums, so the separate colsum pass over dy goes away. Also folds the GELU backward multiply into the SGU gate backward and LN-shift backward kernels, removing a separate elementwise pass over the hidden activations. The cost is extra empty-barrier arrivals and cross-cluster sync in the GEMM pipeline, which could stall the producer, plus more atomics.

```diff
diff --git a/include/progen_b200.h b/include/progen_b200.h
--- a/include/progen_b200.h
+++ b/include/progen_b200.h
@@ -47,6 +47,7 @@
   const void* aux;
   const float* rot_sin;
   const float* rot_cos;
+  float* colsum;
 } progen_gemm_t;
 
 int progen_gemm(const progen_gemm_t* desc, void* stream);
@@ -60,6 +61,10 @@
                         const float* scale, const float* mean, const float* rstd, float* dres, void* dout, long long ldo,
                         float* dscale, float* dres_colsum, long long T, int d, int seq_len, int shift, int residual,
                         void* stream);
+int progen_ln_shift_bwd_ex(const void* dy, long long lddy, int act_dtype, const void* x, long long ldx, int x_dtype,
+                           const float* scale, const float* mean, const float* rstd, float* dres, void* dout, long long ldo,
+                           float* dscale, float* dres_colsum, const void* gelu_u, long long ldu, long long T, int d, int seq_len,
+                           int shift, int residual, void* stream);
 
 int progen_colsum(const void* in, long long ld, int dtype, float* out, long long T, int N, void* stream);
 
@@ -96,6 +101,9 @@
 int progen_sgu_gate_bwd(const void* ds, long long ldds, const void* xs, long long ldx, const void* gp, long long ldg,
                         const float* bias, void* dxs, long long lddx, void* dgp, long long lddg, float* dbias, int dtype,
                         long long T, int C, int seq_len, void* stream);
+int progen_sgu_gate_bwd_ex(const void* ds, long long ldds, const void* xs, long long ldx, const void* gp, long long ldg,
+                           const float* bias, void* dxs, long long lddx, void* dgp, long long lddg, float* dbias,
+                           const void* gelu_u, long long ldu, int dtype, long long T, int C, int seq_len, void* stream);
 int progen_gelu_bwd(void* da, const void* u, int dtype, long long numel, void* stream);
 int progen_cast_f32(const float* in, void* out, int out_dtype, long long numel, void* stream);
 int progen_tril_cast(const float* w, void* out, int out_dtype, int n, void* stream);
diff --git a/progen_b200/csrc/api.cu b/progen_b200/csrc/api.cu
--- a/progen_b200/csrc/api.cu
+++ b/progen_b200/csrc/api.cu
@@ -53,6 +53,15 @@
   if (g.epi_kind == EPI_GLU || g.epi_kind == EPI_GELU) PG_CHECK_ARG(g.epi.out2 != nullptr && g.epi.bias != nullptr);
   if (g.epi_kind == EPI_GLU_BWD || g.epi_kind == EPI_GELU_BWD) PG_CHECK_ARG(g.epi.aux != nullptr);
   if (g.epi_kind == EPI_ROTARY) PG_CHECK_ARG(g.epi.rot_sin && g.epi.rot_cos && d->seq_len > 0 && d->dim_head > 0 && d->dim_head % 2 == 0);
+  g.epi.colsum = d->colsum;
+  if (g.epi.colsum) {
+    PG_CHECK_ARG(g.epi_kind == EPI_ACCUM && g.b_mn_major && g.batch == 1 && !g.batch_reduce);
+    if (!(d->backend == PROGEN_BACKEND_TCGEN05 && gemm_tc2_eligible(g))) {
+      const int rc = progen_colsum(g.B, g.ldb, g.in_dtype, g.epi.colsum, g.K, g.N, stream);
+      if (rc) return rc;
+      g.epi.colsum = nullptr;
+    }
+  }
   if (d->backend == PROGEN_BACKEND_TCGEN05) return gemm_tc_launch(g, (cudaStream_t)stream);
   if (d->backend == PROGEN_BACKEND_SIMT) return gemm_simt_launch(g, (cudaStream_t)stream);
   progen_set_error("progen_gemm: unknown backend %d", d->backend);
diff --git a/progen_b200/csrc/elementwise.cu b/progen_b200/csrc/elementwise.cu
--- a/progen_b200/csrc/elementwise.cu
+++ b/progen_b200/csrc/elementwise.cu
@@ -3,8 +3,8 @@
 
 int ln_shift_bwd_stream_launch(const void* dy, long long lddy, int act_dtype, const void* x, long long ldx, int x_dtype,
                                const float* scale, const float* mean, const float* rstd, float* dres, void* dout,
-                               long long ldo, float* dscale, float* dres_colsum, long long T, int d, int seq_len, int shift,
-                               int residual, cudaStream_t stream);
+                               long long ldo, float* dscale, float* dres_colsum, const void* gelu_u, long long ldu, long long T,
+                               int d, int seq_len, int shift, int residual, cudaStream_t stream);
 
 namespace {
 
@@ -29,6 +29,17 @@
   uint2 t;
   t.x = pack_bf16x2(v[0], v[1]); t.y = pack_bf16x2(v[2], v[3]);
   *reinterpret_cast<uint2*>(p) = t;
+}
+
+template <typename T> __device__ __forceinline__ float round_to(float v) {
+  if constexpr (sizeof(T) == 2) return __bfloat162float(__float2bfloat16_rn(v));
+  else return v;
+}
+template <typename TO> __device__ __forceinline__ void gelu_bwd_post(const TO* u, float (&o)[4]) {
+  float x[4];
+  load4<TO>(u, x);
+#pragma unroll
+  for (int j = 0; j < 4; ++j) o[j] = round_to<TO>(o[j]) * gelu_tanh_grad(x[j]);
 }
 
 __global__ void embed_fwd_kernel(const int* __restrict__ tok, const float* __restrict__ table, float* __restrict__ x,
@@ -113,7 +124,7 @@
                                     const float* __restrict__ scale, const float* __restrict__ mean_in,
                                     const float* __restrict__ rstd_in, float* __restrict__ dres, TO* __restrict__ dout,
                                     long long ldo, float* __restrict__ dscale, float* __restrict__ dres_colsum,
-                                    long long T, int d, int seq_len, int shift) {
+                                    const TO* __restrict__ gelu_u, long long ldu, long long T, int d, int seq_len, int shift) {
   const int lane = threadIdx.x & 31, warp = threadIdx.x >> 5;
   const int half = d >> 1;
   float ds_acc[NCH][4];
@@ -170,6 +181,7 @@
             store4(dres + t * (long long)d + c, rr[ch]);
             if (dout) store4(dout + t * ldo + c, rr[ch]);
           } else {
+            if (gelu_u) gelu_bwd_post<TO>(gelu_u + t * ldu + c, o);
             store4(dout + t * ldo + c, o);
           }
         }
@@ -218,6 +230,7 @@
           store4(dres + t * (long long)d + c, r);
           if (dout) store4(dout + t * ldo + c, r);
         } else {
+          if (gelu_u) gelu_bwd_post<TO>(gelu_u + t * ldu + c, o);
           store4(dout + t * ldo + c, o);
         }
       }
@@ -394,7 +407,8 @@
 __global__ void sgu_gate_bwd_kernel(const TO* __restrict__ ds, long long ldds, const TO* __restrict__ xs, long long ldx,
                                     const TO* __restrict__ gp, long long ldg, const float* __restrict__ bias,
                                     TO* __restrict__ dxs, long long lddx, TO* __restrict__ dgp, long long lddg,
-                                    float* __restrict__ dbias, long long T, int C, int seq_len) {
+                                    float* __restrict__ dbias, const TO* __restrict__ gelu_u, long long ldu, long long T,
+                                    int C, int seq_len) {
   const int lane = threadIdx.x & 31, warp = threadIdx.x >> 5;
   for (long long t = blockIdx.x * (long long)ROWS_PER_BLOCK + warp; t < T; t += (long long)gridDim.x * ROWS_PER_BLOCK) {
     const int m = (int)(t % seq_len);
@@ -411,6 +425,7 @@
         o2[j] = d[j] * x[j];
         acc += o2[j];
       }
+      if (gelu_u) gelu_bwd_post<TO>(gelu_u + t * ldu + c, o1);
       store4(dxs + t * lddx + c, o1);
       store4(dgp + t * lddg + c, o2);
     }
@@ -506,17 +521,26 @@
                         const float* scale, const float* mean, const float* rstd, float* dres, void* dout, long long ldo,
                         float* dscale, float* dres_colsum, long long T, int d, int seq_len, int shift, int residual,
                         void* stream) {
+  return progen_ln_shift_bwd_ex(dy, lddy, act_dtype, x, ldx, x_dtype, scale, mean, rstd, dres, dout, ldo, dscale, dres_colsum,
+                                nullptr, 0, T, d, seq_len, shift, residual, stream);
+}
+
+int progen_ln_shift_bwd_ex(const void* dy, long long lddy, int act_dtype, const void* x, long long ldx, int x_dtype,
+                           const float* scale, const float* mean, const float* rstd, float* dres, void* dout, long long ldo,
+                           float* dscale, float* dres_colsum, const void* gelu_u, long long ldu, long long T, int d, int seq_len,
+                           int shift, int residual, void* stream) {
   PG_CHECK_ARG(T > 0 && d % 8 == 0 && d <= 4096 && seq_len > 0 && T % seq_len == 0);
   PG_CHECK_ARG(residual ? (dres != nullptr && x_dtype == PG_F32) : (dout != nullptr));
+  PG_CHECK_ARG(gelu_u == nullptr || (!residual && ldu % 4 == 0));
   cudaStream_t s = (cudaStream_t)stream;
   const int rc_stream = ln_shift_bwd_stream_launch(dy, lddy, act_dtype, x, ldx, x_dtype, scale, mean, rstd, dres, dout, ldo,
-                                                   dscale, dres_colsum, T, d, seq_len, shift, residual, s);
+                                                   dscale, dres_colsum, gelu_u, ldu, T, d, seq_len, shift, residual, s);
   if (rc_stream <= 0) return rc_stream;
   long long b = (T + ROWS_PER_BLOCK - 1) / ROWS_PER_BLOCK;
   const int per_sm = d <= 1024 ? 6 : 3;
   const int grid = (int)(b > pg_num_sms() * per_sm ? pg_num_sms() * per_sm : b);
   const int nch = (d + 127) / 128;
-#define LN_BWD_N(TI, TO, NCH, RES) ln_shift_bwd_kernel<TI, TO, NCH, RES><<<grid, 256, 0, s>>>((const TO*)dy, lddy, (const TI*)x, ldx, scale, mean, rstd, dres, (TO*)dout, ldo, dscale, dres_colsum, T, d, seq_len, shift)
+#define LN_BWD_N(TI, TO, NCH, RES) ln_shift_bwd_kernel<TI, TO, NCH, RES><<<grid, 256, 0, s>>>((const TO*)dy, lddy, (const TI*)x, ldx, scale, mean, rstd, dres, (TO*)dout, ldo, dscale, dres_colsum, (const TO*)gelu_u, ldu, T, d, seq_len, shift)
 #define LN_BWD(TI, TO, RES) do { if (nch <= 4) LN_BWD_N(TI, TO, 4, RES); else if (nch <= 8) LN_BWD_N(TI, TO, 8, RES); \
     else if (nch <= 16) LN_BWD_N(TI, TO, 16, RES); else LN_BWD_N(TI, TO, 32, RES); } while (0)
   if (residual) {
@@ -589,10 +613,18 @@
 int progen_sgu_gate_bwd(const void* ds, long long ldds, const void* xs, long long ldx, const void* gp, long long ldg,
                         const float* bias, void* dxs, long long lddx, void* dgp, long long lddg, float* dbias, int dtype,
                         long long T, int C, int seq_len, void* stream) {
+  return progen_sgu_gate_bwd_ex(ds, ldds, xs, ldx, gp, ldg, bias, dxs, lddx, dgp, lddg, dbias, nullptr, 0, dtype, T, C, seq_len,
+                                stream);
+}
+
+int progen_sgu_gate_bwd_ex(const void* ds, long long ldds, const void* xs, long long ldx, const void* gp, long long ldg,
+                           const float* bias, void* dxs, long long lddx, void* dgp, long long lddg, float* dbias,
+                           const void* gelu_u, long long ldu, int dtype, long long T, int C, int seq_len, void* stream) {
   PG_CHECK_ARG(T > 0 && C % 4 == 0);
-  cudaStream_t s = (cudaStream_t)stream;
-  if (dtype == PG_F32) sgu_gate_bwd_kernel<float><<<row_grid(T), 256, 0, s>>>((const float*)ds, ldds, (const float*)xs, ldx, (const float*)gp, ldg, bias, (float*)dxs, lddx, (float*)dgp, lddg, dbias, T, C, seq_len);
-  else sgu_gate_bwd_kernel<bf16><<<row_grid(T), 256, 0, s>>>((const bf16*)ds, ldds, (const bf16*)xs, ldx, (const bf16*)gp, ldg, bias, (bf16*)dxs, lddx, (bf16*)dgp, lddg, dbias, T, C, seq_len);
+  PG_CHECK_ARG(gelu_u == nullptr || ldu % 4 == 0);
+  cudaStream_t s = (cudaStream_t)stream;
+  if (dtype == PG_F32) sgu_gate_bwd_kernel<float><<<row_grid(T), 256, 0, s>>>((const float*)ds, ldds, (const float*)xs, ldx, (const float*)gp, ldg, bias, (float*)dxs, lddx, (float*)dgp, lddg, dbias, (const float*)gelu_u, ldu, T, C, seq_len);
+  else sgu_gate_bwd_kernel<bf16><<<row_grid(T), 256, 0, s>>>((const bf16*)ds, ldds, (const bf16*)xs, ldx, (const bf16*)gp, ldg, bias, (bf16*)dxs, lddx, (bf16*)dgp, lddg, dbias, (const bf16*)gelu_u, ldu, T, C, seq_len);
   PG_LAUNCH_CHECK();
   return PROGEN_OK;
 }
diff --git a/progen_b200/csrc/epilogues.cuh b/progen_b200/csrc/epilogues.cuh
--- a/progen_b200/csrc/epilogues.cuh
+++ b/progen_b200/csrc/epilogues.cuh
@@ -24,6 +24,7 @@
   int atomic;
   int tril;
   int tril_rows;
+  float* colsum;
 };
 
 struct DirectIO {
diff --git a/progen_b200/csrc/gemm_tc2.cu b/progen_b200/csrc/gemm_tc2.cu
--- a/progen_b200/csrc/gemm_tc2.cu
+++ b/progen_b200/csrc/gemm_tc2.cu
@@ -90,6 +90,9 @@
   auto tempty_bar = [&](int s) { return bar_base + 8u * (14 + s); };
   auto sready_bar = [&](int grp, int b) { return bar_base + 8u * (16 + grp * 3 + b); };
   const uint32_t tmem_slot = bar_base + 8u * 22;
+  auto sfull_bar = [&](int s) { return bar_base + 8u * (24 + s); };
+  constexpr bool CAN_SUM = KIND == EPI_ACCUM && B_MN;
+  const bool sums = CAN_SUM && g.epi.colsum != nullptr;
   uint8_t* gen = smem_raw + (smem_base - smem_u32(smem_raw));
 
   const int warp = threadIdx.x >> 5, lane = threadIdx.x & 31;
@@ -106,7 +109,11 @@
     if constexpr (E::ROWB1 > 0) prefetch_tensormap(&tma_out2);
   }
   if (warp == 1 && lane == 0) {
-    for (int s = 0; s < STAGES; ++s) { mbar_init(full_bar(s), 1); mbar_init(empty_bar(s), CL); }
+    for (int s = 0; s < STAGES; ++s) {
+      mbar_init(full_bar(s), 1);
+      mbar_init(empty_bar(s), CL + (sums ? 2 : 0));
+      if (sums) mbar_init(sfull_bar(s), 1);
+    }
     for (int s = 0; s < 2; ++s) { mbar_init(tfull_bar(s), 1); mbar_init(tempty_bar(s), 2 * EW); }
     for (int grp = 0; grp < NGROUP; ++grp)
       for (int b = 0; b < E::NB; ++b) mbar_init(sready_bar(grp, b), 1);
@@ -194,7 +201,61 @@
         if (++acc == 2) { acc = 0; acc_phase ^= 1; }
       }
     }
-  } else if (warp >= 4) {
+  } else if (warp < 4) {
+    if constexpr (CAN_SUM) {
+      if (sums) {
+        const int j = (warp - 2) * 32 + lane;
+        const int cc = j & 15, ph = j >> 4;
+        const uint8_t* bcol = gen + A_BYTES + (cc >> 3) * 8192;
+        int stage = 0;
+        uint32_t phase = 0;
+        int m0, n0, kb0, kb1;
+        for (int t = pair; decode_tile2<CL>(g, t, m0, n0, kb0, kb1); t += npairs) {
+          float s[8];
+#pragma unroll
+          for (int e = 0; e < 8; ++e) s[e] = 0.f;
+          for (int kb = kb0; kb < kb1; ++kb) {
+            if (leader) {
+              mbar_wait(full_bar(stage), phase);
+              if (warp == 2 && lane == 0) mbar_arrive_cluster(mapa(sfull_bar(stage), lead_crank + 1));
+            } else {
+              mbar_wait_cluster(sfull_bar(stage), phase);
+            }
+            if (m0 == 0) {
+              const uint8_t* box = bcol + stage * STAGE_BYTES;
+              uint4 v[16];
+#pragma unroll
+              for (int i = 0; i < 16; ++i) {
+                const int r = ph + 4 * i;
+                v[i] = *reinterpret_cast<const uint4*>(box + r * 128 + (((cc & 7) ^ (r & 7)) << 4));
+              }
+#pragma unroll
+              for (int i = 0; i < 16; ++i) {
+                const uint32_t w[4] = {v[i].x, v[i].y, v[i].z, v[i].w};
+#pragma unroll
+                for (int h = 0; h < 4; ++h) {
+                  s[2 * h] += __uint_as_float(w[h] << 16);
+                  s[2 * h + 1] += __uint_as_float(w[h] & 0xffff0000u);
+                }
+              }
+            }
+            __syncwarp();
+            if (lane == 0) mbar_arrive(empty_bar(stage));
+            if (++stage == STAGES) { stage = 0; phase ^= 1; }
+          }
+          if (m0 == 0) {
+#pragma unroll
+            for (int e = 0; e < 8; ++e) s[e] += __shfl_xor_sync(0xffffffffu, s[e], 16);
+            if (lane < 16) {
+              float* dst = g.epi.colsum + n0 + ncol + (int)rank * (BN / 2) + cc * 8;
+#pragma unroll
+              for (int e = 0; e < 8; ++e) atomicAdd(dst + e, s[e]);
+            }
+          }
+        }
+      }
+    }
+  } else {
     const int q = warp & 3;
     const int grp = (warp - 4) >> 2;
     const int r_in_tile = q * 32 + lane;
diff --git a/progen_b200/csrc/ln_stream.cu b/progen_b200/csrc/ln_stream.cu
--- a/progen_b200/csrc/ln_stream.cu
+++ b/progen_b200/csrc/ln_stream.cu
@@ -19,6 +19,7 @@
   float* dres;
   void* dout; long long ldo;
   float* dscale; float* dres_colsum;
+  const void* gelu_u; long long ldu;
   long long T; int d, seq_len, shift;
   int stages;
   int off_dy, off_r, off_out, off_stat, stage_bytes;
@@ -59,7 +60,7 @@
   }
 }
 
-template <typename TI, typename TO, int NCH, bool RESIDUAL, int RBT>
+template <typename TI, typename TO, int NCH, bool RESIDUAL, int RBT, bool GELU>
 __global__ void __launch_bounds__(32 * (RBT * CG + 1), 1) ln_shift_bwd_stream_kernel(const LnStreamArgs a) {
   constexpr int CWT = RBT * CG;
   extern __shared__ __align__(128) uint8_t smem[];
@@ -164,6 +165,16 @@
     const uint8_t* yn = yr + (size_t)d * sizeof(TO);
     float s1 = 0.f, s2 = 0.f;
     float kx[KEEP ? NCH : 1][4], kg[KEEP ? NCH : 1][4];
+    static_assert(!GELU || sizeof(TO) == 2, "GELU variant: bf16 activations");
+    uint2 gu[GELU ? NCH : 1];
+    if constexpr (GELU) {
+      const TO* ur = reinterpret_cast<const TO*>(a.gelu_u) + t * a.ldu;
+#pragma unroll
+      for (int ch = 0; ch < NCH; ++ch) {
+        const int c = ch * 128 + lane * 4;
+        if (c < d) gu[ch] = *reinterpret_cast<const uint2*>(ur + c);
+      }
+    }
 #pragma unroll
     for (int ch = 0; ch < NCH; ++ch) {
       const int c = ch * 128 + lane * 4;
@@ -217,6 +228,13 @@
           st4<float>(rr + c * 4, r);
           if (has_out) st4<TO>(reinterpret_cast<uint8_t*>(orow + c), r);
         } else {
+          if constexpr (GELU) {
+            const float2 u01 = __bfloat1622float2(*reinterpret_cast<const __nv_bfloat162*>(&gu[ch].x));
+            const float2 u23 = __bfloat1622float2(*reinterpret_cast<const __nv_bfloat162*>(&gu[ch].y));
+            const float uv[4] = {u01.x, u01.y, u23.x, u23.y};
+#pragma unroll
+            for (int i = 0; i < 4; ++i) o[i] = __bfloat162float(__float2bfloat16_rn(o[i])) * gelu_tanh_grad(uv[i]);
+          }
           st4<TO>(reinterpret_cast<uint8_t*>(orow + c), o);
         }
       }
@@ -248,22 +266,22 @@
   }
 }
 
-template <typename TI, typename TO, bool RESIDUAL>
+template <typename TI, typename TO, bool RESIDUAL, bool GELU = false>
 int launch_stream(const LnStreamArgs& a, int smem_bytes, int rbt, cudaStream_t s) {
   const long long nchunks = a.T / rbt;
   const int grid = (int)(nchunks < pg_num_sms() ? nchunks : pg_num_sms());
   static bool attr_set = false;
   if (!attr_set) {
-    PG_CUDA(cudaFuncSetAttribute(ln_shift_bwd_stream_kernel<TI, TO, 4, RESIDUAL, 8>, cudaFuncAttributeMaxDynamicSharedMemorySize, SMEM_BUDGET));
-    PG_CUDA(cudaFuncSetAttribute(ln_shift_bwd_stream_kernel<TI, TO, 8, RESIDUAL, 8>, cudaFuncAttributeMaxDynamicSharedMemorySize, SMEM_BUDGET));
-    PG_CUDA(cudaFuncSetAttribute(ln_shift_bwd_stream_kernel<TI, TO, 12, RESIDUAL, 4>, cudaFuncAttributeMaxDynamicSharedMemorySize, SMEM_BUDGET));
-    PG_CUDA(cudaFuncSetAttribute(ln_shift_bwd_stream_kernel<TI, TO, 16, RESIDUAL, 4>, cudaFuncAttributeMaxDynamicSharedMemorySize, SMEM_BUDGET));
+    PG_CUDA(cudaFuncSetAttribute(ln_shift_bwd_stream_kernel<TI, TO, 4, RESIDUAL, 8, GELU>, cudaFuncAttributeMaxDynamicSharedMemorySize, SMEM_BUDGET));
+    PG_CUDA(cudaFuncSetAttribute(ln_shift_bwd_stream_kernel<TI, TO, 8, RESIDUAL, 8, GELU>, cudaFuncAttributeMaxDynamicSharedMemorySize, SMEM_BUDGET));
+    PG_CUDA(cudaFuncSetAttribute(ln_shift_bwd_stream_kernel<TI, TO, 12, RESIDUAL, 4, GELU>, cudaFuncAttributeMaxDynamicSharedMemorySize, SMEM_BUDGET));
+    PG_CUDA(cudaFuncSetAttribute(ln_shift_bwd_stream_kernel<TI, TO, 16, RESIDUAL, 4, GELU>, cudaFuncAttributeMaxDynamicSharedMemorySize, SMEM_BUDGET));
     attr_set = true;
   }
-  if (a.d <= 512) ln_shift_bwd_stream_kernel<TI, TO, 4, RESIDUAL, 8><<<grid, 32 * (8 * CG + 1), smem_bytes, s>>>(a);
-  else if (a.d <= 1024) ln_shift_bwd_stream_kernel<TI, TO, 8, RESIDUAL, 8><<<grid, 32 * (8 * CG + 1), smem_bytes, s>>>(a);
-  else if (a.d <= 1536) ln_shift_bwd_stream_kernel<TI, TO, 12, RESIDUAL, 4><<<grid, 32 * (4 * CG + 1), smem_bytes, s>>>(a);
-  else ln_shift_bwd_stream_kernel<TI, TO, 16, RESIDUAL, 4><<<grid, 32 * (4 * CG + 1), smem_bytes, s>>>(a);
+  if (a.d <= 512) ln_shift_bwd_stream_kernel<TI, TO, 4, RESIDUAL, 8, GELU><<<grid, 32 * (8 * CG + 1), smem_bytes, s>>>(a);
+  else if (a.d <= 1024) ln_shift_bwd_stream_kernel<TI, TO, 8, RESIDUAL, 8, GELU><<<grid, 32 * (8 * CG + 1), smem_bytes, s>>>(a);
+  else if (a.d <= 1536) ln_shift_bwd_stream_kernel<TI, TO, 12, RESIDUAL, 4, GELU><<<grid, 32 * (4 * CG + 1), smem_bytes, s>>>(a);
+  else ln_shift_bwd_stream_kernel<TI, TO, 16, RESIDUAL, 4, GELU><<<grid, 32 * (4 * CG + 1), smem_bytes, s>>>(a);
   PG_LAUNCH_CHECK();
   return PROGEN_OK;
 }
@@ -272,8 +290,8 @@
 
 int ln_shift_bwd_stream_launch(const void* dy, long long lddy, int act_dtype, const void* x, long long ldx, int x_dtype,
                                const float* scale, const float* mean, const float* rstd, float* dres, void* dout,
-                               long long ldo, float* dscale, float* dres_colsum, long long T, int d, int seq_len, int shift,
-                               int residual, cudaStream_t stream) {
+                               long long ldo, float* dscale, float* dres_colsum, const void* gelu_u, long long ldu, long long T,
+                               int d, int seq_len, int shift, int residual, cudaStream_t stream) {
   static int enabled = [] { const char* e = getenv("PROGEN_LN_STREAM"); return e ? atoi(e) : 1; }();
   if (!enabled) return 1;
   const int so = act_dtype == PG_BF16 ? 2 : 4, si = x_dtype == PG_BF16 ? 2 : 4;
@@ -281,9 +299,11 @@
   if (T % RB != 0 || T % seq_len != 0 || d % 128 != 0 || d > 2048 || T < 8 * RB) return 1;
   if ((lddy * so) % 16 || (ldx * si) % 16 || (ldo * so) % 16) return 1;
   if (((uintptr_t)dy | (uintptr_t)x | (uintptr_t)dout | (uintptr_t)dres | (uintptr_t)mean | (uintptr_t)rstd) % 16) return 1;
+  if (gelu_u && (residual || ((uintptr_t)gelu_u % 8) || (ldu * so) % 8)) return 1;
   LnStreamArgs a{};
   a.dy = dy; a.lddy = lddy; a.x = x; a.ldx = ldx; a.scale = scale; a.mean = mean; a.rstd = rstd; a.dres = dres;
   a.dout = dout; a.ldo = ldo; a.dscale = dscale; a.dres_colsum = residual ? dres_colsum : nullptr;
+  a.gelu_u = gelu_u; a.ldu = ldu;
   a.T = T; a.d = d; a.seq_len = seq_len; a.shift = shift;
   auto up = [](int v) { return (v + 127) & ~127; };
   int off = up(rbt * d * si);
@@ -302,6 +322,10 @@
     if (act_dtype == PG_F32) LNS(float, float, true);
     LNS(float, bf16, true);
   }
+  if (gelu_u) {
+    if (act_dtype == PG_BF16 && x_dtype == PG_BF16) return launch_stream<bf16, bf16, false, true>(a, smem_bytes, rbt, stream);
+    return 1;
+  }
   if (act_dtype == PG_F32 && x_dtype == PG_F32) LNS(float, float, false);
   if (act_dtype == PG_BF16 && x_dtype == PG_BF16) LNS(bf16, bf16, false);
   if (act_dtype == PG_BF16 && x_dtype == PG_F32) LNS(float, bf16, false);
diff --git a/progen_b200/csrc/tc_ptx.cuh b/progen_b200/csrc/tc_ptx.cuh
--- a/progen_b200/csrc/tc_ptx.cuh
+++ b/progen_b200/csrc/tc_ptx.cuh
@@ -237,6 +237,17 @@
 __device__ __forceinline__ void mbar_arrive_cluster(uint32_t cluster_addr) {
   asm volatile("mbarrier.arrive.relaxed.cluster.shared::cluster.b64 _, [%0];" ::"r"(cluster_addr) : "memory");
 }
+__device__ __forceinline__ void mbar_wait_cluster(uint32_t bar, uint32_t parity) {
+  uint32_t ok = 0, spins = 0;
+  do {
+    asm volatile(
+        "{\n\t.reg .pred p;\n\t"
+        "mbarrier.try_wait.parity.acquire.cluster.shared::cta.b64 p, [%1], %2;\n\t"
+        "selp.u32 %0, 1, 0, p;\n\t}"
+        : "=r"(ok) : "r"(bar), "r"(parity) : "memory");
+    if (!ok && ++spins > (1u << 26)) __trap();
+  } while (!ok);
+}
 __device__ __forceinline__ void tma_load_2d_pair(uint32_t dst, const CUtensorMap* map, uint32_t bar_cluster_addr, int c0, int c1) {
   asm volatile(
       "cp.async.bulk.tensor.2d.cta_group::2.shared::cluster.global.mbarrier::complete_tx::bytes [%0], [%1, {%3, %4}], [%2];"
diff --git a/progen_b200/engine.py b/progen_b200/engine.py
--- a/progen_b200/engine.py
+++ b/progen_b200/engine.py
@@ -84,6 +84,8 @@
         self.attn_bwd_kind = os.environ.get('PROGEN_ATTN_BWD', 'tcgen05')
         if cfg['window_size'] % 128 != 0:
             self.attn_fwd_kind = self.attn_bwd_kind = 'mma'
+        self.fuse_bias_grad = self.mp and os.environ.get('PROGEN_FUSE_BIAS_GRAD', '1') != '0'
+        self.fuse_gelu_bwd = self.mp and os.environ.get('PROGEN_FUSE_GELU_BWD', '1') != '0'
         d, n, w = cfg['dim'], cfg['seq_len'], cfg['window_size']
         self.d, self.n, self.w, self.V = d, n, w, cfg['num_tokens']
         self.h, self.dh = cfg['heads'], cfg['dim_head']
@@ -243,14 +245,17 @@
         self._mm(M=self.T, N=K_in, K=N_out, A=dy, lda=N_out, B=w, ldb=N_out, out=out, ldo=kw.pop('ldo', K_in), epi=epi,
                  out_dtype=self.act_dt, **kw)
 
-    def wgrad_gemm(self, x, K_in, dy, N_out, dw):
+    def wgrad_gemm(self, x, K_in, dy, N_out, dw, bias_grad=None):
+        if bias_grad is not None and not self.fuse_bias_grad:
+            self.colsum(dy, N_out, bias_grad)
+            bias_grad = None
         split = 1
         if self.backend == L.BACKEND_TC:
             bn = 256 if (N_out % 256 == 0) else 128
             tiles = ((K_in + 127) // 128) * ((N_out + bn - 1) // bn)
             split = max(1, min(self.T // 64, 148 // tiles))
         self._mm(M=K_in, N=N_out, K=self.T, A=x, lda=K_in, a_mn=True, B=dy, ldb=N_out, b_mn=True, out=dw, ldo=N_out,
-                 epi=L.EPI_ACCUM, out_dtype=L.F32, split_k=split, atomic=split > 1)
+                 epi=L.EPI_ACCUM, out_dtype=L.F32, split_k=split, atomic=split > 1, colsum=bias_grad)
 
     def colsum(self, t, N, out, ld=None):
         L.check(self.lib.progen_colsum(t.data_ptr(), N if ld is None else ld, L.dt(t), out.data_ptr(), self.T, N, L.stream()), 'colsum')
@@ -374,8 +379,7 @@
         cfg, d, I, hid, T, n = self.cfg, self.d, self.I, self.hid, self.T, self.n
         shift = cfg['shift_tokens']
         hw, hl = P + 'linear', P + 'layer_norm'
-        self.colsum(self.dlogits, self.V, self.G(hw, 'b'))
-        self.wgrad_gemm(self.yf, d, self.dlogits, self.V, self.G(hw, 'w'))
+        self.wgrad_gemm(self.yf, d, self.dlogits, self.V, self.G(hw, 'w'), bias_grad=self.G(hw, 'b'))
         self.dgrad_gemm(self.dlogits, self.V, self.W(hw, 'w'), d, self.dy)
         self.dres.zero_()
         nl = len(self.kinds)
@@ -391,25 +395,27 @@
                 g = f + 'sgu'
                 self.wgrad_gemm(s['pj'], half, dres_lp, d, self.G(f + 'linear_1', 'w'))
                 self.dgrad_gemm(dres_lp, d, self.W(f + 'linear_1', 'w'), half, self.dpj)
-                self.colsum(self.dpj, half, self.G(g + '/~/linear', 'b'))
-                self.wgrad_gemm(s['sg'], half, self.dpj, half, self.G(g + '/~/linear', 'w'))
+                self.wgrad_gemm(s['sg'], half, self.dpj, half, self.G(g + '/~/linear', 'w'), bias_grad=self.G(g + '/~/linear', 'b'))
                 self.dgrad_gemm(self.dpj, half, self.W(g + '/~/linear', 'w'), half, self.dsg)
                 da = self.dh_
-                L.check(lib.progen_sgu_gate_bwd(self.dsg.data_ptr(), half, s['hact'].data_ptr(), hid, s['gp'].data_ptr(), half,
-                                                self.Pf(g, 'spatial_biases').data_ptr(), da.data_ptr(), hid, self.dgp.data_ptr(),
-                                                half, self.G(g, 'spatial_biases').data_ptr(), self.act_dt, T, half, n, st),
-                        'sgu_gate_bwd')
+                gu = s['u'] if self.fuse_gelu_bwd else None
+                L.check(lib.progen_sgu_gate_bwd_ex(self.dsg.data_ptr(), half, s['hact'].data_ptr(), hid, s['gp'].data_ptr(), half,
+                                                   self.Pf(g, 'spatial_biases').data_ptr(), da.data_ptr(), hid, self.dgp.data_ptr(),
+                                                   half, self.G(g, 'spatial_biases').data_ptr(), L.ptr(gu), hid, self.act_dt, T,
+                                                   half, n, st), 'sgu_gate_bwd')
                 self._mm(M=n, N=n, K=half, A=self.dgp, lda=half, B=s['gn'], ldb=half, out=self.G(g, 'spatial_weights'), ldo=n,
                          epi=L.EPI_ACCUM, out_dtype=L.F32, batch=self.B, a_batch_rows=n, b_batch_rows=n, batch_reduce=True,
                          atomic=True, tril=True, tril_rows=n)
                 self._mm(M=n, N=half, K=n, A=self.wm[i], lda=n, a_mn=True, B=self.dgp, ldb=half, b_mn=True, out=self.dgn,
                          ldo=half, out_dtype=self.act_dt, batch=self.B, b_batch_rows=n, d_batch_rows=n, causal=2)
                 gate = s['hact'][:, half:]
-                L.check(lib.progen_ln_shift_bwd(self.dgn.data_ptr(), half, self.act_dt, gate.data_ptr(), hid, self.act_dt,
-                                                self.Pf(g + '/~/layer_norm', 'scale').data_ptr(), s['mean3'].data_ptr(),
-                                                s['rstd3'].data_ptr(), 0, da[:, half:].data_ptr(), hid,
-                                                self.G(g + '/~/layer_norm', 'scale').data_ptr(), 0, T, half, n, 0, 0, st), 'ln_bwd_sgu')
-                L.check(lib.progen_gelu_bwd(da.data_ptr(), s['u'].data_ptr(), self.act_dt, T * hid, st), 'gelu_bwd')
+                L.check(lib.progen_ln_shift_bwd_ex(self.dgn.data_ptr(), half, self.act_dt, gate.data_ptr(), hid, self.act_dt,
+                                                   self.Pf(g + '/~/layer_norm', 'scale').data_ptr(), s['mean3'].data_ptr(),
+                                                   s['rstd3'].data_ptr(), 0, da[:, half:].data_ptr(), hid,
+                                                   self.G(g + '/~/layer_norm', 'scale').data_ptr(), 0,
+                                                   0 if gu is None else gu[:, half:].data_ptr(), hid, T, half, n, 0, 0, st), 'ln_bwd_sgu')
+                if gu is None:
+                    L.check(lib.progen_gelu_bwd(da.data_ptr(), s['u'].data_ptr(), self.act_dt, T * hid, st), 'gelu_bwd')
                 du, n_in = da, hid
             elif kind == 'glu':
                 self.wgrad_gemm(s['hact'], hid, dres_lp, d, self.G(f + 'linear_1', 'w'))
@@ -420,8 +426,7 @@
                 self.wgrad_gemm(s['hact'], hid, dres_lp, d, self.G(f + 'linear_1', 'w'))
                 self.dgrad_gemm(dres_lp, d, self.W(f + 'linear_1', 'w'), hid, self.dh_, epi=L.EPI_GELU_BWD, aux=s['u'], ldaux=hid)
                 du, n_in = self.dh_, hid
-            self.colsum(du, n_in, self.G(f + 'linear', 'b'))
-            self.wgrad_gemm(s['y2'], d, du, n_in, self.G(f + 'linear', 'w'))
+            self.wgrad_gemm(s['y2'], d, du, n_in, self.G(f + 'linear', 'w'), bias_grad=self.G(f + 'linear', 'b'))
             self.dgrad_gemm(du, n_in, self.W(f + 'linear', 'w'), d, self.dy)
             self.ln_bwd_res(self.dy, x1, self.Pf(f + 'layer_norm', 'scale'), s['mean2'], s['rstd2'], self.G(f + 'layer_norm', 'scale'), shift,
                             next_bias_grad=self.G(a + 'linear_1', 'b'))
diff --git a/progen_b200/lib.py b/progen_b200/lib.py
--- a/progen_b200/lib.py
+++ b/progen_b200/lib.py
@@ -27,6 +27,7 @@
         ('ldo', C.c_int64), ('ldo2', C.c_int64), ('ldaux', C.c_int64),
         ('A', C.c_void_p), ('B', C.c_void_p), ('out', C.c_void_p), ('out2', C.c_void_p),
         ('bias', C.c_void_p), ('aux', C.c_void_p), ('rot_sin', C.c_void_p), ('rot_cos', C.c_void_p),
+        ('colsum', C.c_void_p),
     ]
 
 
@@ -44,6 +45,7 @@
     'progen_embed_bwd': [_P, _P, _P, _LL, _I, _I, _P],
     'progen_ln_shift_fwd': [_P, _LL, _I, _P, _P, _LL, _I, _P, _P, _LL, _I, _I, _I, _P],
     'progen_ln_shift_bwd': [_P, _LL, _I, _P, _LL, _I, _P, _P, _P, _P, _P, _LL, _P, _P, _LL, _I, _I, _I, _I, _P],
+    'progen_ln_shift_bwd_ex': [_P, _LL, _I, _P, _LL, _I, _P, _P, _P, _P, _P, _LL, _P, _P, _P, _LL, _LL, _I, _I, _I, _I, _P],
     'progen_colsum': [_P, _LL, _I, _P, _LL, _I, _P],
     'progen_ce_fwd_bwd': [_P, _I, _P, _P, _P, _P, _I, _I, _I, _I, _F, _P],
     'progen_rotary_bwd': [_P, _LL, _I, _P, _P, _LL, _I, _I, _I, _P],
@@ -56,6 +58,7 @@
     'progen_local_attn_bwd_tc_ex': [_P, _P, _P, _P, _P, _P, _P, _P, _P, _P, _I, _I, _I, _I, _I, _I, _P],
     'progen_sgu_gate_fwd': [_P, _LL, _P, _LL, _P, _P, _LL, _I, _LL, _I, _I, _P],
     'progen_sgu_gate_bwd': [_P, _LL, _P, _LL, _P, _LL, _P, _P, _LL, _P, _LL, _P, _I, _LL, _I, _I, _P],
+    'progen_sgu_gate_bwd_ex': [_P, _LL, _P, _LL, _P, _LL, _P, _P, _LL, _P, _LL, _P, _P, _LL, _I, _LL, _I, _I, _P],
     'progen_gelu_bwd': [_P, _P, _I, _LL, _P],
     'progen_cast_f32': [_P, _P, _I, _LL, _P],
     'progen_tril_cast': [_P, _P, _I, _I, _P],
@@ -119,7 +122,7 @@
 def gemm(*, M, N, K, A, lda, B, ldb, out, ldo, epi=EPI_STORE, backend, a_mn=False, b_mn=False, in_dtype, out_dtype=F32,
          batch=1, a_batch_rows=0, b_batch_rows=0, d_batch_rows=0, batch_reduce=False, causal=0, split_k=1,
          out2=None, ldo2=0, bias=None, aux=None, ldaux=0, rot_sin=None, rot_cos=None, seq_len=0, dim_head=0,
-         atomic=False, tril=False, tril_rows=0):
+         atomic=False, tril=False, tril_rows=0, colsum=None):
     d = GemmDesc()
     d.M, d.N, d.K = M, N, K
     d.a_mn_major, d.b_mn_major = int(a_mn), int(b_mn)
@@ -133,4 +136,5 @@
     as_ptr = lambda x: x if isinstance(x, int) else ptr(x)
     d.A, d.B, d.out, d.out2 = as_ptr(A), as_ptr(B), as_ptr(out), as_ptr(out2)
     d.bias, d.aux, d.rot_sin, d.rot_cos = as_ptr(bias), as_ptr(aux), as_ptr(rot_sin), as_ptr(rot_cos)
+    d.colsum = as_ptr(colsum)
     check(load().progen_gemm(C.byref(d), stream()), 'progen_gemm')
```

After: 1.913 million (median of 6 runs). 2.7% higher.
